# yell/boltzmann-machines

Measured on AMD Instinct MI355X. Metric: Gibbs-steps/sec (CD-k, 784x1024 RBM, batch 512), higher is better.
Workload: dtype f32

## Files before the change

boltzmann_machines_amd/_ffi.py:

```python
import ctypes as C
import os

import numpy as np

from . import build as _build

MAX_LAYERS = 4
UNIT_BERNOULLI, UNIT_GAUSSIAN, UNIT_MULTINOMIAL = 0, 1, 2


class Bm355Error(RuntimeError):
    pass


class RbmConfig(C.Structure):
    _fields_ = [('n_visible', C.c_int32), ('n_hidden', C.c_int32), ('v_unit', C.c_int32),
                ('sample_v_states', C.c_int32), ('sample_h_states', C.c_int32),
                ('dbm_first', C.c_int32), ('dbm_last', C.c_int32), ('max_batch', C.c_int32),
                ('l2', C.c_float), ('sparsity_target', C.c_float), ('sparsity_cost', C.c_float),
                ('sparsity_damping', C.c_float), ('dropout', C.c_float),
                ('h_unit', C.c_int32), ('n_samples', C.c_int32)]


class DbmConfig(C.Structure):
# ... 67 lines not shown
    'bm_rbm64_train_step': [_vp, _vp, C.c_int32, C.c_double, C.c_double, C.c_int32],
    'bm_rbm64_train_step_metrics': [_vp, _vp, C.c_int32, C.c_double, C.c_double, C.c_int32, C.POINTER(C.c_double)],
    'bm_rbm64_transform': [_vp, _vp, C.c_int32, C.c_int32, _vp],
    'bm_rbm64_metrics': [_vp, _vp, C.c_int32, C.c_int32, C.POINTER(C.c_double)],
    'bm_rbm64_free_energy': [_vp, _vp, C.c_int32, C.POINTER(C.c_double)],
    'bm_dbm64_create': [C.POINTER(DbmConfig), C.POINTER(C.c_double), C.POINTER(_vp)],
    'bm_dbm64_destroy': [_vp],
    'bm_dbm64_sync': [_vp],
    'bm_dbm64_seed': [_vp, C.c_uint64],
    'bm_dbm64_set_row_offset': [_vp, C.c_int64, C.c_int64],
    'bm_dbm64_set_param': [_vp, C.c_char_p, _vp, _sz],
    'bm_dbm64_get_param': [_vp, C.c_char_p, _vp, _sz],
    'bm_dbm64_train_step': [_vp, _vp, C.c_double, C.c_double, C.c_int32, C.POINTER(C.c_int32), C.POINTER(C.c_double)],
    'bm_dbm64_metrics': [_vp, _vp, C.c_int32, C.POINTER(C.c_int32), C.POINTER(C.c_double)],
    'bm_dbm64_mean_field': [_vp, _vp, _vp, C.POINTER(C.c_int32)],
    'bm_dbm64_reconstruct': [_vp, _vp, _vp],
    'bm_dbm64_sample_v': [_vp, C.c_int32, _vp],
    'bm_dbm64_ais': [_vp, C.c_int32, C.c_int32, C.c_int32, C.c_uint64, C.c_int64, _vp],
    'bm_dbm64_log_proba': [_vp, _vp, _vp],
    'bm_rbm_create': [C.POINTER(RbmConfig), C.POINTER(_vp)],
    'bm_rbm_destroy': [_vp],
    'bm_rbm_sync': [_vp],
    'bm_rbm_set_param': [_vp, C.c_char_p, _vp, _sz],
    'bm_rbm_get_param': [_vp, C.c_char_p, _vp, _sz],
    'bm_rbm_set_param_dev': [_vp, C.c_char_p, _vp, _sz],
    'bm_rbm_dev_ptr': [_vp, C.c_char_p, C.POINTER(_vp), C.POINTER(_sz)],
    'bm_rbm_seed': [_vp, _u64],
    'bm_rbm_set_row_offset': [_vp, _i64],
    'bm_rbm_train_step': [_vp, _vp, _i32, _f32, _f32, _i32],
    'bm_rbm_train_step_metrics': [_vp, _vp, _i32, _f32, _f32, _i32, _fp],
    'bm_rbm_train_step_metrics_async': [_vp, _vp, _i32, _f32, _f32, _i32],
    'bm_rbm_collect_metrics': [_vp, _fp, _i32, C.POINTER(C.c_int32)],
    'bm_rbm_train_epoch': [_vp, _vp, _i64, _i32, _f32, _f32, _i32],
    'bm_rbm_stage': [_vp, _i32],
    'bm_rbm_get_staged': [_vp, _i32, C.c_char_p, _vp, _sz],
    'bm_rbm_grad_step': [_vp, _vp, _i32, _i32],
    'bm_rbm_apply_step': [_vp, _i32, _f32, _f32],
    'bm_rbm_transform': [_vp, _vp, _i32, _i32, _vp],
    'bm_rbm_metrics': [_vp, _vp, _i32, _i32, _fp],
    'bm_rbm_free_energy': [_vp, _vp, _i32, _fp],
    'bm_rbm_free_energy_rows': [_vp, _vp, _i32, _vp],
    'bm_rbm_ais': [_vp, _i32, _i32, _i32, _vp, _u64, _i64, _vp],
    'bm_rbm_gibbs': [_vp, _vp, _vp, _i32, _i32],
    'bm_rbm_gibbs_clamped': [_vp, _vp, _vp, _vp, _i32, _i32, _vp, _vp],
    'bm_rbm_pt_init': [_vp, _i32, _i32, _vp, _vp, _i64],
    'bm_rbm_pt_sweep': [_vp, _i32],
    'bm_rbm_pt_read': [_vp, _vp, _vp, _vp, _vp],
    'bm_rbm_train_step_pt': [_vp, _vp, _i32, _f32, _f32, _i32],
    'bm_rbm_train_epoch_pt': [_vp, _vp, _i64, _i32, _f32, _f32, _i32],
    'bm_rbm_stream': [_vp, C.POINTER(_vp)],
    'bm_rbm_profile': [_vp, _i32],
    'bm_rbm_kernel_times': [_vp, _fp, _ip],
    'bm_rbm_chain_stats': [_vp, C.POINTER(C.c_int64)],
    'bm_rbm_timer_start': [_vp],
    'bm_rbm_timer_stop': [_vp, _fp],
    'bm_rbm_timer_mark': [_vp],
    'bm_rbm_timer_elapsed': [_vp, _fp],
    'bm_dbm_create': [C.POINTER(DbmConfig), C.POINTER(_vp)],
    'bm_dbm_destroy': [_vp],
    'bm_dbm_sync': [_vp],
    'bm_dbm_seed': [_vp, _u64],
    'bm_dbm_set_row_offset': [_vp, _i64, _i64],
    'bm_dbm_set_param': [_vp, C.c_char_p, _vp, _sz],
    'bm_dbm_get_param': [_vp, C.c_char_p, _vp, _sz],
    'bm_dbm_dev_ptr': [_vp, C.c_char_p, C.POINTER(_vp), C.POINTER(_sz)],
    'bm_dbm_train_step': [_vp, _vp, _f32, _f32, _i32, _ip, _fp],
    'bm_dbm_metrics': [_vp, _vp, _i32, _ip, _fp],
    'bm_dbm_grad_step': [_vp, _vp, _i32, _ip],
    'bm_dbm_apply_step': [_vp, _i32, _i32, _f32, _f32],
    'bm_dbm_set_mf_allreduce': [_vp, _vp, _vp],
    'bm_dbm_set_comm': [_vp, _vp],
    'bm_dbm_ais_sharded': [_vp, _vp, _i32, _i32, _i32, _u64, _vp],
    'bm_dbm_ais_sharded_direct': [_vp, _vp, _i32, _i32, _i32, _u64, _vp],
    'bm_dbm_stream': [_vp, C.POINTER(_vp)],
    'bm_dbm_mean_field': [_vp, _vp, _vp, _ip],
    'bm_dbm_reconstruct': [_vp, _vp, _vp],
    'bm_dbm_sample_v': [_vp, _i32, _vp],
    'bm_dbm_sample_v_clamped': [_vp, _i32, _vp, _vp, _vp],
    'bm_dbm_pt_init': [_vp, _i32, _i32, _vp, _vp, _i64],
    'bm_dbm_pt_sweep': [_vp, _i32],
    'bm_dbm_pt_read': [_vp, _vp, _vp, _vp, _vp, _vp],
    'bm_dbm_ais': [_vp, _i32, _i32, _i32, _u64, _i64, _vp],
    'bm_dbm_log_proba': [_vp, _vp, _vp],
    'bm_dbm_timer_start': [_vp],
    'bm_dbm_timer_stop': [_vp, _fp],
    'bm_dbm_timer_mark': [_vp],
    'bm_dbm_timer_elapsed': [_vp, _fp],
}
_RESTYPE = {'bm_last_error': C.c_char_p, 'bm_version': C.c_char_p}
MF_REDUCE_FN = C.CFUNCTYPE(C.c_float, C.c_float, C.c_void_p)

_lib = None


def load(rebuild=True):
    global _lib
    if _lib is not None:
        return _lib
    path = _build.LIB
    if rebuild and _build.needs_build():
        import shutil
        have_hipcc = bool(shutil.which('hipcc')) or os.path.exists('/opt/rocm/bin/hipcc')
        try:
            _build.build()
        except Exception as e:
            if have_hipcc or not os.path.exists(path):
# ... 86 lines not shown
```

boltzmann_machines_amd/csrc/bm_gemm.h:

```cpp
#pragma once
#include <hip/hip_runtime.h>
#include <stdint.h>
#include <stdlib.h>
#include <string.h>

namespace bm {

struct NoSide {
    static constexpr bool kFinalSync = true;
    static constexpr bool kSplitFill = false, kCohQ = false;
    static constexpr bool kCanAbort = false;
    __device__ __forceinline__ void wait_inputs() {}
    __device__ __forceinline__ void post_fill() {}
    __device__ __forceinline__ void fill() {}
    __device__ __forceinline__ void drain() {}
};

#define BM_ABL(bit) ((ABL >> (bit)) & 1)

typedef float f32x4 __attribute__((ext_vector_type(4)));
typedef float f32x2v __attribute__((ext_vector_type(2)));

constexpr int NT = 256;

enum : int { KM = 0, XM = 1 };

template <int WI_, int WJ_, int MI_, int NJ_, int BK_, int NB_ = 4>
struct Geo {
    static constexpr int WI = WI_, WJ = WJ_, MI = MI_, NJ = NJ_, BK = BK_;
    static constexpr int NBUF = NB_;
    static constexpr int PF = NB_ - 1;
    static constexpr int NW = WI * WJ;
    static constexpr int NT = 64 * NW;
    static constexpr int TI = 16 * MI * WI;
    static constexpr int TJ = 16 * NJ * WJ;
    static constexpr int E = 4 * MI;
    static constexpr int P_BUF = TI * BK;
    static constexpr int Q_BUF = TJ * BK;
    static constexpr int SMEM_FLOATS = NBUF * (P_BUF + Q_BUF);
    static constexpr int NPP = P_BUF * 4 / (1024 * NW);
    static constexpr int NPQ = Q_BUF * 4 / (1024 * NW);
    static constexpr int NVP = TI * BK / (4 * NT);
    static constexpr int NVQ = TJ * BK / (4 * NT);
    static constexpr int SP = (MI == 2) ? 8 : 4;
    static constexpr int SQ = (NJ == 2) ? 8 : 4;
    static_assert(MI == 1 || MI == 2, "MI");
    static_assert(NJ == 1 || NJ == 2, "NJ");
    static_assert(BK == 32 || BK == 64, "BK");
    static_assert(NB_ >= 4 && NB_ <= 8, "ring depth");
    static_assert(NPP >= 1 && NPP * 1024 * NW == P_BUF * 4, "P chunk must split into whole DMA pieces per wave");
    static_assert(NPQ >= 1 && NPQ * 1024 * NW == Q_BUF * 4, "Q chunk must split into whole DMA pieces per wave");
    static_assert(NVP >= 1 && NVP * 4 * NT == TI * BK && NVQ >= 1 && NVQ * 4 * NT == TJ * BK, "register path split");
    static_assert(SMEM_FLOATS * 4 <= 160 * 1024 - 1024, "LDS");
};
using GeoAct = Geo<2, 2, 2, 1, 64>;
using GeoAct8 = Geo<2, 4, 1, 1, 64>;
using GeoActS = Geo<2, 2, 1, 1, 64>;
using GeoActS32 = Geo<2, 2, 1, 1, 32>;
using GeoAct32 = Geo<2, 2, 2, 1, 32>;
using GeoGrad = Geo<2, 2, 2, 2, 64>;
using GeoGrad8 = Geo<2, 4, 2, 1, 64>;
using GeoGrad8h = Geo<2, 4, 2, 1, 32>;
using GeoBf3S = Geo<1, 4, 2, 1, 64>;

struct Operand {
    const float *ptr;
    int ld;
    int nx;
    int vec;
};

static inline Operand make_operand(const float *p, int ld, int nx) {
    Operand o;
    o.ptr = p; o.ld = ld; o.nx = nx;
    o.vec = (((uintptr_t)p & 15u) == 0 && (ld & 3) == 0) ? 1 : 0;
    return o;
}

static inline bool operand_fast(const Operand &o, int layout, int K) {
    if (!o.ptr) return true;
    if (!o.vec) return false;
    return layout == KM ? (o.nx % 4 == 0 && o.nx >= 4) : (K % 4 == 0);
}

template <int BK> __device__ __forceinline__ int fx(int row) { return (BK == 64) ? (row & 15) : ((row >> 1) & 7); }
template <int S> __device__ __forceinline__ int fk(int row) { return S * ((row >> 2) & 1); }

template <int L, int TX, int BK, int S>
__device__ __forceinline__ int img_off(int row, int c4) {
    return (L == XM) ? row * BK + ((c4 ^ fx<BK>(row)) << 2) : row * TX + ((c4 ^ fk<S>(row)) << 2);
}

__device__ __forceinline__ float4 load4_guard(const float *p, bool row_ok, int col, int ncols, bool vec) {
    float4 v = make_float4(0.f, 0.f, 0.f, 0.f);
    if (row_ok) {
        if (vec && col + 3 < ncols) {
            v = *reinterpret_cast<const float4 *>(p);
        } else {
            if (col     < ncols) v.x = p[0];
            if (col + 1 < ncols) v.y = p[1];
            if (col + 2 < ncols) v.z = p[2];
            if (col + 3 < ncols) v.w = p[3];
        }
    }
    return v;
}

__device__ __forceinline__ float4 load4_coh(const float *p) {
    const unsigned long long *q = reinterpret_cast<const unsigned long long *>(p);
    const unsigned long long a = __hip_atomic_load(q, __ATOMIC_RELAXED, __HIP_MEMORY_SCOPE_AGENT);
    const unsigned long long b = __hip_atomic_load(q + 1, __ATOMIC_RELAXED, __HIP_MEMORY_SCOPE_AGENT);
    return make_float4(__uint_as_float((unsigned)a), __uint_as_float((unsigned)(a >> 32)),
                       __uint_as_float((unsigned)b), __uint_as_float((unsigned)(b >> 32)));
}

template <int L, int TX, int BK, int NTH, bool FAST, bool COH = false>
__device__ __forceinline__ void g2r(float4 (&reg)[TX * BK / (4 * NTH)], const float *ptr, int ld, int nx, int vec,
                                    int x0, int k0, int K, int tid) {
    static_assert(!COH || FAST, "coherent register path: 16-byte-legal operands only");
    constexpr int NV = TX * BK / (4 * NTH);
    constexpr int RC = (L == KM) ? TX / 4 : BK / 4;
#pragma unroll
    for (int n = 0; n < NV; ++n) {
        const int f = tid + n * NTH;
        const int row = f / RC, c4 = f % RC;
        const int k = (L == KM) ? k0 + row : k0 + c4 * 4;
        const int x = (L == KM) ? x0 + c4 * 4 : x0 + row;
        if (FAST) {
            const int kc = (L == KM) ? min(k, K - 1) : min(k, K - 4);
            const int xc = (L == KM) ? min(x, nx - 4) : min(x, nx - 1);
            const float *pc = (L == KM) ? ptr + (size_t)kc * ld + xc : ptr + (size_t)xc * ld + kc;
            reg[n] = COH ? load4_coh(pc) : *reinterpret_cast<const float4 *>(pc);
        } else if (L == KM) {
            reg[n] = load4_guard(ptr + (size_t)k * ld + x, k < K, x, nx, vec);
        } else {
            reg[n] = load4_guard(ptr + (size_t)x * ld + k, x < nx, k, K, vec);
        }
    }
}

template <int L, int TX, int BK, int NTH, int S, bool ZF = true>
__device__ __forceinline__ void r2s(const float4 (&reg)[TX * BK / (4 * NTH)], float *s, int tid, int kz) {
    constexpr int NV = TX * BK / (4 * NTH);
    constexpr int RC = (L == KM) ? TX / 4 : BK / 4;
#pragma unroll
    for (int n = 0; n < NV; ++n) {
        const int f = tid + n * NTH;
        const int row = f / RC, c4 = f % RC;
        float4 v = reg[n];
        if (!ZF) {
        } else if (L == KM) {
            if (row >= kz) v = make_float4(0.f, 0.f, 0.f, 0.f);
        } else {
            const int k = c4 * 4;
            if (k     >= kz) v.x = 0.f;
            if (k + 1 >= kz) v.y = 0.f;
            if (k + 2 >= kz) v.z = 0.f;
            if (k + 3 >= kz) v.w = 0.f;
        }
        *reinterpret_cast<float4 *>(s + img_off<L, TX, BK, S>(row, c4)) = v;
    }
}

template <class G> struct Frags {
    float p[G::BK / 4][G::MI];
    float q[G::BK / 4][G::NJ];
};

template <int QL, class G, int ABL = 0, int PL = KM>
__device__ __forceinline__ void read_frags(Frags<G> &f, const float *sP, const float *sQ, int wi, int wj, int lane) {
    static_assert(PL == KM || G::MI == 1, "x-major P needs MI == 1 (no interleaved sub-tiles)");
    constexpr int BK = G::BK;
    const int g = lane >> 4, l15 = lane & 15;
    if (BM_ABL(3)) {
#pragma unroll
        for (int kk = 0; kk < BK / 4; ++kk) { f.p[kk][0] = 1.f; f.p[kk][G::MI - 1] = 2.f; f.q[kk][0] = 1.f; f.q[kk][G::NJ - 1] = 1.f; }
        return;
    }
    if (PL == XM) {
        const int row = wi * 16 + l15;
#pragma unroll
        for (int m = 0; m < BK / 16; ++m) {
            const f32x4 v = *reinterpret_cast<const f32x4 *>(sP + img_off<XM, 0, BK, 0>(row, 4 * m + g));
#pragma unroll
            for (int j = 0; j < 4; ++j) f.p[4 * m + j][0] = v[j];
// ... 90 lines not shown
    Operand P2, Q2; int K2;
};

__device__ __forceinline__ int sel_i(int a, int b, int m) { return a ^ ((a ^ b) & m); }
__device__ __forceinline__ const float *sel_p(const float *a, const float *b, int m) {
    const uintptr_t ua = (uintptr_t)a, ub = (uintptr_t)b;
    return (const float *)(ua ^ ((ua ^ ub) & (uintptr_t)(intptr_t)m));
}

template <class G, int DW = G::NW> struct DmaPlan {
    static constexpr int NPP = G::P_BUF / (256 * DW), NPQ = G::Q_BUF / (256 * DW);
    uint32_t p[NPP], q[NPQ];
};

template <int L, int TX, int BK, int NW, int NP, int S>
__device__ __forceinline__ void plan_offsets(uint32_t (&off)[NP], int ld, int nx, int x0, int wave, int lane) {
    constexpr int RC = (L == KM) ? TX / 4 : BK / 4;
    constexpr int R = 64 / RC;
#pragma unroll
    for (int n = 0; n < NP; ++n) {
        const int pc = wave + n * NW;
        const int row = pc * R + lane / RC, slot = lane % RC;
        if (L == KM) {
            const int c4 = slot ^ fk<S>(row);
            off[n] = (uint32_t)(row * ld + min(x0 + c4 * 4, nx - 4)) * 4u;
        } else {
            const int c4 = slot ^ fx<BK>(row);
            off[n] = (uint32_t)(min(x0 + row, nx - 1) * ld + c4 * 4) * 4u;
        }
    }
}

template <int QL, class G, int PL = KM, int DW = G::NW>
__device__ __forceinline__ void make_plan(DmaPlan<G, DW> &pl, const Operand &P, const Operand &Q, int i0, int j0, int wave, int lane) {
    plan_offsets<PL, G::TI, G::BK, DW, DmaPlan<G, DW>::NPP, G::SP>(pl.p, P.ld, P.nx, i0, wave, lane);
    plan_offsets<QL, G::TJ, G::BK, DW, DmaPlan<G, DW>::NPQ, G::SQ>(pl.q, Q.ld, Q.nx, j0, wave, lane);
}

__device__ __forceinline__ void dma16(const char *src, float *lds_dst) {
    unsigned keep;
    const unsigned lds_addr = (unsigned)(uintptr_t)(__attribute__((address_space(3))) void *)lds_dst;
    asm volatile("s_mov_b32 %0, m0\n\ts_mov_b32 m0, %2\n\ts_nop 0\n\tglobal_load_lds_dwordx4 %1, off\n\ts_mov_b32 m0, %0"
                 : "=&s"(keep) : "v"(src), "s"(__builtin_amdgcn_readfirstlane(lds_addr)) : "memory");
}

__device__ __forceinline__ void dma16s(const void *sbase, uint32_t voff, unsigned lds_byte) {
    asm volatile("s_mov_b32 m0, %2\n\ts_nop 0\n\tglobal_load_lds_dwordx4 %1, %0"
                 :: "s"(sbase), "v"(voff), "s"(lds_byte) : "memory");
}
__device__ __forceinline__ void dma16s_coh(const void *sbase, uint32_t voff, unsigned lds_byte) {
    asm volatile("s_mov_b32 m0, %2\n\ts_nop 0\n\tglobal_load_lds_dwordx4 %1, %0 sc1"
                 :: "s"(sbase), "v"(voff), "s"(lds_byte) : "memory");
}
template <class G, int DW, bool QSC = false, bool QHALF = false>
__device__ __forceinline__ void dma_chunk_s(const DmaPlan<G, DW> &pl, const char *pb, const char *qb, unsigned ldsP, unsigned ldsQ) {
#pragma unroll
    for (int n = 0; n < DmaPlan<G, DW>::NPP; ++n) dma16s(pb, pl.p[n], ldsP + (unsigned)(n * DW * 1024));
#pragma unroll
    for (int n = 0; n < DmaPlan<G, DW>::NPQ; ++n) {
        if (QHALF && (n & 1)) continue;
        if (QSC) dma16s_coh(qb, pl.q[n], ldsQ + (unsigned)(n * DW * 1024));
        else     dma16s(qb, pl.q[n], ldsQ + (unsigned)(n * DW * 1024));
    }
}

template <int QL, class G, bool SEG2, int PL = KM, int DW = G::NW, bool QHALF = false>
__device__ __forceinline__ void dma_chunk(const KRange &kr, const DmaPlan<G, DW> &pl1, const DmaPlan<G, DW> &pl2, int nch1, int c,
                                          float *sP, float *sQ, int wave) {
    constexpr int BK = G::BK;
    const int m = SEG2 ? -(int)(c >= nch1) : 0;
    const int kc = c - (nch1 & m);
    const int ldp = SEG2 ? sel_i(kr.P1.ld, kr.P2.ld, m) : kr.P1.ld;
    const int ldq = SEG2 ? sel_i(kr.Q1.ld, kr.Q2.ld, m) : kr.Q1.ld;
    const char *pb = (const char *)((SEG2 ? sel_p(kr.P1.ptr, kr.P2.ptr, m) : kr.P1.ptr) +
                                    ((PL == KM) ? (size_t)kc * BK * ldp : (size_t)kc * BK));
    const char *qb = (const char *)((SEG2 ? sel_p(kr.Q1.ptr, kr.Q2.ptr, m) : kr.Q1.ptr) +
                                    ((QL == KM) ? (size_t)kc * BK * ldq : (size_t)kc * BK));
#pragma unroll
    for (int n = 0; n < DmaPlan<G, DW>::NPP; ++n) {
        const uint32_t o1 = pl1.p[n], o2 = SEG2 ? pl2.p[n] : 0u;
        const uint32_t o = SEG2 ? (o1 ^ ((o1 ^ o2) & (uint32_t)m)) : o1;
        dma16(pb + o, sP + (wave + n * DW) * 256);
    }
#pragma unroll
    for (int n = 0; n < DmaPlan<G, DW>::NPQ; ++n) {
        if (QHALF && (n & 1)) continue;
        const uint32_t o1 = pl1.q[n], o2 = SEG2 ? pl2.q[n] : 0u;
        const uint32_t o = SEG2 ? (o1 ^ ((o1 ^ o2) & (uint32_t)m)) : o1;
        dma16(qb + o, sQ + (wave + n * DW) * 256);
    }
}

template <int QL, class G, bool FAST, bool SEG2, int PL = KM, bool COHQ = false>
__device__ __forceinline__ void load_chunk(ChunkRegs<G> &r, const KRange &kr, int nch1, int i0, int j0, int c, int tid) {
    constexpr int BK = G::BK;
    if (!SEG2) {
        g2r<PL, G::TI, BK, G::NT, FAST>(r.p, kr.P1.ptr, kr.P1.ld, kr.P1.nx, kr.P1.vec, i0, c * BK, kr.K1, tid);
        g2r<QL, G::TJ, BK, G::NT, FAST, COHQ>(r.q, kr.Q1.ptr, kr.Q1.ld, kr.Q1.nx, kr.Q1.vec, j0, c * BK, kr.K1, tid);
    } else {
        const int m = -(int)((c >= nch1) & (kr.K2 > 0));
        const int kc = c - (nch1 & m);
        const int K = sel_i(kr.K1, kr.K2, m);
        g2r<PL, G::TI, BK, G::NT, FAST>(r.p, sel_p(kr.P1.ptr, kr.P2.ptr, m), sel_i(kr.P1.ld, kr.P2.ld, m),
                                        sel_i(kr.P1.nx, kr.P2.nx, m), sel_i(kr.P1.vec, kr.P2.vec, m), i0, kc * BK, K, tid);
        g2r<QL, G::TJ, BK, G::NT, FAST, COHQ>(r.q, sel_p(kr.Q1.ptr, kr.Q2.ptr, m), sel_i(kr.Q1.ld, kr.Q2.ld, m),
                                              sel_i(kr.Q1.nx, kr.Q2.nx, m), sel_i(kr.Q1.vec, kr.Q2.vec, m), j0, kc * BK, K, tid);
    }
}

template <int QL, class G, bool SEG2, int PL = KM>
__device__ __forceinline__ void store_chunk(const ChunkRegs<G> &r, const KRange &kr, int nch1, int c,
                                            float *sP, float *sQ, int tid) {
    constexpr int BK = G::BK;
    const int m = SEG2 ? -(int)((c >= nch1) & (kr.K2 > 0)) : 0;
    const int kz = sel_i(kr.K1, kr.K2, m) - (c - (nch1 & m)) * BK;
    r2s<PL, G::TI, BK, G::NT, G::SP>(r.p, sP, tid, kz);
    r2s<QL, G::TJ, BK, G::NT, G::SQ>(r.q, sQ, tid, kz);
}

template <class G> struct RegPlan {
    uint32_t p[G::NVP], q[G::NVQ];
};
template <int L, int TX, int BK, int NTH>
__device__ __forceinline__ void reg_offsets(uint32_t (&off)[TX * BK / (4 * NTH)], int ld, int nx, int x0, int tid) {
    constexpr int NV = TX * BK / (4 * NTH);
    constexpr int RC = (L == KM) ? TX / 4 : BK / 4;
#pragma unroll
    for (int n = 0; n < NV; ++n) {
        const int f = tid + n * NTH;
        const int row = f / RC, c4 = f % RC;
        off[n] = (L == KM) ? (uint32_t)(row * ld + min(x0 + c4 * 4, nx - 4)) * 4u
                           : (uint32_t)(min(x0 + row, nx - 1) * ld + c4 * 4) * 4u;
    }
}
template <int QL, class G, int PL = KM>
__device__ __forceinline__ void make_reg_plan(RegPlan<G> &pl, const Operand &P, const Operand &Q, int i0, int j0, int tid) {
    reg_offsets<PL, G::TI, G::BK, G::NT>(pl.p, P.ld, P.nx, i0, tid);
    reg_offsets<QL, G::TJ, G::BK, G::NT>(pl.q, Q.ld, Q.nx, j0, tid);
}
template <int QL, class G, bool SEG2, int PL = KM>
__device__ __forceinline__ void load_chunk_slim(ChunkRegs<G> &r, const KRange &kr, const RegPlan<G> &pl1,
                                                const RegPlan<G> &pl2, int nch1, int c) {
    constexpr int BK = G::BK;
    const int m = SEG2 ? -(int)(c >= nch1) : 0;
    const int kc = c - (nch1 & m);
    const int ldp = SEG2 ? sel_i(kr.P1.ld, kr.P2.ld, m) : kr.P1.ld;
    const int ldq = SEG2 ? sel_i(kr.Q1.ld, kr.Q2.ld, m) : kr.Q1.ld;
    const char *pb = (const char *)((SEG2 ? sel_p(kr.P1.ptr, kr.P2.ptr, m) : kr.P1.ptr) +
                                    ((PL == KM) ? (size_t)kc * BK * ldp : (size_t)kc * BK));
    const char *qb = (const char *)((SEG2 ? sel_p(kr.Q1.ptr, kr.Q2.ptr, m) : kr.Q1.ptr) +
                                    ((QL == KM) ? (size_t)kc * BK * ldq : (size_t)kc * BK));
#pragma unroll
    for (int n = 0; n < G::NVP; ++n) {
        const uint32_t o1 = pl1.p[n], o2 = SEG2 ? pl2.p[n] : 0u;
        const uint32_t o = SEG2 ? (o1 ^ ((o1 ^ o2) & (uint32_t)m)) : o1;
        r.p[n] = *reinterpret_cast<const float4 *>(pb + o);
    }
#pragma unroll
// ... 8 lines not shown
    r2s<PL, G::TI, G::BK, G::NT, G::SP, false>(r.p, sP, tid, 0);
    r2s<QL, G::TJ, G::BK, G::NT, G::SQ, false>(r.q, sQ, tid, 0);
}

enum : int { STG_DMA = 0, STG_REG = 1, STG_DMAH = 2 };

#define BM_WAIT_VM(n) asm volatile("s_waitcnt vmcnt(%0)" ::"n"(n) : "memory")
template <int NPW, int MAXC>
__device__ __forceinline__ void wait_vm_chunks(int n) {
    static_assert(MAXC * NPW <= 63, "vmcnt range");
    if (MAXC >= 4 && n >= 4)      BM_WAIT_VM(4 * NPW <= 63 ? 4 * NPW : 0);
    else if (MAXC >= 3 && n == 3) BM_WAIT_VM(3 * NPW <= 63 ? 3 * NPW : 0);
    else if (MAXC >= 2 && n == 2) BM_WAIT_VM(2 * NPW <= 63 ? 2 * NPW : 0);
    else if (n == 1)              BM_WAIT_VM(NPW);
    else                          BM_WAIT_VM(0);
}
__device__ __forceinline__ void wg_barrier() {
    asm volatile("s_waitcnt lgkmcnt(0)" ::: "memory");
    __builtin_amdgcn_s_barrier();
    asm volatile("" ::: "memory");
}

template <int QL, class G, bool FAST, bool SEG2, int ABL = 0, int PL = KM, int STG = STG_DMA, class Side = NoSide>
__device__ __forceinline__ void mainloop(f32x4 (&acc)[G::MI][G::NJ], const KRange &kr, int i0, int j0, float *smem,
                                         Side &side, long long *stamps = nullptr) {
#ifdef BM_PROBE
#define BM_MSTAMP(n) do { if (stamps && threadIdx.x == 0) stamps[n] = (long long)__builtin_readcyclecounter(); } while (0)
#else
#define BM_MSTAMP(n) do {} while (0)
#endif
    constexpr int BK = G::BK, P_BUF = G::P_BUF, Q_BUF = G::Q_BUF, NBUF = G::NBUF, PF = G::PF;
    constexpr int DW = (STG == STG_DMAH && G::NW == 8) ? 4 : G::NW;
    constexpr int NPW = DmaPlan<G, DW>::NPP + (BM_ABL(9) ? (DmaPlan<G, DW>::NPQ + 1) / 2 : DmaPlan<G, DW>::NPQ);
    const int tid = threadIdx.x, lane = tid & 63;
    const int w = __builtin_amdgcn_readfirstlane(tid >> 6);
    const int wi = w % G::WI, wj = w / G::WI;
    float *sP = smem, *sQ = smem + NBUF * P_BUF;
    const int nch1 = (kr.K1 + BK - 1) / BK;
    const int nch = nch1 + (SEG2 ? (kr.K2 + BK - 1) / BK : 0);
    const int nfull1 = kr.K1 / BK, nfull2 = SEG2 ? kr.K2 / BK : 0;
    auto is_full = [&](int c) -> bool {
        return (c < nfull1) | (SEG2 && c >= nch1 && c - nch1 < nfull2);
    };
    auto is_dma = [&](int c) -> bool {
        if (!FAST || STG == STG_REG || BM_ABL(6)) return false;
        return is_full(c);
    };
    ChunkRegs<G> gr;
    Frags<G> fa, fb;
    DmaPlan<G, DW> pl1, pl2;
    RegPlan<G> rp1, rp2;
    const bool dmaw = (DW == G::NW) || w < DW;
    ChunkRegs<G> g0, g1;
    if (FAST && STG != STG_REG && dmaw) {
        make_plan<QL, G, PL, DW>(pl1, kr.P1, kr.Q1, i0, j0, w, lane);
        if (SEG2) make_plan<QL, G, PL, DW>(pl2, kr.P2, kr.Q2, i0, j0, w, lane);
    }
    int n_reg = 0;
    if (FAST && STG == STG_REG && !BM_ABL(6) && !BM_ABL(0)) {
        while (n_reg + 4 < nch && is_full(n_reg + 4) && is_full(n_reg + 2)) ++n_reg;
        n_reg &= ~1;
        if (n_reg > 0 && !(is_full(0) && is_full(1) && is_full(2) && is_full(3))) n_reg = 0;
        if (n_reg > 0) {
            make_reg_plan<QL, G, PL>(rp1, kr.P1, kr.Q1, i0, j0, tid);
            if (SEG2) make_reg_plan<QL, G, PL>(rp2, kr.P2, kr.Q2, i0, j0, tid);
        }
    }
    BM_MSTAMP(0);
    if (n_reg > 0) {
        ChunkRegs<G> ga, gb;
        load_chunk_slim<QL, G, SEG2, PL>(ga, kr, rp1, rp2, nch1, 0);
        load_chunk_slim<QL, G, SEG2, PL>(gb, kr, rp1, rp2, nch1, 1);
        load_chunk_slim<QL, G, SEG2, PL>(g0, kr, rp1, rp2, nch1, 2);
        load_chunk_slim<QL, G, SEG2, PL>(g1, kr, rp1, rp2, nch1, 3);
        __builtin_amdgcn_sched_barrier(0);
        side.fill();
        __builtin_amdgcn_sched_barrier(0);
        store_chunk_slim<QL, G, PL>(ga, sP, sQ, tid);
        store_chunk_slim<QL, G, PL>(gb, sP + P_BUF, sQ + Q_BUF, tid);
    } else if constexpr (Side::kSplitFill) {
        static_assert(FAST && STG == STG_DMA && DW == G::NW, "chained fill");
        const unsigned l0 = (unsigned)(uintptr_t)(__attribute__((address_space(3))) void *)smem;
        const unsigned lP = l0 + (unsigned)w * 1024u, lQ = l0 + (unsigned)(NBUF * P_BUF * 4) + (unsigned)w * 1024u;
#pragma unroll
        for (int c = 0; c < PF; ++c) {
            const char *pb = (const char *)kr.P1.ptr + (size_t)c * ((PL == KM) ? (size_t)BK * kr.P1.ld * 4 : (size_t)BK * 4);
#pragma unroll
            for (int n = 0; n < DmaPlan<G, DW>::NPP; ++n) dma16s(pb, pl1.p[n], lP + (unsigned)(c * P_BUF * 4 + n * DW * 1024));
        }
        __builtin_amdgcn_sched_barrier(0);
        side.fill();
        __builtin_amdgcn_sched_barrier(0);
        side.wait_inputs();
#pragma unroll
        for (int c = 0; c < PF; ++c) {
            const char *qb = (const char *)kr.Q1.ptr + (size_t)c * ((QL == KM) ? (size_t)BK * kr.Q1.ld * 4 : (size_t)BK * 4);
#pragma unroll
            for (int n = 0; n < DmaPlan<G, DW>::NPQ; ++n) dma16s_coh(qb, pl1.q[n], lQ + (unsigned)(c * Q_BUF * 4 + n * DW * 1024));
        }
        constexpr int NQ_LEFT = (PF - 2) * DmaPlan<G, DW>::NPQ;
        BM_WAIT_VM(NQ_LEFT);
    } else {
#pragma unroll
        for (int c = 0; c < PF; ++c)
            if (c < nch && is_dma(c) && dmaw && !BM_ABL(0))
                dma_chunk<QL, G, SEG2, PL, DW, (BM_ABL(9) != 0)>(kr, pl1, pl2, nch1, c, sP + (c % NBUF) * P_BUF, sQ + (c % NBUF) * Q_BUF, w);
        __builtin_amdgcn_sched_barrier(0);
        side.fill();
        __builtin_amdgcn_sched_barrier(0);
#pragma unroll
        for (int c = 0; c < 2; ++c)
            if (c < nch && !is_dma(c) && !BM_ABL(0)) {
                load_chunk<QL, G, FAST, SEG2, PL>(gr, kr, nch1, i0, j0, c, tid);
                store_chunk<QL, G, SEG2, PL>(gr, kr, nch1, c, sP + (c % NBUF) * P_BUF, sQ + (c % NBUF) * Q_BUF, tid);
            }
        {
            int n_after = 0;
#pragma unroll
            for (int c = 2; c < PF; ++c) n_after += (c < nch && is_dma(c) && !BM_ABL(0)) ? 1 : 0;
            wait_vm_chunks<NPW, PF - 2>(n_after);
        }
    }
    BM_MSTAMP(1);
    if (!BM_ABL(5)) wg_barrier();
    if constexpr (Side::kCanAbort) {
        side.post_fill();
        if (side.aborted) { BM_WAIT_VM(0); return; }
    }
    read_frags<QL, G, ABL, PL>(fa, sP, sQ, wi, wj, lane);
    BM_MSTAMP(2);
    const int klast = (SEG2 && kr.K2 > 0) ? kr.K2 - (nch - nch1 - 1) * BK : kr.K1 - (nch1 - 1) * BK;
    const int nq_last = (klast + 15) / 16;
    constexpr int NM = (BK / 4) * G::MI * G::NJ;
    constexpr int NRP = (PL == XM) ? BK / 16 : BK / 4;
    constexpr int NRQ = (QL == XM) ? (BK / 16) * G::NJ : BK / 4;
    constexpr int NR = NRP + NRQ;
#define BM_SG(mask, n) __builtin_amdgcn_sched_group_barrier(mask, n, 0);
#ifndef BM_SCHED_VARIANT
#define BM_SCHED_VARIANT 0
#endif
#if BM_SCHED_VARIANT == 0
#define BM_SCHED_STEP                                                                             \
    if (DW == G::NW) { _Pragma("unroll") for (int s_ = 0; s_ < NPW; ++s_) { BM_SG(0x008, 1) BM_SG(0x020, 1) } } \
    _Pragma("unroll") for (int s_ = 0; s_ < NR; ++s_) { BM_SG(0x008, 1) BM_SG(0x100, 1) }         \
    BM_SG(0x008, NM)
#elif BM_SCHED_VARIANT == 1
#define BM_SCHED_STEP                                                                             \
    _Pragma("unroll") for (int s_ = 0; s_ < NR; ++s_) { BM_SG(0x008, 1) BM_SG(0x100, 1) }         \
    _Pragma("unroll") for (int s_ = 0; s_ < NPW; ++s_) { BM_SG(0x008, 1) BM_SG(0x020, 1) }        \
    BM_SG(0x008, NM)
#else
#define BM_SCHED_STEP
#endif
    static_assert(NBUF == 4, "the steps below are written for a 4-slot ring");
    int cc = 0;
    const unsigned lds0 = (unsigned)(uintptr_t)(__attribute__((address_space(3))) void *)smem;
    const unsigned ldsPw = lds0 + (unsigned)w * 1024u, ldsQw = lds0 + (unsigned)(NBUF * P_BUF * 4) + (unsigned)w * 1024u;
    bool in2 = false;
    auto chunk_bases = [&](int c, const char *&pb, const char *&qb) {
        const bool s2 = SEG2 && c >= nch1;
        const Operand &P = s2 ? kr.P2 : kr.P1, &Q = s2 ? kr.Q2 : kr.Q1;
        const int kc = s2 ? c - nch1 : c;
        pb = (const char *)P.ptr + (size_t)kc * ((PL == KM) ? (size_t)BK * P.ld * 4 : (size_t)BK * 4);
        qb = (const char *)Q.ptr + (size_t)kc * ((QL == KM) ? (size_t)BK * Q.ld * 4 : (size_t)BK * 4);
    };
#define BM_DMA_AT(CD, SD)                                                                         \
    {                                                                                             \
        if (SEG2 && !in2 && (CD) >= nch1) { in2 = true; pl1 = pl2; }                              \
        const char *pb_, *qb_;                                                                    \
        chunk_bases((CD), pb_, qb_);                                                              \
        if (dmaw) dma_chunk_s<G, DW, Side::kCohQ, (BM_ABL(9) != 0)>(pl1, pb_, qb_, ldsPw + (unsigned)((SD) * P_BUF * 4), \
                                     ldsQw + (unsigned)((SD) * Q_BUF * 4));                       \
    }
#define BM_STEP_Q(FC, FN, S)                                                                      \
    {                                                                                             \
        BM_DMA_AT(cc + PF, ((S) + PF) % NBUF)                                                     \
        read_frags<QL, G, ABL, PL>(FN, sP + (((S) + 1) % NBUF) * P_BUF, sQ + (((S) + 1) % NBUF) * Q_BUF, wi, wj, lane); \
        mfma_frags<G, ABL>(acc, FC);                                                              \
        BM_SCHED_STEP                                                                             \
        if (!BM_ABL(8)) BM_WAIT_VM((PF - 2) * NPW);                                               \
        if (!BM_ABL(5)) wg_barrier();                                                             \
        ++cc;                                                                                     \
    }
#define BM_STEP_T(FC, FN, S1, S2, S3)       \
    {                                                                                             \
        const int cd = cc + PF, cr = cc + 2;                                                      \
        const bool do_dma = cd < nch && is_dma(cd) && !BM_ABL(0);                                 \
        const bool do_reg = cr < nch && !is_dma(cr) && !BM_ABL(0);                                \
        if (cc == last - 1) side.drain();       \
        if (do_reg) load_chunk<QL, G, FAST, SEG2, PL, Side::kCohQ>(gr, kr, nch1, i0, j0, cr, tid); \
        if (do_dma) BM_DMA_AT(cd, S3)                                                             \
        read_frags<QL, G, ABL, PL>(FN, sP + (S1) * P_BUF, sQ + (S1) * Q_BUF, wi, wj, lane);       \
        mfma_frags<G, ABL>(acc, FC);                                                              \
        _Pragma("unroll") for (int s_ = 0; s_ < NR; ++s_) { BM_SG(0x008, 1) BM_SG(0x100, 1) }     \
        BM_SG(0x008, NM)                                                                          \
        if (do_reg) {                                                                             \
            BM_WAIT_VM(0);                                                                        \
            store_chunk<QL, G, SEG2, PL>(gr, kr, nch1, cr, sP + (S2) * P_BUF, sQ + (S2) * Q_BUF, tid); \
        } else if (cr < nch) {                                                                    \
             \
            int n_after = 0;                                                                      \
            _Pragma("unroll") for (int c_ = 3; c_ <= PF; ++c_) n_after += (cc + c_ < nch && is_dma(cc + c_) && !BM_ABL(0)) ? 1 : 0; \
            wait_vm_chunks<NPW, PF - 2>(n_after);                                                 \
        }                                                                                         \
        if (!BM_ABL(5)) wg_barrier();                                                             \
        ++cc;                                                                                     \
    }
#define BM_STEP_TC(FC, FN, S) BM_STEP_T(FC, FN, ((S) + 1) % NBUF, ((S) + 2) % NBUF, ((S) + 3) % NBUF)
#define BM_STEP_TR(FC, FN)    BM_STEP_T(FC, FN, (cc + 1) % NBUF, (cc + 2) % NBUF, (cc + 3) % NBUF)
    constexpr int NWR = G::NVP + G::NVQ;
#ifndef BM_REG_SCHED_VARIANT
#define BM_REG_SCHED_VARIANT 0
#endif
#if BM_REG_SCHED_VARIANT == 0
#define BM_REG_SCHED(RELOAD)                                                                      \
        _Pragma("unroll") for (int s_ = 0; s_ < NWR; ++s_) { BM_SG(0x008, 1) BM_SG(0x200, 1) }    \
        if (RELOAD) { _Pragma("unroll") for (int s_ = 0; s_ < NWR; ++s_) { BM_SG(0x008, 1) BM_SG(0x020, 1) } } \
        _Pragma("unroll") for (int s_ = 0; s_ < NR; ++s_) { BM_SG(0x008, 1) BM_SG(0x100, 1) }     \
        BM_SG(0x008, NM)
#elif BM_REG_SCHED_VARIANT == 1
#define BM_REG_SCHED(RELOAD)                                                                      \
        _Pragma("unroll") for (int s_ = 0; s_ < NR; ++s_) { BM_SG(0x008, (NM >= 64 ? 2 : 1)) BM_SG(0x100, 2) } \
        _Pragma("unroll") for (int s_ = 0; s_ < NWR; ++s_) { BM_SG(0x008, (NM >= 32 ? 2 : 1)) BM_SG(0x200, 1) } \
        if (RELOAD) { _Pragma("unroll") for (int s_ = 0; s_ < NWR; ++s_) { BM_SG(0x008, 1) BM_SG(0x020, 1) } } \
        BM_SG(0x008, NM)
#else
#define BM_REG_SCHED(RELOAD)
#endif
#define BM_STEP_REG(FC, FN, G_, RELOAD, S)                                                        \
    {                                                                                             \
        store_chunk_slim<QL, G, PL>(G_, sP + (((S) + 2) % NBUF) * P_BUF, sQ + (((S) + 2) % NBUF) * Q_BUF, tid); \
        if (RELOAD) load_chunk_slim<QL, G, SEG2, PL>(G_, kr, rp1, rp2, nch1, cc + 4);             \
        read_frags<QL, G, ABL, PL>(FN, sP + (((S) + 1) % NBUF) * P_BUF, sQ + (((S) + 1) % NBUF) * Q_BUF, wi, wj, lane); \
        mfma_frags<G, ABL>(acc, FC);                                                              \
        BM_REG_SCHED(RELOAD)                                                                      \
        if (!BM_ABL(5)) wg_barrier();                                                             \
        ++cc;                                                                                     \
    }
    if (n_reg > 0) {
        int left = n_reg;
#pragma unroll 1
        while (left >= 4) {
            BM_STEP_REG(fa, fb, g0, true, 0)
// ... 200 lines not shown
```

boltzmann_machines_amd/csrc/bm_kernels.h:

```cpp
#pragma once
#include <stdio.h>
#include <stdlib.h>
#include <string.h>
#include "bm_gemm.h"
#include "bm_bf3.h"
#include "bm_numerics.h"
#include "bm_rng.h"

namespace bm {

struct MfCtl { unsigned maxdiff; int done; int steps; float resid; };

struct ActArgs {
    Operand P1, Q1; int K1;
    int p_xm;
    Operand P2, Q2; int K2;
    int I, J;
    const float *bias;
    const float *sigma;
    float mult;
    float bmult;
    int kind;
    int sample;
    int lit;
// ... 62 lines not shown
        if (a.kind == 0) {
#pragma unroll
            for (int r = 0; r < 4; ++r) s[r] = (u32_to_uniform(wds[r]) < m[r]) ? 1.f : 0.f;
        } else {
            float n[4];
            box_muller(wds[0], wds[1], n[0], n[1]);
            box_muller(wds[2], wds[3], n[2], n[3]);
#pragma unroll
            for (int r = 0; r < 4; ++r) s[r] = n[r] * a.sigma[ib + r] + m[r];
        }
    } else {
#pragma unroll
        for (int r = 0; r < 4; ++r) {
            if (r >= nvalid) break;
            const unsigned long long idx = flat + r;
            uint32_t wds[4];
            philox_block(key, idx >> 2, wds);
            if (a.kind == 0) {
                s[r] = (u32_to_uniform(wds[idx & 3]) < m[r]) ? 1.f : 0.f;
            } else {
                float n0, n1;
                const int pr = (int)(idx & 3) >> 1;
                box_muller(wds[2 * pr], wds[2 * pr + 1], n0, n1);
                s[r] = ((idx & 1) ? n1 : n0) * a.sigma[ib + r] + m[r];
            }
        }
    }
}

#ifndef BM_NT_STORES
#define BM_NT_STORES 1
#endif
typedef float f32x2 __attribute__((ext_vector_type(2)));
__device__ __forceinline__ void stream_store4(float *p, float x, float y, float z, float w) {
    if (BM_NT_STORES) __builtin_nontemporal_store((f32x4){x, y, z, w}, reinterpret_cast<f32x4 *>(p));
    else *reinterpret_cast<float4 *>(p) = make_float4(x, y, z, w);
}
__device__ __forceinline__ void stream_store2(float *p, float x, float y) {
    if (BM_NT_STORES) __builtin_nontemporal_store((f32x2){x, y}, reinterpret_cast<f32x2 *>(p));
    else *reinterpret_cast<float2 *>(p) = make_float2(x, y);
}

template <bool CACHED = false>
__device__ __forceinline__ void store4(float *dst, size_t o, const float *v, int nvalid, bool v4) {
    if (v4) {
        if (CACHED) *reinterpret_cast<float4 *>(dst + o) = make_float4(v[0], v[1], v[2], v[3]);
        else stream_store4(dst + o, v[0], v[1], v[2], v[3]);
    } else {
#pragma unroll
        for (int r = 0; r < 4; ++r) if (r < nvalid) dst[o + r] = v[r];
    }
}

template <int MI> struct PhiloxFor { typedef PhiloxPair type; };
template <> struct PhiloxFor<1> { typedef PhiloxOne type; };

__device__ __forceinline__ float wave_max_lane63(float v) {
#define BM_DPP_MAX(ctrl, rmask) v = fmaxf(v, __int_as_float(__builtin_amdgcn_update_dpp(__float_as_int(v), __float_as_int(v), ctrl, rmask, 0xf, false)))
    BM_DPP_MAX(0xb1, 0xf);
    BM_DPP_MAX(0x4e, 0xf);
    BM_DPP_MAX(0x124, 0xf);
    BM_DPP_MAX(0x128, 0xf);
    BM_DPP_MAX(0x142, 0xa);
    BM_DPP_MAX(0x143, 0xc);
#undef BM_DPP_MAX
    return v;
}

template <int E, class Rng, bool MF = false, int NTH = 256> struct ActSide {
    static constexpr bool kFinalSync = false;
    static constexpr bool kSplitFill = false, kCohQ = false, kCanAbort = MF;
    static constexpr bool kMF = MF;
    const float *bias, *sigma;
    const float *prev_row;
    int ib0, I, with_rng;
    float bs[E], sg[E], pv[E];
    Rng rng;
    MfCtl *chk_ctl; const float *chk_slots; int chk_n; float chk_tol; const int *skip; float *s_chk; int aborted, nthreads;

    __device__ __forceinline__ void load_inputs() {
        const float *sp = sigma ? sigma : bias;
        const bool has_sigma = sigma != nullptr;
        if (MF && prev_row) {
            if (E == 4 && ib0 + 3 < I && (((uintptr_t)prev_row & 15u) == 0)) {
                const float4 t = *reinterpret_cast<const float4 *>(prev_row);
                pv[0] = t.x; pv[1] = t.y; pv[2] = t.z; pv[E - 1] = t.w;
            } else {
#pragma unroll
                for (int e = 0; e < E; ++e) pv[e] = (ib0 + e < I) ? prev_row[e] : 0.f;
            }
        }
        if (MF && E == 4 && ib0 + 3 < I && (((uintptr_t)(bias + ib0) & 15u) == 0) && (((uintptr_t)(sp + ib0) & 15u) == 0)) {
            const float4 b = *reinterpret_cast<const float4 *>(bias + ib0), v = *reinterpret_cast<const float4 *>(sp + ib0);
            bs[0] = b.x; bs[1] = b.y; bs[2] = b.z; bs[E - 1] = b.w;
            sg[0] = has_sigma ? v.x : 1.0f; sg[1] = has_sigma ? v.y : 1.0f; sg[2] = has_sigma ? v.z : 1.0f; sg[E - 1] = has_sigma ? v.w : 1.0f;
            return;
        }
#pragma unroll
        for (int e = 0; e < E; ++e) {
            const int i = (ib0 + e < I) ? ib0 + e : I - 1;
            bs[e] = bias[i];
            const float sv = sp[i];
            sg[e] = has_sigma ? sv : 1.0f;
        }
    }
    static constexpr int CHK_MAX = 4096;
    float *s_slots;
    static __device__ __forceinline__ void dma4_lane0(const void *src, float *lds_dst) {
        if ((threadIdx.x & 63) == 0) {
            unsigned keep;
            const unsigned lds_addr = (unsigned)(uintptr_t)(__attribute__((address_space(3))) void *)lds_dst;
            asm volatile("s_mov_b32 %0, m0\n\ts_mov_b32 m0, %2\n\ts_nop 0\n\tglobal_load_lds_dword %1, off\n\ts_mov_b32 m0, %0"
                         : "=&s"(keep) : "v"(src), "s"(__builtin_amdgcn_readfirstlane(lds_addr)) : "memory");
        }
    }
    __device__ __forceinline__ void preload() {
        if constexpr (MF) {
            load_inputs();
            aborted = 0;
            const int w = threadIdx.x >> 6, lane = threadIdx.x & 63;
            if (chk_ctl) {
                for (int p = w; p * 256 < chk_n && p * 256 < CHK_MAX; p += nthreads / 64)
                    dma16(reinterpret_cast<const char *>(chk_slots + 256 * p) + 16 * lane, s_slots + 256 * p);
                if (w == 0) dma4_lane0(&chk_ctl->done, s_slots + CHK_MAX);
            } else if (skip) {
// ... 98 lines not shown
            const int ib = ib0 + 4 * hlf;
            if (ib >= a.I) break;
            const int nvalid = (a.I - ib < 4) ? a.I - ib : 4;
            float m[4], s[4];
#pragma unroll
            for (int r = 0; r < 4; ++r) {
                const float x = (RT ? rm : a.mult) * z[4 * hlf + r];
                const float b = (RT ? rm : a.bmult) * bs[4 * hlf + r];
                m[r] = (a.kind == 0) ? (LIT ? sigmoid_literal(x + b) : (HWMATH ? sigmoid_hw(x + b) : sigmoid(x + b)))
                                     : (a.kind == 1 ? (x * sg[4 * hlf + r] + b) : (a.kind == 3 ? x + b : x));
                s[r] = m[r];
            }
            if (a.sample) {
                if (rng_fast) {
                    const uint32_t *wds = rng.words(hlf);
                    if (a.kind == 0) {
#pragma unroll
                        for (int r = 0; r < 4; ++r) s[r] = (u32_to_uniform(wds[r]) < m[r]) ? 1.f : 0.f;
                    } else {
                        float n[4];
                        box_muller(wds[0], wds[1], n[0], n[1]);
                        box_muller(wds[2], wds[3], n[2], n[3]);
#pragma unroll
                        for (int r = 0; r < 4; ++r) s[r] = n[r] * sg[4 * hlf + r] + m[r];
                    }
                } else {
                    const unsigned long long flat = (unsigned long long)(a.row0 + j) * (unsigned long long)a.I + ib;
                    draw4(a, key, flat, ib, nvalid, m, s, false);
                }
            }
            if constexpr (CL) {
#pragma unroll
                for (int r = 0; r < 4; ++r)
                    if (cm[hlf][r] != 0.f) { m[r] = cv[hlf][r]; s[r] = cv[hlf][r]; }
            }
            if constexpr (RT) {
#pragma unroll
                for (int r = 0; r < 4; ++r) sv[4 * hlf + r] = s[r];
            }
            const size_t o = (size_t)j * a.ldo + ib;
            if constexpr (SideT::kMF) {
                if (a.prev) {
#pragma unroll
                    for (int r = 0; r < 4; ++r)
                        if (r < nvalid) dmax = fmaxf(dmax, fabsf(m[r] - side.pv[4 * hlf + r]));
                }
            }
            const bool v4 = al_out && nvalid == 4;
            if (a.means) store4<HWMATH>(a.means, o, m, nvalid, v4 && (((uintptr_t)a.means & 15u) == 0));
            if (a.negmeans) {
                float nm[4];
#pragma unroll
                for (int r = 0; r < 4; ++r) nm[r] = -m[r];
                store4<HWMATH>(a.negmeans, o, nm, nvalid, v4 && (((uintptr_t)a.negmeans & 15u) == 0));
            }
            if (a.states) store4<HWMATH>(a.states, o, s, nvalid, v4 && (((uintptr_t)a.states & 15u) == 0));
            if constexpr (RT) {
                if (a.sel_out && rm == 1.0f) {
                    const int c = j / a.sel_R;
                    if (c < a.sel_rows)
                        store4<HWMATH>(a.sel_out, (size_t)c * a.sel_ld + ib, s, nvalid,
                                       nvalid == 4 && ((a.sel_ld & 3) == 0) && (((uintptr_t)a.sel_out & 15u) == 0));
                }
            }
            if (HWMATH && a.states16) {
                uint16_t *d = a.states16 + (size_t)j * a.ld16 + ib;
                if (nvalid == 4 && (ib & 3) == 0) {
                    uint2 pk;
                    pk.x = (__float_as_uint(s[0]) >> 16) | (__float_as_uint(s[1]) & 0xffff0000u);
                    pk.y = (__float_as_uint(s[2]) >> 16) | (__float_as_uint(s[3]) & 0xffff0000u);
                    *reinterpret_cast<uint2 *>(d) = pk;
                } else {
#pragma unroll
                    for (int r = 0; r < 4; ++r) if (r < nvalid) d[r] = (uint16_t)(__float_as_uint(s[r]) >> 16);
                }
            }
        }
    }
    if constexpr (FE) { if (a.fe_zero && i0 == 0 && j0 == 0 && tid < 6) a.fe_zero[tid] = 0.0; }
    bool row_sums = a.rowacc || a.rowdot_out;
    if constexpr (RT) row_sums = row_sums || a.rowen_out;
    if (row_sums) {
        float racc = 0.f, rdot = 0.f, racc2 = 0.f, ren = 0.f;
        (void)ren;
        if (j < a.J) {
            int fc = 0; float delta = 0.f;
            if constexpr (FE) {
                fc = (a.fe_flip == FE_FLIP_FROM_KEY) ? pll_flip_col(a.fe_key, (unsigned long long)(a.row0 + j), a.K1) : a.fe_flip[j];
                delta = 1.0f - 2.0f * a.fe_x[(size_t)j * a.fe_ldx + fc];
            }
#pragma unroll
            for (int hlf = 0; hlf < NH; ++hlf) {
                float qa = 0.f, qd = 0.f, qa2 = 0.f, qe = 0.f;
                (void)qe;
#pragma unroll
                for (int r = 0; r < 4; ++r) {
                    const int e = 4 * hlf + r, i = ib0 + e;
                    if (i >= a.I) break;
                    if (a.rowacc) {
                        if (a.dot_mat) {
                            qa += z[e] * a.dot_mat[(size_t)j * a.ld_dot + i];
                        } else {
                            const float t = z[e] + bs[e];
                            if constexpr (FE) qa2 += softplus(t + delta * a.fe_w[(size_t)fc * a.fe_ldw + i]);
                            if (a.rowacc_single) qa += HWMATH ? softplus_hw(a.beta_b * t) : softplus(a.beta_b * t);
                            else qa += softplus_hw(a.beta_b * t) - softplus_hw(a.beta_a * t);
                        }
// ... 116 lines not shown

template <class G, bool SEG2, int MINW>
__global__ __launch_bounds__(G::NT, MINW) void act_bf3_kernel(ActArgs a, Bf3Strip sp) {
    __shared__ __attribute__((aligned(16))) float smem[Bf3Geo<G>::SMEM_FLOATS];
    constexpr int E = G::E;
    const int ti = (int)blockIdx.x / sp.strips, st = (int)blockIdx.x % sp.strips;
    const int per = sp.tiles_j / sp.strips, rem = sp.tiles_j % sp.strips;
    const int tj0 = st * per + (st < rem ? st : rem), tj1 = tj0 + per + (st < rem ? 1 : 0);
    const int i0 = ti * G::TI;
    const int tid = threadIdx.x, lane = tid & 63, w = tid >> 6;
    const int wi = w % G::WI, wj = w / G::WI;
    const int g = lane >> 4, l15 = lane & 15;
    const int ib0 = i0 + wi * (16 * G::MI) + g * E;
    ActSide<E, typename PhiloxFor<G::MI>::type> side;
    side.bias = a.bias; side.sigma = a.sigma; side.ib0 = ib0; side.I = a.I; side.with_rng = 0;
    side.prev_row = nullptr;
    side.fill();
    side.with_rng = a.sample;
    Bf3Pipe<G, SEG2> pipe;
    pipe.setup(a.b3, i0, smem);
    if (tj0 < tj1) { pipe.set_tile(a.b3, tj0 * G::TJ); pipe.prefetch(); }
    for (int tj = tj0; tj < tj1; ++tj) {
        const int j0 = tj * G::TJ, j = j0 + wj * 16 + l15;
        f32x4 acc[G::MI][1];
#pragma unroll
        for (int t = 0; t < G::MI; ++t) acc[t][0] = (f32x4){0.f, 0.f, 0.f, 0.f};
        side.rng.init(a.key, ((unsigned long long)(a.row0 + j) * (unsigned long long)a.I + ib0) >> 2);
        if (a.sample) side.rng.fill();
        if (!(sp.abl & 2)) pipe.run(acc);
        if (tj + 1 < tj1) { pipe.set_tile(a.b3, (tj + 1) * G::TJ); pipe.prefetch(); }
        if (!(sp.abl & 1)) (void)act_epilogue<G, 0, decltype(side), true>(a, a.key, acc, side, i0, j0);
    }
}

struct ColSumJob {
    const float *A, *Bm;
    int lda, ldb, ncols, nrows;
    float *out;
};
constexpr int MAX_COLJOBS = 12;
struct ColSumArgs {
    ColSumJob job[MAX_COLJOBS];
    int first_wave[MAX_COLJOBS + 1];
    int njobs;
};

constexpr int CS_ROWS = 128;
constexpr int CS_LD = 80;
constexpr int CS_SMEM_FLOATS = 2 * CS_ROWS * CS_LD;

constexpr int CS_NV = CS_ROWS * 16 / NT;
struct ColRegs { float4 a[CS_NV], b[CS_NV]; };

__device__ __forceinline__ void cs_fetch(ColRegs &r, const float *A, int lda, const float *Bm, int ldb,
                                         int c0, int ncols, int nrows, int r0, int tid) {
    const int c4 = tid & 15;
    const int cc = min(c0 + 4 * c4, ncols - 4);
#pragma unroll
    for (int n = 0; n < CS_NV; ++n) {
        const int rc = min(r0 + (tid >> 4) + 16 * n, nrows - 1);
        r.a[n] = *reinterpret_cast<const float4 *>(A + (size_t)rc * lda + cc);
        r.b[n] = Bm ? *reinterpret_cast<const float4 *>(Bm + (size_t)rc * ldb + cc) : make_float4(0.f, 0.f, 0.f, 0.f);
    }
}

__device__ __forceinline__ void cs_stash(const ColRegs &r, float *sA, float *sB, int c0, int ncols, int nrows,
                                         int r0, int tid) {
    const int c4 = tid & 15;
#pragma unroll
    for (int n = 0; n < CS_NV; ++n) {
        const int row = (tid >> 4) + 16 * n;
        const bool ok = (r0 + row < nrows) && (c0 + 4 * c4 < ncols);
        float4 va = r.a[n], vb = r.b[n];
        if (!ok) { va = make_float4(0.f, 0.f, 0.f, 0.f); vb = va; }
        *reinterpret_cast<float4 *>(sA + row * CS_LD + 4 * c4) = va;
        *reinterpret_cast<float4 *>(sB + row * CS_LD + 4 * c4) = vb;
    }
}

__device__ __forceinline__ void block_colsum(const float *A, int lda, const float *Bm, int ldb,
                                             int c0, int ncols, int nrows, bool want2,
                                             float *smem, f32x4 &sum1, f32x4 &sum2, bool negB = false) {
    const int tid = threadIdx.x, lane = tid & 63, w = tid >> 6;
    const int g = lane >> 4, l15 = lane & 15;
    float *sA = smem, *sB = smem + CS_ROWS * CS_LD;
    sum1 = (f32x4){0.f, 0.f, 0.f, 0.f};
    sum2 = (f32x4){0.f, 0.f, 0.f, 0.f};
    const bool vec = (((uintptr_t)A & 15u) == 0) && ((lda & 3) == 0) && ((ncols & 3) == 0) &&
                     (!Bm || ((((uintptr_t)Bm & 15u) == 0) && ((ldb & 3) == 0)));
    ColRegs regs;
    if (vec) cs_fetch(regs, A, lda, Bm, ldb, c0, ncols, nrows, 0, tid);
    for (int r0 = 0; r0 < nrows; r0 += CS_ROWS) {
        const int nr = (nrows - r0 < CS_ROWS) ? nrows - r0 : CS_ROWS;
        if (vec) {
            cs_stash(regs, sA, sB, c0, ncols, nrows, r0, tid);
        } else {
            for (int e = tid; e < CS_ROWS * 64; e += NT) {
                const int row = e >> 6, cc = e & 63, c = c0 + cc;
                const bool ok = row < nr && c < ncols;
                sA[row * CS_LD + cc] = ok ? A[(size_t)(r0 + row) * lda + c] : 0.f;
                sB[row * CS_LD + cc] = (ok && Bm) ? Bm[(size_t)(r0 + row) * ldb + c] : 0.f;
            }
        }
        wg_barrier();
        if (vec) cs_fetch(regs, A, lda, Bm, ldb, c0, ncols, nrows, r0 + CS_ROWS, tid);
        const int nsteps = (((nr + 3) / 4) + 7) & ~7;
        const int co = w * 16 + l15;
        for (int s = 0; s < nsteps; s += 8) {
            float d[8], e[8];
#pragma unroll
            for (int u = 0; u < 8; ++u) {
                const int o = (4 * (s + u) + g) * CS_LD + co;
                e[u] = sB[o];
                d[u] = negB ? sA[o] + e[u] : sA[o] - e[u];
            }
#pragma unroll
            for (int u = 0; u < 8; ++u) {
                sum1 = __builtin_amdgcn_mfma_f32_16x16x4f32(d[u], 1.0f, sum1, 0, 0, 0);
                if (want2) sum2 = __builtin_amdgcn_mfma_f32_16x16x4f32(e[u], 1.0f, sum2, 0, 0, 0);
            }
        }
        wg_barrier();
    }
    if (negB) sum2 = -sum2;
}

__global__ __launch_bounds__(NT) void colsum_kernel(ColSumArgs a) {
    __shared__ __attribute__((aligned(16))) float smem[CS_SMEM_FLOATS];
    const int wv = blockIdx.x, lane = threadIdx.x & 63, w = threadIdx.x >> 6;
    int jb = 0;
    while (jb + 1 < a.njobs && wv >= a.first_wave[jb + 1]) ++jb;
    const ColSumJob J = a.job[jb];
    const int c0 = (wv - a.first_wave[jb]) * 64;
    f32x4 s1, s2;
    block_colsum(J.A, J.lda, J.Bm, J.ldb, c0, J.ncols, J.nrows, false, smem, s1, s2);
    if ((lane & 15) == 0) {
        const int g = lane >> 4;
#pragma unroll
        for (int r = 0; r < 4; ++r) {
            const int cc = c0 + w * 16 + g * 4 + r;
            if (cc < J.ncols) J.out[cc] = s1[r];
        }
    }
}

struct RbmBiasArgs {
    const float *sv, *sh, *sq;
    float *vb, *dvb, *hb, *dhb, *q, *pen;
    int V, H;
    float N, lr, mom, damping, cost, target;
};
__global__ void rbm_bias_kernel(RbmBiasArgs a) {
    const int c = blockIdx.x * blockDim.x + threadIdx.x;
    if (c < a.V) {
        const float g = a.sv[c] / a.N;
        const float d = a.lr * (a.mom * a.dvb[c] + g);
        a.dvb[c] = d;
        a.vb[c] = a.vb[c] + d;
    } else if (c < a.V + a.H) {
        const int h = c - a.V;
        const float qn = a.damping * a.q[h] + (1.0f - a.damping) * a.sq[h];
        a.q[h] = qn;
        const float pen = a.cost * (qn - a.target);
        a.pen[h] = pen;
        float g = a.sh[h] / a.N;
        g = g - pen;
        const float d = a.lr * (a.mom * a.dhb[h] + g);
        a.dhb[h] = d;
        a.hb[h] = a.hb[h] + d;
    }
}

struct RbmBiasFusedArgs {
    const float *X, *vs, *h0m, *hm;
    int ldx, ldv, ldh0, ldh, B;
    int hm_negated;
    float *raw_tail;
    int raw_only;
    RbmBiasArgs u;
};
__device__ __forceinline__ void rbm_bias_fused_block(const RbmBiasFusedArgs &a, int wv, float *smem) {
    const int lane = threadIdx.x & 63, w = threadIdx.x >> 6, g = lane >> 4;
    const int nv = (a.u.V + 63) / 64;
    f32x4 s1, s2;
    if (wv < nv) {
        const int c0 = wv * 64;
        block_colsum(a.X, a.ldx, a.vs, a.ldv, c0, a.u.V, a.B, false, smem, s1, s2);
        if ((lane & 15) == 0) {
#pragma unroll
            for (int r = 0; r < 4; ++r) {
                const int c = c0 + w * 16 + g * 4 + r;
                if (c < a.u.V) {
                    a.raw_tail[c] = s1[r];
                    if (a.raw_only) continue;
                    const float gr = s1[r] / a.u.N;
                    const float d = a.u.lr * (a.u.mom * a.u.dvb[c] + gr);
                    a.u.dvb[c] = d;
                    a.u.vb[c] = a.u.vb[c] + d;
                }
            }
        }
    } else {
        const int c0 = (wv - nv) * 64;
        block_colsum(a.h0m, a.ldh0, a.hm, a.ldh, c0, a.u.H, a.B, true, smem, s1, s2, a.hm_negated != 0);
        if ((lane & 15) == 0) {
#pragma unroll
            for (int r = 0; r < 4; ++r) {
                const int h = c0 + w * 16 + g * 4 + r;
                if (h < a.u.H) {
                    const float sq = s2[r];
                    a.raw_tail[a.u.V + h] = s1[r];
                    a.raw_tail[a.u.V + a.u.H + h] = sq;
                    if (a.raw_only) continue;
                    const float qn = a.u.damping * a.u.q[h] + (1.0f - a.u.damping) * sq;
                    a.u.q[h] = qn;
                    const float pen = a.u.cost * (qn - a.u.target);
                    a.u.pen[h] = pen;
                    float gr = s1[r] / a.u.N;
                    gr = gr - pen;
                    const float d = a.u.lr * (a.u.mom * a.u.dhb[h] + gr);
                    a.u.dhb[h] = d;
                    a.u.hb[h] = a.u.hb[h] + d;
                }
            }
        }
    }
}

__global__ __launch_bounds__(NT) void rbm_bias_fused_kernel(RbmBiasFusedArgs a) {
    __shared__ __attribute__((aligned(16))) float smem[CS_SMEM_FLOATS];
    rbm_bias_fused_block(a, blockIdx.x, smem);
}

struct GradArgs {
    Operand Ppos, Qpos; int Kpos;
    Operand Pneg, Qneg; int Kneg;
    int I, J;
    int form;
    int fused;
    float *raw;
    float *raw2;
    float *W, *dW;
    float *Wt;
    int ldw, ldwt;
    const float *pen;
    float N, M, l2, lr, mom;
    int nbias;
    RbmBiasFusedArgs bias;
    int fetch_at_fill;
    int map_xi;
#ifdef BM_PROBE
    long long *dbg;
#endif
};

__device__ __forceinline__ void apply_w_update(float g, float pen, float l2, float lr, float mom,
                                               float &w, float &dw) {
    g = __fsub_rn(g, __fmul_rn(l2, w));
    g = __fsub_rn(g, pen);
    const float d = __fmul_rn(lr, __fadd_rn(__fmul_rn(mom, dw), g));
    dw = d;
    w = __fadd_rn(w, d);
}
__device__ __forceinline__ bool grad_pow2(float N) { return ((__float_as_uint(N) & 0x007fffffu) == 0u) && N >= 1.0f; }
__device__ __forceinline__ float grad_norm1(float r, float N, float invN, bool pow2) {
    return pow2 ? __fmul_rn(r, invN) : __fdiv_rn(r, N);
}
__device__ __forceinline__ float grad_norm2(float r, float r2, float N, float M, float invN, float invM, bool pow2) {
    return pow2 ? __fsub_rn(__fmul_rn(r, invN), __fmul_rn(r2, invM)) : __fsub_rn(__fdiv_rn(r, N), __fdiv_rn(r2, M));
}

struct DivBy {
    float n, inv; bool pow2;
    __device__ __forceinline__ explicit DivBy(float N) : n(N), inv(1.0f / N),
        pow2(grad_pow2(N)) {}
};

template <int NJ> struct GradSide {
    static constexpr bool kFinalSync = true;
    static constexpr bool kSplitFill = false, kCohQ = false, kCanAbort = false;
    const float *W, *dW; int ldw, I, J, ib0, jb[NJ]; bool on, vec8;
    float4 w[NJ][2], d[NJ][2];
    bool at_fill;
    __device__ __forceinline__ void fill() { if (at_fill) fetch(); }
    __device__ __forceinline__ void drain() { if (!at_fill) fetch(); }
    __device__ __forceinline__ void fetch() {
        if (!on || ib0 >= I) return;
#pragma unroll
        for (int n = 0; n < NJ; ++n) {
            if (jb[n] >= J) continue;
            const size_t o = (size_t)jb[n] * ldw + ib0;
            if (vec8) {
                w[n][0] = *reinterpret_cast<const float4 *>(W + o);  w[n][1] = *reinterpret_cast<const float4 *>(W + o + 4);
                d[n][0] = *reinterpret_cast<const float4 *>(dW + o); d[n][1] = *reinterpret_cast<const float4 *>(dW + o + 4);
            } else {
                float tw[8], td[8];
#pragma unroll
                for (int e = 0; e < 8; ++e) {
                    const bool ok = ib0 + e < I;
                    tw[e] = ok ? W[o + e] : 0.f;
                    td[e] = ok ? dW[o + e] : 0.f;
                }
                w[n][0] = make_float4(tw[0], tw[1], tw[2], tw[3]); w[n][1] = make_float4(tw[4], tw[5], tw[6], tw[7]);
                d[n][0] = make_float4(td[0], td[1], td[2], td[3]); d[n][1] = make_float4(td[4], td[5], td[6], td[7]);
            }
        }
    }
};

template <class G, bool FAST, int ABL = 0, int STG = STG_DMA, int MINB = 1>
__global__ __launch_bounds__(G::NT, MINB) void grad_kernel(GradArgs a, TileMap tmap) {
    constexpr int TI = G::TI, NJ = G::NJ;
    static_assert(G::MI == 2 && G::TI == 64 && G::TJ == 64, "grad_kernel: 64 x 64 tiles, 8 consecutive outputs per lane");
    __shared__ __attribute__((aligned(16))) float smem[G::SMEM_FLOATS];
    constexpr bool kBias = G::SMEM_FLOATS >= CS_SMEM_FLOATS;
    static_assert(G::NT >= NT, "bias path");
    const int ntile_blocks = (int)gridDim.x - a.nbias;
    if ((int)blockIdx.x >= ntile_blocks) {
        if constexpr (kBias) {
            if (G::NT > NT && threadIdx.x >= NT) return;
            rbm_bias_fused_block(a.bias, (int)blockIdx.x - ntile_blocks, smem);
        }
        return;
    }
    asm volatile("" :: "s"(a.Ppos.ptr), "s"(a.Qpos.ptr), "s"(a.Ppos.ld), "s"(a.Qpos.ld), "s"(a.Ppos.nx), "s"(a.Qpos.nx),
                       "s"(a.Pneg.ptr), "s"(a.Qneg.ptr), "s"(a.Pneg.ld), "s"(a.Qneg.ld), "s"(a.Kpos), "s"(a.Kneg),
                       "s"(a.I), "s"(a.J), "s"(a.W), "s"(a.dW), "s"(a.ldw), "s"(a.form), "s"(a.fused));
    constexpr int TJ2 = G::TJ;
    int ti, tj;
    if (tmap.slab) {
        block_to_tile((a.J + TJ2 - 1) / TJ2, ti, tj, 0, a.nbias);
    } else {
        TILE_WORDS(tmap, (int)blockIdx.x);
        TILE_OF_BLOCK(tmap, (int)blockIdx.x, ntile_blocks, ti, tj);
    }
    const int i0 = ti * TI, j0 = tj * TJ2;
    const int tid = threadIdx.x, lane = tid & 63, w = tid >> 6;
    const int wi = w % G::WI, wj = w / G::WI;
    const int g = lane >> 4, l15 = lane & 15;
    const int ib0 = i0 + wi * 32 + g * 8;

#ifdef BM_PROBE
#define BM_GSTAMP(n) do { if (a.dbg && threadIdx.x == 0) a.dbg[blockIdx.x * 4 + (n)] = (long long)__builtin_readcyclecounter(); } while (0)
#else
#define BM_GSTAMP(n) do {} while (0)
#endif
    BM_GSTAMP(0);
    f32x4 pos[2][NJ], neg[2][NJ];
#pragma unroll
    for (int t = 0; t < 2; ++t)
#pragma unroll
        for (int n = 0; n < NJ; ++n) pos[t][n] = neg[t][n] = (f32x4){0.f, 0.f, 0.f, 0.f};
    GradSide<NJ> side;
    side.W = a.W; side.dW = a.dW; side.ldw = a.ldw; side.I = a.I; side.J = a.J; side.ib0 = ib0;
#pragma unroll
    for (int n = 0; n < NJ; ++n) side.jb[n] = j0 + wj * (16 * NJ) + lane_j<KM, G>(l15, n);
    side.vec8 = (ib0 + 7 < a.I) && ((a.ldw & 3) == 0);
    side.at_fill = true;
    side.on = a.fused != 0 && a.fetch_at_fill != 0;
    KRange kr;
    kr.P1 = a.Ppos; kr.Q1 = a.Qpos; kr.K1 = a.Kpos;
    if (a.form == 0) {
        kr.P2 = a.Pneg; kr.Q2 = a.Qneg; kr.K2 = a.Kneg;
        mainloop<KM, G, FAST, true, ABL, KM, STG>(pos, kr, i0, j0, smem, side);
    } else {
        kr.P2 = a.Ppos; kr.Q2 = a.Qpos; kr.K2 = 0;
        mainloop<KM, G, FAST, false, 0, KM, STG>(pos, kr, i0, j0, smem, side);
        kr.P1 = a.Pneg; kr.Q1 = a.Qneg; kr.K1 = a.Kneg;
        mainloop<KM, G, FAST, false, 0, KM, STG>(neg, kr, i0, j0, smem, side);
    }

    BM_GSTAMP(1);
    if (ib0 >= a.I) return;
    if (!a.fetch_at_fill) { side.on = a.fused != 0; side.fetch(); }
    const DivBy divN(a.N), divM(a.M);
    float wt[NJ][8];
    bool jok[NJ];
#pragma unroll
    for (int n = 0; n < NJ; ++n) {
        const int j = side.jb[n];
        jok[n] = j < a.J;
        if (!jok[n]) continue;
        float pv[8], nv[8];
        lane_outputs<G>(pos, n, pv);
        lane_outputs<G>(neg, n, nv);
        const size_t o = (size_t)j * a.ldw + ib0;
        if (!a.fused) {
#pragma unroll
            for (int e = 0; e < 8; ++e) {
                if (ib0 + e >= a.I) break;
                a.raw[o + e] = pv[e];
                if (a.form != 0) a.raw2[o + e] = nv[e];
            }
            continue;
        }
        float wv[8] = {side.w[n][0].x, side.w[n][0].y, side.w[n][0].z, side.w[n][0].w, side.w[n][1].x, side.w[n][1].y, side.w[n][1].z, side.w[n][1].w};
        float dv[8] = {side.d[n][0].x, side.d[n][0].y, side.d[n][0].z, side.d[n][0].w, side.d[n][1].x, side.d[n][1].y, side.d[n][1].z, side.d[n][1].w};
        float pe[8];
#pragma unroll
        for (int e = 0; e < 8; ++e) pe[e] = (a.pen && ib0 + e < a.I) ? a.pen[ib0 + e] : 0.f;
        float gr[8];
        if (divN.pow2 && divM.pow2) {
#pragma unroll
            for (int e = 0; e < 8; ++e) gr[e] = (a.form == 0) ? grad_norm1(pv[e], a.N, divN.inv, true)
                                                              : grad_norm2(pv[e], nv[e], a.N, a.M, divN.inv, divM.inv, true);
        } else {
#pragma unroll
            for (int e = 0; e < 8; ++e) gr[e] = (a.form == 0) ? grad_norm1(pv[e], a.N, 0.f, false)
                                                              : grad_norm2(pv[e], nv[e], a.N, a.M, 0.f, 0.f, false);
        }
#pragma unroll
        for (int e = 0; e < 8; ++e) {
            apply_w_update(gr[e], pe[e], a.l2, a.lr, a.mom, wv[e], dv[e]);
            wt[n][e] = wv[e];
        }
        if (side.vec8) {
            stream_store4(a.W + o, wv[0], wv[1], wv[2], wv[3]);
            stream_store4(a.W + o + 4, wv[4], wv[5], wv[6], wv[7]);
            stream_store4(a.dW + o, dv[0], dv[1], dv[2], dv[3]);
            stream_store4(a.dW + o + 4, dv[4], dv[5], dv[6], dv[7]);
        } else {
#pragma unroll
            for (int e = 0; e < 8; ++e)
                if (ib0 + e < a.I) { a.W[o + e] = wv[e]; a.dW[o + e] = dv[e]; }
        }
    }
    if (a.fused && a.Wt) {
        const int ja = side.jb[0];
        const bool pair = NJ == 2 && jok[0] && jok[NJ - 1] && ((a.ldwt & 1) == 0);
#pragma unroll
        for (int e = 0; e < 8; ++e) {
            if (ib0 + e >= a.I) break;
            float *dst = a.Wt + (size_t)(ib0 + e) * a.ldwt + ja;
            if (pair) {
                stream_store2(dst, wt[0][e], wt[NJ - 1][e]);
            } else {
                if (jok[0]) dst[0] = wt[0][e];
                if (NJ == 2 && jok[NJ - 1]) dst[1] = wt[NJ - 1][e];
            }
        }
    }
    BM_GSTAMP(2);
}

struct ApplyWArgs {
    const float *raw, *raw2;
    float *W, *dW, *Wt;
    const float *pen;
    int I, J, ldw, ldwt;
    int form;
    float N, M, l2, lr, mom;
};
__global__ void apply_w_kernel(ApplyWArgs a) {
    const size_t n = (size_t)a.I * a.J;
    for (size_t e = (size_t)blockIdx.x * blockDim.x + threadIdx.x; e < n; e += (size_t)gridDim.x * blockDim.x) {
        const int i = (int)(e % (size_t)a.I), j = (int)(e / (size_t)a.I);
        const size_t o = (size_t)j * a.ldw + i;
        const float gr = (a.form == 0) ? grad_norm1(a.raw[o], a.N, 0.f, false) : grad_norm2(a.raw[o], a.raw2[o], a.N, a.M, 0.f, 0.f, false);
        float wv = a.W[o], dv = a.dW[o];
        apply_w_update(gr, a.pen ? a.pen[i] : 0.f, a.l2, a.lr, a.mom, wv, dv);
        a.W[o] = wv;
        a.dW[o] = dv;
        if (a.Wt) a.Wt[(size_t)i * a.ldwt + j] = wv;
    }
}

__device__ __forceinline__ void rbm_bias_update(const RbmBiasArgs &a, int c) {
    if (c < a.V) {
        const float g = a.sv[c] / a.N;
        const float d = a.lr * (a.mom * a.dvb[c] + g);
        a.dvb[c] = d;
        a.vb[c] = a.vb[c] + d;
    } else if (c < a.V + a.H) {
        const int h = c - a.V;
        const float qn = a.damping * a.q[h] + (1.0f - a.damping) * a.sq[h];
        a.q[h] = qn;
        const float pen = a.cost * (qn - a.target);
        a.pen[h] = pen;
        float g = a.sh[h] / a.N;
        g = g - pen;
        const float d = a.lr * (a.mom * a.dhb[h] + g);
        a.dhb[h] = d;
        a.hb[h] = a.hb[h] + d;
    }
}
__global__ __launch_bounds__(256) void apply_w_tiled_kernel(ApplyWArgs a, RbmBiasArgs b, int nbias) {
    __shared__ float tile[64][65];
    const int ntile = (int)gridDim.x - nbias;
    if ((int)blockIdx.x >= ntile) {
        rbm_bias_update(b, ((int)blockIdx.x - ntile) * 256 + (int)threadIdx.x);
        return;
    }
    const int tiles_i = (a.I + 63) / 64;
    const int i0 = ((int)blockIdx.x % tiles_i) * 64, j0 = ((int)blockIdx.x / tiles_i) * 64;
    const int tid = threadIdx.x, c4 = tid & 15, r0 = tid >> 4;
// ... 718 lines not shown
```

boltzmann_machines_amd/csrc/bm_launch.h:

```cpp
#pragma once
#include <array>
#include <map>
#include <mutex>
#include "bm_common.h"

namespace bm {

template <class G> static inline int tile_grid(int I, int J) { return ((I + G::TI - 1) / G::TI) * ((J + G::TJ - 1) / G::TJ); }

static inline int device_cu_count() {
    static const int n = [] {
        hipDeviceProp_t pr;
        int d = 0;
        (void)hipGetDevice(&d);
        return (hipGetDeviceProperties(&pr, d) == hipSuccess && pr.multiProcessorCount > 0) ? pr.multiProcessorCount : 256;
    }();
    return n;
}
static inline int dbg_int(const char *name) { const char *e = dbg(name); return e ? atoi(e) : 0; }

constexpr int XI_MODEL = 0, XI_SLAB = -1;
struct Tuned { int geo = 0; int xi = XI_MODEL; };
constexpr int TUNE_REP = 4, TUNE_ROUNDS = 3;
constexpr float NOT_TIMED = 1e30f;
// ... 297 lines not shown
                      operand_fast(g.Pneg, KM, g.Kneg) && operand_fast(g.Qneg, KM, g.Kneg);
    const dim3 grid(tile_grid<G>(g.I, g.J) + g.nbias), blk(G::NT);
    if (fast) hipLaunchKernelGGL((grad_kernel<G, true, 0, STG, MINB>), grid, blk, 0, st, g, tmap);
    else      hipLaunchKernelGGL((grad_kernel<G, false, 0, STG_DMA, MINB>), grid, blk, 0, st, g, tmap);
}
static inline void launch_grad_as(int geo, const GradArgs &g, hipStream_t st) {
    if (geo == 9 && g.nbias == 0) launch_grad_geo<GeoGrad8h, STG_DMA, 4>(g, st);
    else if (geo == 9)   launch_grad_geo<GeoGrad8, STG_DMA>(g, st);
    else if (geo == 208) launch_grad_geo<GeoGrad8, STG_DMAH>(g, st);
    else if (geo == 108) launch_grad_geo<GeoGrad8, STG_REG>(g, st);
    else if (geo == 104) launch_grad_geo<GeoGrad, STG_REG>(g, st);
    else if (geo == 8)   launch_grad_geo<GeoGrad8, STG_DMA>(g, st);
    else                 launch_grad_geo<GeoGrad, STG_DMA>(g, st);
}
static inline Tuned tune_grad_shape(const GradArgs &g, hipStream_t st) {
    constexpr int NC = 5;
    static const int cand[NC] = {4, 8, 104, 108, 9};
    Tuned T;
    T.geo = 4;
    const size_t mat = (((size_t)g.J * (size_t)g.ldw) + 3) & ~(size_t)3;
    float *s = tune_scratch(4 * mat);
    if (!s) return T;
    GradArgs t = g;
    t.nbias = 0; t.pen = nullptr; t.Wt = nullptr;
    t.W = s; t.dW = s + mat; t.raw = s + 2 * mat; t.raw2 = s + 3 * mat;
    (void)hipMemsetAsync(s, 0, 4 * mat * sizeof(float), st);
#ifdef BM_PROBE
    t.dbg = nullptr;
#endif
    TuneTimer tm;
    if (!tm.init(st)) return T;
    float us[NC], xi_us[5];
    best_of(tm, TUNE_ROUNDS, TUNE_REP, NC, us, [&](int c) { launch_grad_as(cand[c], t, st); });
    const int b = fastest(us, NC);
    if (b >= 0) T.geo = cand[b];
    T.xi = tune_tile_map(tm, t, xi_us, [&] { launch_grad_as(T.geo, t, st); });
    if (tune_log())
        fprintf(stderr, "bm355 tune: grad I=%d J=%d K=%d+%d form=%d fused=%d -> geometry %d (us, dma: 4w %.1f, 8w %.1f; reg: 4w %.1f, 8w %.1f; 8w bk32 x2: %.1f), "
                        "tile map %d (9 slab, else XCD grid xi; us: slab %.1f, 8x1 %.1f, 4x2 %.1f, 2x4 %.1f, 1x8 %.1f)\n",
                g.I, g.J, g.Kpos, g.Kneg, g.form, g.fused, T.geo, us[0], us[1], us[2], us[3], us[4], T.xi == XI_SLAB ? 9 : T.xi, xi_us[4], xi_us[0], xi_us[1], xi_us[2], xi_us[3]);
    return T;
}
static inline void launch_grad(const GradArgs &g_in, hipStream_t st) {
    static const int fetch_env = std::max(0, dbg_int("grad_fetch")), geo_env = dbg_int("grad_geo");
    GradArgs g = g_in;
    g.fetch_at_fill = fetch_env;
    if (geo_env) { launch_grad_as(geo_env, g, st); return; }
    static TuneMemo<6> memo;
    const Tuned T = memo.get({g.I, g.J, g.Kpos, g.Kneg, g.form | (g.fused << 1), g.ldw}, [&] { return tune_grad_shape(g, st); });
    if (T.xi != XI_MODEL && !g.map_xi) g.map_xi = T.xi;
    launch_grad_as(T.geo, g, st);
}

static inline void launch_fe_hidden(const FeArgs &f, hipStream_t st) {
    const bool fast = operand_fast(f.P, KM, f.K) && operand_fast(f.Q, XM, f.K);
    const dim3 grid(tile_grid<GeoAct>(f.I, f.J)), blk(NT);
    if (fast) hipLaunchKernelGGL((fe_hidden_kernel<true>), grid, blk, 0, st, f);
    else      hipLaunchKernelGGL((fe_hidden_kernel<false>), grid, blk, 0, st, f);
}

static inline void launch_apply_w(const ApplyWArgs &a, const RbmBiasArgs *bias, hipStream_t st) {
    const bool tiled = (a.I % 4 == 0) && (a.ldw % 4 == 0) && (!a.Wt || a.ldwt % 4 == 0);
    if (tiled) {
        RbmBiasArgs b;
        memset(&b, 0, sizeof(b));
        int nb = 0;
        if (bias) { b = *bias; nb = (b.V + b.H + 255) / 256; }
        const int ntile = ((a.I + 63) / 64) * ((a.J + 63) / 64);
        hipLaunchKernelGGL(apply_w_tiled_kernel, dim3(ntile + nb), dim3(256), 0, st, a, b, nb);
    } else {
        if (bias) hipLaunchKernelGGL(rbm_bias_kernel, dim3((bias->V + bias->H + 255) / 256), dim3(256), 0, st, *bias);
        hipLaunchKernelGGL(apply_w_kernel, dim3(1024), dim3(256), 0, st, a);
    }
}

}
```

boltzmann_machines_amd/csrc/bm_rbm.hip:

```cpp
#include "../../include/bm355.h"
#include "bm_common.h"
#include "bm_kernels.h"
#include "bm_chain.h"
#include "bm_pt.h"

#include <math.h>
#include <atomic>
#include <memory>

namespace bm {

static thread_local char g_err[1024] = "";
void set_error(const char *fmt, ...) {
    va_list ap;
    va_start(ap, fmt);
    vsnprintf(g_err, sizeof(g_err), fmt, ap);
    va_end(ap);
}

enum : uint32_t { SITE_DROPOUT = 1, SITE_H0 = 2, SITE_V = 3, SITE_H = 4, SITE_PLL = 5, SITE_FE = 6 };
enum : uint32_t { SITE_AIS_V0 = 7, SITE_AIS_V = 8, SITE_AIS_H = 9 };
enum : uint32_t { SITE_PT_SWAP = 10, SITE_PT_V0 = 11 };

}

using namespace bm;

struct bm_xchg;
static int xchg_check_status(bm_xchg *x);
static void xchg_bind_user(bm_xchg *x, bm_xchg **slot);
static void xchg_dw_replaced(bm_xchg *x);

struct bm_rbm {
    bm_rbm_config cfg;
    bm_xchg *xchg_used = nullptr;
    bool dw_sharded = false;
    int V, H, maxB;
    Stream stream;
    Stream comm_stream;
    Stream stage_stream;
    Event ev0, ev1;
    Mat W, dW;
    Mat Wt;
    bool use_wt = false, wt_valid = false;
    DevBuf vb, hb, dvb, dhb, q, sigma;
    Mat h0m, h0s, hm, hs, hneg;
    Mat vm, vs, Xs, Xd;
    DevBuf grad;
    DevBuf grad_alt;
    int grad_slot = 0;
    Event ev_ready[2], ev_reduced[2];
    DevBuf pen;
    DevBuf rowacc;
    DevBuf hhat;
    DevArray<int> flip;
    DevArray<double> scal;
    bool multinomial() const { return cfg.h_unit == BM_UNIT_MULTINOMIAL; }
    uint64_t seed = 0;
    uint32_t call = 0;
    int64_t row0 = 0;
    const float *Xin = nullptr;
    int Xin_ld = 0;
    bool hm_is_neg = false;
    bool fe_in_chain = false;
    DevBuf fe_part;
    int ais_rows = 0;
    Mat av, ah;
    DevBuf apart_h, apart_v;
    DevArray<double> alogw;
    DevBuf abase, adot, abeta, atable;
    int pt_rows = 0, pt_M = 0, pt_R = 0;
    int64_t pt_chain0 = 0;
    long long pt_step = 0;
    Mat ptv, pth;
    DevBuf ptpart_v, ptpart_h;
    DevBuf pt_mult, pt_beta;
    DevArray<int> pt_idx;
    DevArray<unsigned long long> pt_cnt;
    int fer_rows = 0;
    DevBuf fer_part, fer_out;
    int fast = 0;
    bool fast_now = false;
    Mat16 W3, W3t, hs16, vs16;
    DevArray<int> nonbinary;
    struct Stage { Mat W, dW; DevBuf vb, hb, dvb, dhb, q, sigma; Event ev; bool ready = false;
                   std::atomic<int> readers{0}; } stage[2];
    int last_stage = -1;
    Pinned<float> stage_host;
    int device = 0;
    static constexpr int MRING = 4096;
    Pinned<double> mring;
    double *mring_dev = nullptr;
    std::vector<int> mring_B;
    int mring_n = 0;
    Event ev_mlast;
    bool prof = false;
    struct Rec { int cls; Event a, b; };
    std::vector<Rec> recs;
    size_t grad_tail() const { return (size_t)V * W.ld; }
    ChainState chain;
};

enum { KC_UP = 0, KC_DOWN = 1, KC_GRAD = 2, KC_COLSUM = 3, KC_BIAS = 4, KC_OTHER = 5 };

static int check_dw(const bm_rbm *h, const char *what) {
    BM_CHECK(!h->dw_sharded, "%s: after bm_rbm_exchange_apply_direct this rank holds only its slice of the momentum buffer dW; "
             "every rank must call bm_rbm_exchange_gather_dw first (DirectExchange.gather_dw())", what);
    return 0;
}

struct ProfScope {
    bm_rbm *h; hipEvent_t b = nullptr;
    ProfScope(bm_rbm *h_, int cls) : h(h_) {
        if (!h->prof) return;
        bm_rbm::Rec r{cls};
        (void)create(r.a); (void)create(r.b);
        (void)hipEventRecord(r.a, h->stream);
        b = r.b;
        h->recs.push_back(std::move(r));
    }
    ~ProfScope() { if (b) (void)hipEventRecord(b, h->stream); }
};

static PhiloxKey make_key(const bm_rbm *h, uint32_t site, int t) {
    PhiloxKey k;
    k.k0 = (uint32_t)h->seed;
    k.k1 = (uint32_t)(h->seed >> 32);
    k.site = site + 16u * (uint32_t)t;
    k.call = h->call;
    return k;
}

static void act_pass(bm_rbm *h, const ActArgs &a, const Operand *alt_p = nullptr) {
    if (h->chain.on) {
        h->chain.rec.push_back(a);
        h->chain.alt_p.resize(h->chain.rec.size(), Operand{nullptr, 0, 0, 0});
        if (alt_p) h->chain.alt_p.back() = *alt_p;
    } else if (alt_p) {
        ActArgs b = a;
        b.P1 = *alt_p; b.p_xm = 1;
        launch_act(b, h->stream);
    } else launch_act(a, h->stream);
}
static void chain_begin(bm_rbm *h) {
    h->chain.on = !h->prof && !h->multinomial() && !h->fast_now && chain_mode(h->chain) > 0;
}
static int chain_end(bm_rbm *h) {
    BM_CHECK(chain_flush(h->chain, h->stream, h->maxB) == 0, "chained launch: %s", hipGetErrorString(hipGetLastError()));
    return 0;
}

static void ensure_wt(bm_rbm *h) {
    if (!h->use_wt || h->wt_valid) return;
    const int nt = ((h->V + 31) / 32) * ((h->H + 31) / 32);
    hipLaunchKernelGGL(transpose_kernel, dim3(nt), dim3(256), 0, h->stream, (const float *)h->W.p, h->W.ld, h->Wt.p, h->Wt.ld, h->V, h->H);
    h->wt_valid = true;
}

static void launch_up(bm_rbm *h, const float *v, int ldv, int B, float *means, float *states, int ldo,
                      int sample, uint32_t site, int t, float *negmeans = nullptr, bool fe = false) {
    ProfScope _ps(h, KC_UP);
    ActArgs a;
    memset(&a, 0, sizeof(a));
    a.P1 = make_operand(h->W.p, h->W.ld, h->H);
    a.Q1 = make_operand(v, ldv, B);
    a.K1 = h->V;
    a.I = h->H; a.J = B;
    a.bias = h->hb.p; a.sigma = nullptr;
    a.mult = 1.0f + (h->cfg.dbm_first ? 1.0f : 0.0f);
    a.bmult = a.mult;
    a.kind = BM_UNIT_BERNOULLI;
    a.sample = states ? sample : 0;
    a.means = means; a.states = states; a.negmeans = negmeans; a.ldo = ldo;
    a.key = make_key(h, site, t);
    a.row0 = h->row0;
    if (fe) {
        const int nslot = (h->H + 15) / 16, rm = (nslot + 3) & ~3;
        a.rowacc = h->fe_part.p; a.rowacc_single = 1; a.beta_b = 1.f; a.ld_part = h->maxB; a.fe_rm = rm;
        a.fe_rowacc2 = h->fe_part.p + (size_t)rm * h->maxB;
        a.fe_flip = FE_FLIP_FROM_KEY; a.fe_key = make_key(h, SITE_PLL, 0); a.fe_zero = h->scal.p;
        a.fe_x = v; a.fe_ldx = ldv; a.fe_w = h->W.p; a.fe_ldw = h->W.ld;
    }
    if (h->fast_now && v == h->vs.p) {
        a.b3.P1 = Bf3Operand{h->W3t.p, h->W3t.plane_stride(), h->W3t.ld, h->H};
        a.b3.Q1 = Bf3Operand{h->vs16.p, 0, h->vs16.ld, B};
        a.b3.K1 = h->vs16.ld;
        if (states == h->hs.p) { a.states16 = h->hs16.p; a.ld16 = h->hs16.ld; }
    }
    if (h->multinomial()) {
        if (!means) { means = h->hm.p; ldo = h->hm.ld; }
        a.kind = 3; a.sample = 0; a.means = means; a.ldo = ldo; a.states = nullptr; a.negmeans = nullptr;
        launch_act(a, h->stream);
        SmArgs m;
        memset(&m, 0, sizeof(m));
        m.L = means; m.ld = ldo; m.I = h->H; m.J = B; m.M = h->cfg.n_samples; m.sample = sample;
        m.states = states; m.negmeans = negmeans; m.key = a.key; m.row0 = h->row0;
        hipLaunchKernelGGL(softmax_multinomial_kernel, dim3(B), dim3(64), 2 * (size_t)h->H * sizeof(float), h->stream, m);
        return;
    }
    if (h->use_wt && h->wt_valid && !(h->fast_now && v == h->vs.p)) {
        const Operand wt = make_operand(h->Wt.p, h->Wt.ld, h->H);
        act_pass(h, a, &wt);
    } else act_pass(h, a);
}

static void launch_down(bm_rbm *h, const float *hs, int ldh, int B, float *means, float *states, int ldo,
                        int sample, uint32_t site, int t, const float *clamp_val = nullptr, const float *clamp_mask = nullptr) {
    ProfScope _ps(h, KC_DOWN);
    ActArgs a;
    memset(&a, 0, sizeof(a));
    a.P1 = make_operand(h->W.p, h->W.ld, h->V);
    a.p_xm = 1;
    a.Q1 = make_operand(hs, ldh, B);
    a.K1 = h->H;
    a.I = h->V; a.J = B;
    a.bias = h->vb.p; a.sigma = h->sigma.p;
    a.mult = 1.0f + (h->cfg.dbm_last ? 1.0f : 0.0f);
    a.bmult = a.mult;
    a.kind = h->cfg.v_unit;
    a.sample = sample;
    a.means = means; a.states = states; a.ldo = ldo;
    a.key = make_key(h, site, t);
    a.row0 = h->row0;
    a.clamp_val = clamp_val; a.clamp_mask = clamp_mask; a.ld_clamp = h->V;
    if (h->fast_now && hs == h->hs.p) {
        a.b3.P1 = Bf3Operand{h->W3.p, h->W3.plane_stride(), h->W3.ld, h->V};
        a.b3.Q1 = Bf3Operand{h->hs16.p, 0, h->hs16.ld, B};
        a.b3.K1 = h->hs16.ld;
        if (states == h->vs.p) { a.states16 = h->vs16.p; a.ld16 = h->vs16.ld; }
    }
    act_pass(h, a);
}

static bool metrics_fused_ok(const bm_rbm *h);
static void metrics_prep(bm_rbm *h, int B);
static int run_chain(bm_rbm *h, const float *X_dev, int B, int k, float *hm_out, bool need_vm = true, bool for_update = false,
                     bool split_step = false, bool fetch = false) {
    BM_CHECK(B >= 1 && B <= h->maxB, "batch %d outside [1, max_batch=%d]", B, h->maxB);
    BM_CHECK(k >= 1, "n_gibbs_steps must be >= 1 (got %d)", k);
    if (!split_step) ensure_wt(h);
    const float *Xin = X_dev;
    int ldx = h->V;
    if (h->cfg.v_unit == BM_UNIT_GAUSSIAN) {
        hipLaunchKernelGGL(div_cols_kernel, dim3(256), dim3(256), 0, h->stream, Xin, ldx, h->sigma.p, h->Xs.p,
                           h->Xs.ld, B, h->V);
        Xin = h->Xs.p; ldx = h->Xs.ld;
    }
    if (h->cfg.dropout >= 0.f) {
        hipLaunchKernelGGL(dropout_kernel, dim3(256), dim3(256), 0, h->stream, Xin, ldx, h->Xd.p, h->Xd.ld, B, h->V,
                           h->cfg.dropout, make_key(h, SITE_DROPOUT, 0),
                           (unsigned long long)h->row0 * (unsigned long long)h->V);
        Xin = h->Xd.p; ldx = h->Xd.ld;
    }
    h->Xin = Xin; h->Xin_ld = ldx;
    const bool fe = fetch && metrics_fused_ok(h);
    if (fe && !h->fe_part.p) BM_TRY(h->fe_part.alloc((size_t)2 * ((((h->H + 15) / 16) + 3) & ~3) * h->maxB));
    h->fe_in_chain = fe;
    if (fetch && !fe) metrics_prep(h, B);
    chain_begin(h);
    launch_up(h, Xin, ldx, B, h->h0m.p, h->h0s.p, h->h0m.ld, 1, SITE_H0, 0, nullptr, fe);
    const float *hstate = h->cfg.sample_h_states ? h->h0s.p : h->h0m.p;
    for (int t = 0; t < k; ++t) {
        const bool last = t == k - 1;
        launch_down(h, hstate, h->hs.ld, B, (need_vm && last) ? h->vm.p : nullptr, h->vs.p, h->vm.ld,
                    h->cfg.sample_v_states, SITE_V, t);
        const bool last_out = hm_out && last;
        const bool neg_only = last && !hm_out && !need_vm && !h->multinomial();
        h->hm_is_neg = neg_only;
        launch_up(h, h->vs.p, h->vs.ld, B, last_out ? hm_out : (neg_only ? nullptr : h->hm.p), last ? nullptr : h->hs.p,
                  last_out ? h->H : h->hm.ld, h->cfg.sample_h_states, SITE_H, t, (!hm_out && last) ? h->hneg.p : nullptr);
        hstate = h->hs.p;
    }
    BM_TRY(chain_end(h));
    return 0;
}

static void fill_bias(bm_rbm *h, float N, float lr, float mom, RbmBiasArgs &b) {
    float *tail = h->grad.p + h->grad_tail();
    b.sv = tail; b.sh = tail + h->V; b.sq = tail + h->V + h->H;
    b.vb = h->vb.p; b.dvb = h->dvb.p; b.hb = h->hb.p; b.dhb = h->dhb.p; b.q = h->q.p; b.pen = h->pen.p;
    b.V = h->V; b.H = h->H;
    b.N = N; b.lr = lr; b.mom = mom;
    b.damping = h->cfg.sparsity_damping; b.cost = h->cfg.sparsity_cost; b.target = h->cfg.sparsity_target;
}

static int fill_bias_fused(bm_rbm *h, int B, float lr, float mom, RbmBiasFusedArgs &a) {
    memset(&a, 0, sizeof(a));
    a.X = h->Xin; a.ldx = h->Xin_ld; a.vs = h->vs.p; a.ldv = h->vs.ld;
    a.h0m = h->h0m.p; a.ldh0 = h->h0m.ld; a.B = B;
    if (h->hm_is_neg) { a.hm = h->hneg.p; a.ldh = h->hneg.ld; a.hm_negated = 1; }
    else              { a.hm = h->hm.p; a.ldh = h->hm.ld; }
    a.raw_tail = h->grad.p + h->grad_tail();
    RbmBiasArgs &b = a.u;
    b.vb = h->vb.p; b.dvb = h->dvb.p; b.hb = h->hb.p; b.dhb = h->dhb.p; b.q = h->q.p; b.pen = h->pen.p;
    b.V = h->V; b.H = h->H;
    b.N = (float)B; b.lr = lr; b.mom = mom;
    b.damping = h->cfg.sparsity_damping; b.cost = h->cfg.sparsity_cost; b.target = h->cfg.sparsity_target;
    return (h->V + 63) / 64 + (h->H + 63) / 64;
}

static void launch_bias_fused(bm_rbm *h, int B, float lr, float mom) {
    ProfScope _ps(h, KC_COLSUM);
    RbmBiasFusedArgs a;
    const int nw = fill_bias_fused(h, B, lr, mom, a);
    hipLaunchKernelGGL(rbm_bias_fused_kernel, dim3(nw), dim3(NT), 0, h->stream, a);
}

static void rbm_grad(bm_rbm *h, int B, int fused, float N, float lr, float mom, bool with_bias);

static void launch_update_fused(bm_rbm *h, int B, float lr, float mom) {
    if (h->cfg.sparsity_cost != 0.f) {
        launch_bias_fused(h, B, lr, mom);
        rbm_grad(h, B, 1, (float)B, lr, mom, false);
    } else {
        rbm_grad(h, B, 1, (float)B, lr, mom, true);
    }
}

static void fill_grad(bm_rbm *h, int B, int fused, float N, float lr, float mom, GradArgs &g) {
    memset(&g, 0, sizeof(g));
    g.Ppos = make_operand(h->h0m.p, h->h0m.ld, h->H);
    g.Qpos = make_operand(h->Xin, h->Xin_ld, h->V);
    g.Kpos = B;
    g.Pneg = make_operand(h->hneg.p, h->hneg.ld, h->H);
    g.Qneg = make_operand(h->vs.p, h->vs.ld, h->V);
    g.Kneg = B;
    g.I = h->H; g.J = h->V;
    g.form = 0; g.fused = fused;
    g.raw = h->grad.p; g.raw2 = nullptr;
    g.W = h->W.p; g.dW = h->dW.p; g.Wt = nullptr;
    g.ldw = h->W.ld; g.ldwt = 0;
    if (h->use_wt && fused) { g.Wt = h->Wt.p; g.ldwt = h->Wt.ld; }
    g.N = N; g.M = N; g.l2 = h->cfg.l2; g.lr = lr; g.mom = mom;
}
static void rbm_grad(bm_rbm *h, int B, int fused, float N, float lr, float mom, bool with_bias) {
    ProfScope _ps(h, KC_GRAD);
    GradArgs g;
    fill_grad(h, B, fused, N, lr, mom, g);
    g.pen = with_bias ? nullptr : h->pen.p;
    if (with_bias) {
        g.nbias = fill_bias_fused(h, B, lr, mom, g.bias);
        g.bias.raw_only = fused ? 0 : 1;
    }
    bm::launch_grad(g, h->stream);
    if (fused && h->use_wt) h->wt_valid = true;
}

static void launch_fe(bm_rbm *h, const float *Xin, int ldx, int B, bool with_flip) {
    FeArgs f;
    memset(&f, 0, sizeof(f));
    f.P = make_operand(h->W.p, h->W.ld, h->H);
    f.Q = make_operand(Xin, ldx, B);
    f.K = h->V; f.I = h->H; f.J = B;
    f.hb = h->hb.p;
    f.rowacc = h->rowacc.p;
    if (with_flip) { f.rowacc2 = h->rowacc.p + h->maxB; f.flip_col = h->flip.p; }
    if (h->multinomial()) {
        (void)hipMemsetAsync(h->hhat.p, 0, 3 * (size_t)h->H * sizeof(float), h->stream);
        const int M = h->cfg.n_samples;
        hipLaunchKernelGGL(mn_hhat_kernel, dim3((M + 255) / 256), dim3(256), 0, h->stream, h->hhat.p, h->H, M,
                           make_key(h, SITE_FE, 0), make_key(h, SITE_FE, 1), make_key(h, SITE_FE, 2));
        f.hvec = h->hhat.p;
        f.rowacc3 = h->rowacc.p + 2 * (size_t)h->maxB;
    }
    launch_fe_hidden(f, h->stream);
    FeRowArgs r;
    memset(&r, 0, sizeof(r));
    r.X = Xin; r.ld = ldx; r.V = h->V; r.B = B;
    r.vb = h->vb.p; r.sigma = (h->cfg.v_unit == BM_UNIT_GAUSSIAN) ? h->sigma.p : nullptr;
    r.rowacc = f.rowacc; r.rowacc2 = f.rowacc2; r.rowacc3 = f.rowacc3; r.flip_col = f.flip_col; r.out = h->scal.p + 2;
    hipLaunchKernelGGL(fe_row_kernel, dim3((B + FE_ROWS_PER_WG - 1) / FE_ROWS_PER_WG), dim3(256), 0, h->stream, r);
}

static double mn_fe_const(const bm_rbm *h) {
    if (!h->multinomial()) return 0.0;
    const double M = h->cfg.n_samples, K = h->H;
    return -lgamma(M + K) + lgamma(M + 1.0) + lgamma(K);
}

static void metrics_to_out4(const bm_rbm *h, const double *host, int B, float *out4);
static bool metrics_fused_ok(const bm_rbm *h) {
    static const bool off = bm::dbg("metrics_fused") && atoi(bm::dbg("metrics_fused")) == 0;
    return !off && !h->multinomial() && !h->cfg.dbm_first && !h->fast_now && (h->W.ld & 3) == 0;
}
static void metrics_prep(bm_rbm *h, int B) {
    MetricsPrepArgs mp;
    mp.scal = h->scal.p; mp.rowacc = h->rowacc.p; mp.n_rowacc = 3 * h->maxB; mp.flip = h->flip.p; mp.B = B; mp.V = h->V;
    mp.key = make_key(h, SITE_PLL, 0); mp.row0 = (unsigned long long)h->row0;
    hipLaunchKernelGGL(metrics_prep_kernel, dim3(8), dim3(256), 0, h->stream, mp);
}
static int metrics_from_chain(bm_rbm *h, int B, float *out4) {
    const SqJob msre{h->Xin, h->Xin_ld, h->vm.p, h->vm.ld, B, h->V, h->scal.p + 0};
    const SqJob l2{h->W.p, h->W.ld, nullptr, 0, h->V, h->H, h->scal.p + 1};
    if (h->fe_in_chain) {
        FeRowArgs r;
// ... 258 lines not shown
    auto h = std::make_unique<bm_rbm>();
    h->cfg = *cfg;
    h->V = cfg->n_visible; h->H = cfg->n_hidden; h->maxB = cfg->max_batch;
    const int V = h->V, H = h->H, B = h->maxB;
    BM_HIP(hipGetDevice(&h->device));
    BM_TRY(create(h->stream)); BM_TRY(create(h->ev0)); BM_TRY(create(h->ev1));
    BM_TRY(h->W.alloc(V, H)); BM_TRY(h->dW.alloc(V, H));
    {
        const char *e = bm::dbg("up_xm");
        h->use_wt = !(e && atoi(e) == 0) && (V % 4 == 0) && !h->multinomial();
        if (h->use_wt) BM_TRY(h->Wt.alloc(H, V));
    }
    BM_TRY(h->vb.alloc(V)); BM_TRY(h->hb.alloc(H)); BM_TRY(h->dvb.alloc(V)); BM_TRY(h->dhb.alloc(H));
    BM_TRY(h->q.alloc(H)); BM_TRY(h->sigma.alloc(V));
    BM_TRY(h->h0m.alloc(B, H)); BM_TRY(h->h0s.alloc(B, H)); BM_TRY(h->hm.alloc(B, H)); BM_TRY(h->hs.alloc(B, H)); BM_TRY(h->hneg.alloc(B, H));
    BM_TRY(h->vm.alloc(B, V)); BM_TRY(h->vs.alloc(B, V)); BM_TRY(h->Xs.alloc(B, V)); BM_TRY(h->Xd.alloc(B, V));
    BM_TRY(h->grad.alloc(h->grad_tail() + V + 2 * (size_t)H));
    BM_TRY(h->pen.alloc(H));
    BM_TRY(h->rowacc.alloc(3 * (size_t)B)); BM_TRY(h->hhat.alloc(3 * (size_t)H));
    BM_TRY(h->flip.alloc(B)); BM_TRY(h->scal.alloc(6));
    {
        std::vector<float> ones(V, 1.0f);
        BM_HIP(hipMemcpy(h->sigma.p, ones.data(), V * sizeof(float), hipMemcpyHostToDevice));
    }
    *out = h.release();
    return 0;
}

int bm_rbm_destroy(bm_rbm *h) {
    if (!h) return 0;
    for (hipStream_t st : {h->stream.h, h->comm_stream.h, h->stage_stream.h}) if (st) (void)hipStreamSynchronize(st);
    if (h->xchg_used) xchg_bind_user(h->xchg_used, nullptr);
    delete h;
    return 0;
}

static int check_device_status(bm_rbm *h) {
    if (h->xchg_used) BM_TRY(xchg_check_status(h->xchg_used));
    if (h->chain.status) {
        int st[2] = {0, 0};
        BM_HIP(hipMemcpy(st, h->chain.status, sizeof(st), hipMemcpyDeviceToHost));
        const long long expect = h->chain.tiles_expected & 0xffffffffLL;
        if (st[0] != 0 || (long long)(unsigned)st[1] != expect) {
            h->chain.mode = 0;
            h->chain.tiles_expected = 0;
            BM_HIP(hipMemset(h->chain.status, 0, sizeof(st)));
            BM_CHECK(st[0] == 0, "chained propagation launch failed (status %d: %s); the results since the last check are "
                     "invalid, chained launches are now off for this handle", st[0],
                     st[0] == CHAIN_ERR_TIMEOUT ? "a wait for a producing tile expired" : "not an 8-XCD device");
            BM_CHECK(false, "chained propagation launches computed %u tiles, expected %lld; the results since the last check "
                     "are invalid, chained launches are now off for this handle", (unsigned)st[1], expect);
        }
    }
    return 0;
}

int bm_rbm_sync(bm_rbm *h) {
    BM_HIP(hipStreamSynchronize(h->stream));
    BM_TRY(check_device_status(h));
    if (h->nonbinary.p) {
        int bad = 0;
        BM_HIP(hipMemcpy(&bad, h->nonbinary.p, sizeof(int), hipMemcpyDeviceToHost));
        if (bad) {
            BM_HIP(hipMemset(h->nonbinary.p, 0, sizeof(int)));
            BM_CHECK(false, "fast-binary mode: bm_rbm_gibbs was given hidden states that are not a {0,1} bitmap");
        }
    }
    return 0;
}

int bm_rbm_set_fast_binary(bm_rbm *h, int32_t on) {
    BM_CHECK(h, "null argument");
    h->fast = (on >= 2 || (on == 1 && (long long)h->V * h->H >= (8ll << 20))) ? 1 : 0;
    return 0;
}

static DevBuf *find_vec(bm_rbm *h, const std::string &n) {
    if (n == "vb") return &h->vb;
    if (n == "hb") return &h->hb;
    if (n == "dvb") return &h->dvb;
    if (n == "dhb") return &h->dhb;
    if (n == "q_means") return &h->q;
    if (n == "sigma") return &h->sigma;
    return nullptr;
}

int bm_rbm_set_param(bm_rbm *h, const char *name, const float *host, size_t n) {
    const std::string nm(name ? name : "");
    BM_HIP(hipStreamSynchronize(h->stream));
    if (nm == "W" || nm == "dW") {
        BM_CHECK(n == (size_t)h->V * h->H, "variable '%s' has %zu elements, got %zu", name, (size_t)h->V * h->H, n);
        BM_TRY((nm == "W" ? h->W : h->dW).upload(host));
        if (nm == "W") h->wt_valid = false;
        else { h->dw_sharded = false; if (h->xchg_used) xchg_dw_replaced(h->xchg_used); }
        return 0;
    }
    DevBuf *b = find_vec(h, nm);
    BM_CHECK(b, "unknown RBM variable '%s'", name ? name : "(null)");
    BM_CHECK(n == b->n, "variable '%s' has %zu elements, got %zu", name, b->n, n);
    BM_HIP(hipMemcpy(b->p, host, n * sizeof(float), hipMemcpyHostToDevice));
    return 0;
}

int bm_rbm_set_param_dev(bm_rbm *h, const char *name, const float *src_dev, size_t n) {
    const std::string nm(name ? name : "");
    BM_CHECK(h && src_dev, "null argument");
// ... 97 lines not shown
    if (out_n) *out_n = b->n;
    return 0;
}

int bm_rbm_seed(bm_rbm *h, uint64_t seed) { h->seed = seed; h->call = 0; return 0; }
int bm_rbm_set_row_offset(bm_rbm *h, int64_t row0) { h->row0 = row0; return 0; }

int bm_rbm_train_step(bm_rbm *h, const float *X_dev, int32_t B, float lr, float mom, int32_t k) {
    BM_TRY(check_dw(h, "bm_rbm_train_step"));
    BM_TRY(run_chain(h, X_dev, B, k, nullptr, false, true));
    launch_update_fused(h, B, lr, mom);
    h->call++;
    BM_HIP(hipGetLastError());
    return 0;
}

int bm_rbm_train_step_metrics(bm_rbm *h, const float *X_dev, int32_t B, float lr, float mom, int32_t k,
                              float *out4) {
    BM_TRY(check_dw(h, "bm_rbm_train_step_metrics"));
    BM_TRY(run_chain(h, X_dev, B, k, nullptr, true, false, false, true));
    BM_TRY(metrics_from_chain(h, B, out4));
    launch_update_fused(h, B, lr, mom);
    h->call++;
    BM_HIP(hipGetLastError());
    return 0;
}

int bm_rbm_train_step_metrics_async(bm_rbm *h, const float *X_dev, int32_t B, float lr, float mom, int32_t k) {
    if (!h->mring) {
        Pinned<double> ring;
        BM_TRY(create(ring, (size_t)bm_rbm::MRING * 6));
        BM_TRY(create(h->ev_mlast, hipEventDisableTiming));
        BM_HIP(hipHostGetDevicePointer((void **)&h->mring_dev, ring, 0));
        h->mring_B.resize(bm_rbm::MRING);
        h->mring = std::move(ring);
    }
    BM_CHECK(h->mring_n < bm_rbm::MRING, "%d metric fetches are pending: call bm_rbm_collect_metrics", h->mring_n);
    BM_TRY(check_dw(h, "bm_rbm_train_step_metrics_async"));
    BM_TRY(run_chain(h, X_dev, B, k, nullptr, true, false, false, true));
    BM_TRY(metrics_from_chain(h, B, nullptr));
    hipLaunchKernelGGL(scal_to_host_kernel, dim3(1), dim3(64), 0, h->stream, (const double *)h->scal.p,
                       h->mring_dev + (size_t)h->mring_n * 6);
    BM_HIP(hipEventRecord(h->ev_mlast, h->stream));
    h->mring_B[h->mring_n++] = B;
    launch_update_fused(h, B, lr, mom);
    h->call++;
    BM_HIP(hipGetLastError());
    return 0;
}
int bm_rbm_collect_metrics(bm_rbm *h, float *out4n, int32_t max_n, int32_t *out_n) {
    BM_CHECK(h && out_n && (out4n || max_n == 0), "null argument");
    BM_CHECK(h->mring_n <= max_n, "%d fetches pending, room for %d", h->mring_n, (int)max_n);
    if (h->mring_n > 0 && h->ev_mlast) BM_HIP(hipEventSynchronize(h->ev_mlast));
    if (h->chain.status || h->xchg_used) {
        BM_HIP(hipStreamSynchronize(h->stream));
        const int rc = check_device_status(h);
        if (rc) { h->mring_n = 0; *out_n = 0; return rc; }
    }
    for (int i = 0; i < h->mring_n; ++i) metrics_to_out4(h, h->mring + (size_t)i * 6, h->mring_B[i], out4n + 4 * (size_t)i);
    *out_n = h->mring_n;
    h->mring_n = 0;
    return 0;
}

int bm_rbm_train_epoch(bm_rbm *h, const float *X_dev, int64_t N, int32_t batch, float lr, float mom, int32_t k) {
    BM_CHECK(batch >= 1 && N >= 1, "bad N=%lld batch=%d", (long long)N, batch);
    for (int64_t s = 0; s < N; s += batch) {
        const int B = (int)((N - s < batch) ? (N - s) : batch);
        BM_TRY(bm_rbm_train_step(h, X_dev + (size_t)s * h->V, B, lr, mom, k));
    }
    return 0;
}

int bm_rbm_grad_step(bm_rbm *h, const float *X_dev, int32_t B, int32_t k) {
    BM_TRY(run_chain(h, X_dev, B, k, nullptr, false, false, true));
    rbm_grad(h, B, 0, (float)B, 0.f, 0.f, true);
    h->call++;
    BM_HIP(hipGetLastError());
    return 0;
}

static int ensure_delayed(bm_rbm *h) {
    if (h->comm_stream) return 0;
    BM_TRY(h->grad_alt.alloc(h->grad.n));
    for (int i = 0; i < 2; ++i) {
        BM_TRY(create(h->ev_ready[i], hipEventDisableTiming));
        BM_TRY(create(h->ev_reduced[i], hipEventDisableTiming));
    }
    return create(h->comm_stream);
}
int bm_rbm_set_grad_slot(bm_rbm *h, int32_t slot) {
    BM_CHECK(h && (slot == 0 || slot == 1), "slot must be 0 or 1");
    if (slot == h->grad_slot) return 0;
    BM_TRY(ensure_delayed(h));
    std::swap(h->grad, h->grad_alt);
    h->grad_slot = slot;
    return 0;
}
int bm_rbm_allreduce_grads_async(bm_rbm *h, bm_comm *c) {
    BM_CHECK(h && c, "null argument");
    BM_TRY(ensure_delayed(h));
    const int s = h->grad_slot;
    BM_HIP(hipEventRecord(h->ev_ready[s], h->stream));
    BM_HIP(hipStreamWaitEvent(h->comm_stream, h->ev_ready[s], 0));
    BM_TRY(bm_comm_allreduce_sum(c, h->grad.p, h->grad.n, (void *)h->comm_stream));
    BM_HIP(hipEventRecord(h->ev_reduced[s], h->comm_stream));
    return 0;
// ... 307 lines not shown
    h->pt_step += k;
    h->call++;
    BM_HIP(hipGetLastError());
    return 0;
}

int bm_rbm_train_epoch_pt(bm_rbm *h, const float *X_dev, int64_t N, int32_t batch, float lr, float mom, int32_t k) {
    BM_CHECK(h && X_dev, "null argument");
    BM_CHECK(batch >= 1 && N >= 1, "bad N=%lld batch=%d", (long long)N, batch);
    for (int64_t s = 0; s < N; s += batch) {
        const int B = (int)((N - s < batch) ? (N - s) : batch);
        BM_TRY(bm_rbm_train_step_pt(h, X_dev + (size_t)s * h->V, B, lr, mom, k));
    }
    return 0;
}

int bm_debug_tile_map(int32_t tiles_i, int32_t tiles_j, double bytes_i, double bytes_j, int32_t *out_ti, int32_t *out_tj,
                      int32_t *out_map5) {
    BM_CHECK(tiles_i >= 1 && tiles_j >= 1 && out_ti && out_tj, "bad arguments");
    const TileMap m = make_tile_map(tiles_i, tiles_j, bytes_i, bytes_j);
    const int nb = tiles_i * tiles_j;
    for (int b = 0; b < nb; ++b) { int ti = -1, tj = -1; tile_of_block(m, b, nb, ti, tj); out_ti[b] = ti; out_tj[b] = tj; }
    if (out_map5) { out_map5[0] = m.xi; out_map5[1] = m.xj; out_map5[2] = m.gj; out_map5[3] = m.tiles_i; out_map5[4] = m.tiles_j; }
    return 0;
}

int bm_rbm_stream(bm_rbm *h, void **out_stream) { *out_stream = (void *)h->stream; return 0; }

int bm_rbm_profile(bm_rbm *h, int32_t enable) {
    BM_HIP(hipStreamSynchronize(h->stream));
    h->recs.clear();
    h->prof = enable != 0;
    return 0;
}

int bm_rbm_kernel_times(bm_rbm *h, float *ms6, int32_t *n6) {
    BM_HIP(hipStreamSynchronize(h->stream));
    for (int c = 0; c < BM_NUM_KERNEL_CLASSES; ++c) { ms6[c] = 0.f; n6[c] = 0; }
    for (auto &r : h->recs) {
        float ms = 0.f;
        BM_HIP(hipEventElapsedTime(&ms, r.a, r.b));
        ms6[r.cls] += ms;
        n6[r.cls] += 1;
    }
    return 0;
}

int bm_rbm_chain_stats(bm_rbm *h, int64_t *out3) {
    BM_CHECK(h && out3, "null argument");
    out3[0] = (int64_t)h->chain.launches; out3[1] = (int64_t)h->chain.tiles_expected; out3[2] = (int64_t)chain_mode(h->chain);
    return 0;
}

int bm_rbm_timer_start(bm_rbm *h) { BM_HIP(hipEventRecord(h->ev0, h->stream)); return 0; }
int bm_rbm_timer_mark(bm_rbm *h) { BM_HIP(hipEventRecord(h->ev1, h->stream)); return 0; }
int bm_rbm_timer_elapsed(bm_rbm *h, float *out_ms) {
    BM_HIP(hipEventSynchronize(h->ev1));
    BM_HIP(hipEventElapsedTime(out_ms, h->ev0, h->ev1));
    return 0;
}
int bm_rbm_timer_stop(bm_rbm *h, float *out_ms) {
    BM_HIP(hipEventRecord(h->ev1, h->stream));
    BM_HIP(hipEventSynchronize(h->ev1));
    BM_HIP(hipEventElapsedTime(out_ms, h->ev0, h->ev1));
    return 0;
}

}
```

boltzmann_machines_amd/engine.py:

```python
import ctypes as C

import numpy as np

from . import _ffi
from ._ffi import DeviceArray, check

RBM_VARS = ('W', 'vb', 'hb', 'dW', 'dvb', 'dhb', 'q_means', 'sigma')


def as_device(X):
    if isinstance(X, DeviceArray):
        return X
    return DeviceArray.from_numpy(np.asarray(X), np.float32)


class RbmEngine(object):
    dtype = np.float32

    def __init__(self, n_visible, n_hidden, v_unit=_ffi.UNIT_BERNOULLI, sample_v_states=False,
                 sample_h_states=True, dbm_first=False, dbm_last=False, max_batch=10, l2=1e-4,
                 sparsity_target=0.1, sparsity_cost=0., sparsity_damping=0.9, dropout=None,
                 h_unit=_ffi.UNIT_BERNOULLI, n_samples=0):
        self.lib = _ffi.load()
        self.V, self.H, self.max_batch = int(n_visible), int(n_hidden), int(max_batch)
# ... 120 lines not shown
    def ais(self, n_betas, n_runs, k, seed, chain0=0, base_bias=None):
        out = np.empty(n_runs, dtype=np.float32)
        a = None
        if base_bias is not None:
            a = np.ascontiguousarray(base_bias, dtype=np.float32)
            if a.shape != (self.V,):
                raise ValueError('base_bias has shape %r, expected (%d,)' % (a.shape, self.V))
        check(self.lib.bm_rbm_ais(self._h, n_betas, n_runs, k, a.ctypes.data_as(C.c_void_p) if a is not None else None,
                                  int(seed), int(chain0), out.ctypes.data_as(C.c_void_p)))
        return out

    def gibbs(self, Hd, Vd, B, n_steps):
        check(self.lib.bm_rbm_gibbs(self._h, Hd.ptr, Vd.ptr, B, n_steps))

    def gibbs_clamped(self, Vd, Hd, B, n_steps, clamp_val_d, clamp_mask_d, Vmean_d=None, row=0):
        ov, oh = row * self.V, row * self.H
        check(self.lib.bm_rbm_gibbs_clamped(self._h, Vd.offset_ptr(ov), Hd.offset_ptr(oh),
                                            Vmean_d.offset_ptr(ov) if Vmean_d is not None else None, B, n_steps,
                                            clamp_val_d.offset_ptr(ov), clamp_mask_d.offset_ptr(ov)))

    def pt_init(self, n_chains, betas, V0_d=None, chain0=0):
        b = np.ascontiguousarray(betas, dtype=np.float32).ravel()
        check(self.lib.bm_rbm_pt_init(self._h, int(n_chains), len(b), b.ctypes.data_as(C.c_void_p),
                                      V0_d.ptr if V0_d is not None else None, int(chain0)))
        self._pt_shape = (int(n_chains), len(b))
        self._pt_train_key = None

    def pt_sweep(self, n_steps):
        check(self.lib.bm_rbm_pt_sweep(self._h, int(n_steps)))

    def pt_read(self, Vd=None, Hd=None):
        M, R = getattr(self, '_pt_shape', (0, 1))
        swaps = np.zeros((2, max(R - 1, 0)), dtype=np.int64)
        idx = np.zeros((M, R), dtype=np.int32)
        check(self.lib.bm_rbm_pt_read(self._h, Vd.ptr if Vd is not None else None, Hd.ptr if Hd is not None else None,
                                      swaps.ctypes.data_as(C.c_void_p) if swaps.size else None,
                                      idx.ctypes.data_as(C.c_void_p) if idx.size else None))
        return swaps, idx

    def train_step_pt(self, Xd, B, lr, momentum, k, row=0):
        check(self.lib.bm_rbm_train_step_pt(self._h, Xd.offset_ptr(row * self.V), B, lr, momentum, k))

    def train_epoch_pt(self, Xd, N, batch, lr, momentum, k, row=0):
        check(self.lib.bm_rbm_train_epoch_pt(self._h, Xd.offset_ptr(row * self.V), N, batch, lr, momentum, k))

    def stream(self):
        p = C.c_void_p()
        check(self.lib.bm_rbm_stream(self._h, C.byref(p)))
        return p.value

    def chain_stats(self):
        out = (C.c_int64 * 3)()
        check(self.lib.bm_rbm_chain_stats(self._h, out))
        return int(out[0]), int(out[1]), int(out[2])

    def profile(self, enable):
        check(self.lib.bm_rbm_profile(self._h, int(bool(enable))))

    def kernel_times(self):
        ms, n = (C.c_float * 6)(), (C.c_int32 * 6)()
        check(self.lib.bm_rbm_kernel_times(self._h, ms, n))
        names = ('act_up', 'act_down', 'grad', 'colsum', 'bias', 'other')
        return {k: (float(ms[i]), int(n[i])) for i, k in enumerate(names)}

    def timer_start(self):
        check(self.lib.bm_rbm_timer_start(self._h))

    def timer_stop(self):
        ms = C.c_float()
        check(self.lib.bm_rbm_timer_stop(self._h, C.byref(ms)))
        return float(ms.value)

    def timer_mark(self):
        check(self.lib.bm_rbm_timer_mark(self._h))

    def timer_elapsed(self):
        ms = C.c_float()
        check(self.lib.bm_rbm_timer_elapsed(self._h, C.byref(ms)))
        return float(ms.value)


class RbmEngine64(object):

    dtype = np.float64

    def __init__(self, n_visible, n_hidden, v_unit=_ffi.UNIT_BERNOULLI, sample_v_states=False,
                 sample_h_states=True, dbm_first=False, dbm_last=False, max_batch=10, l2=1e-4,
                 sparsity_target=0.1, sparsity_cost=0., sparsity_damping=0.9, dropout=None,
                 h_unit=_ffi.UNIT_BERNOULLI, n_samples=0):
        self.lib = _ffi.load()
        self.V, self.H, self.max_batch = int(n_visible), int(n_hidden), int(max_batch)
        drop = -1.0 if dropout is None else float(dropout)
        cfg = _ffi.RbmConfig(self.V, self.H, int(v_unit), int(bool(sample_v_states)),
                             int(bool(sample_h_states)), int(bool(dbm_first)), int(bool(dbm_last)),
                             self.max_batch, float(l2), float(sparsity_target), float(sparsity_cost),
                             float(sparsity_damping), drop, int(h_unit), int(n_samples))
        hyper = (C.c_double * 5)(float(l2), float(sparsity_target), float(sparsity_cost), float(sparsity_damping), drop)
        self._h = C.c_void_p()
        check(self.lib.bm_rbm64_create(C.byref(cfg), hyper, C.byref(self._h)))

    def close(self):
        if getattr(self, '_h', None) is not None and self._h:
            self.lib.bm_rbm64_destroy(self._h)
            self._h = None

    def __del__(self):
# ... 347 lines not shown
```

include/bm355.h:

```cpp
#ifndef BM355_H
#define BM355_H

#include <stddef.h>
#include <stdint.h>

#ifdef __cplusplus
extern "C" {
#endif

const char *bm_last_error(void);
const char *bm_version(void);
int bm_device_count(void);
int bm_set_device(int device);

int bm_dev_alloc(size_t bytes, void **out_dev);
int bm_dev_free(void *dev);
int bm_h2d(void *dst_dev, const void *src_host, size_t bytes);
int bm_d2h(void *dst_host, const void *src_dev, size_t bytes);
int bm_dev_memset(void *dst_dev, int value, size_t bytes);

int bm_debug_tile_map(int32_t tiles_i, int32_t tiles_j, double bytes_i, double bytes_j, int32_t *out_ti,
                      int32_t *out_tj, int32_t *out_map5);

typedef struct bm_rbm bm_rbm;
// ... 26 lines not shown
int bm_rbm_set_param_dev(bm_rbm *h, const char *name, const float *src_dev, size_t n);
int bm_rbm_get_param(bm_rbm *h, const char *name, float *host, size_t n);
int bm_rbm_dev_ptr(bm_rbm *h, const char *name, void **out_dev, size_t *out_n);

int bm_rbm_seed(bm_rbm *h, uint64_t seed);
int bm_rbm_set_row_offset(bm_rbm *h, int64_t row0);

int bm_rbm_train_step(bm_rbm *h, const float *X_dev, int32_t B,
                      float learning_rate, float momentum, int32_t n_gibbs_steps);
int bm_rbm_train_step_metrics(bm_rbm *h, const float *X_dev, int32_t B,
                              float learning_rate, float momentum, int32_t n_gibbs_steps,
                              float *out4);
int bm_rbm_train_step_metrics_async(bm_rbm *h, const float *X_dev, int32_t B,
                                    float learning_rate, float momentum, int32_t n_gibbs_steps);
int bm_rbm_collect_metrics(bm_rbm *h, float *out4n, int32_t max_n, int32_t *out_n);
int bm_rbm_train_epoch(bm_rbm *h, const float *X_dev, int64_t N, int32_t batch,
                       float learning_rate, float momentum, int32_t n_gibbs_steps);

int bm_rbm_stage(bm_rbm *h, int32_t slot);
int bm_rbm_get_staged(bm_rbm *h, int32_t slot, const char *name, float *host, size_t n);

int bm_rbm_grad_step(bm_rbm *h, const float *X_dev, int32_t B_local, int32_t n_gibbs_steps);
int bm_rbm_apply_step(bm_rbm *h, int32_t B_global, float learning_rate, float momentum);

int bm_rbm_transform(bm_rbm *h, const float *X_dev, int32_t B, int32_t n_gibbs_steps,
                     float *H_dev);

int bm_rbm_metrics(bm_rbm *h, const float *X_dev, int32_t B, int32_t n_gibbs_steps,
                   float *out4);
int bm_rbm_free_energy(bm_rbm *h, const float *X_dev, int32_t B, float *out1);
int bm_rbm_free_energy_rows(bm_rbm *h, const float *X_dev, int32_t B, float *out_host);
int bm_rbm_ais(bm_rbm *h, int32_t n_betas, int32_t n_runs, int32_t n_gibbs_steps, const float *base_bias_host,
               uint64_t seed, int64_t chain0, float *values_host);

int bm_rbm_gibbs(bm_rbm *h, float *H_dev, float *V_dev, int32_t B, int32_t n_steps);

int bm_rbm_gibbs_clamped(bm_rbm *h, float *V_dev, float *H_dev, float *Vmean_dev, int32_t B, int32_t n_steps,
                         const float *clamp_val_dev, const float *clamp_mask_dev);

int bm_rbm_pt_init(bm_rbm *h, int32_t n_chains, int32_t n_temps, const float *betas_host, const float *V0_dev, int64_t chain0);
int bm_rbm_pt_sweep(bm_rbm *h, int32_t n_steps);
int bm_rbm_pt_read(bm_rbm *h, float *V_dev, float *H_dev, int64_t *swaps_host, int32_t *ladder_idx_host);

int bm_rbm_train_step_pt(bm_rbm *h, const float *X_dev, int32_t B, float lr, float mom, int32_t n_gibbs_steps);
int bm_rbm_train_epoch_pt(bm_rbm *h, const float *X_dev, int64_t N, int32_t batch, float lr, float mom, int32_t n_gibbs_steps);

int bm_rbm_stream(bm_rbm *h, void **out_stream);

#define BM_NUM_KERNEL_CLASSES 6
int bm_rbm_profile(bm_rbm *h, int32_t enable);
int bm_rbm_kernel_times(bm_rbm *h, float *ms6, int32_t *n6);

int bm_rbm_chain_stats(bm_rbm *h, int64_t *out3);

int bm_rbm_timer_start(bm_rbm *h);
int bm_rbm_timer_stop(bm_rbm *h, float *out_ms);
int bm_rbm_timer_mark(bm_rbm *h);
int bm_rbm_timer_elapsed(bm_rbm *h, float *out_ms);

typedef struct bm_rbm64 bm_rbm64;
int bm_rbm64_create(const bm_rbm_config *cfg, const double *hyper5, bm_rbm64 **out);
int bm_rbm64_destroy(bm_rbm64 *h);
int bm_rbm64_sync(bm_rbm64 *h);
int bm_rbm64_seed(bm_rbm64 *h, uint64_t seed);
int bm_rbm64_set_row_offset(bm_rbm64 *h, int64_t row0);
int bm_rbm64_set_param(bm_rbm64 *h, const char *name, const double *host, size_t n);
int bm_rbm64_get_param(bm_rbm64 *h, const char *name, double *host, size_t n);
int bm_rbm64_train_step(bm_rbm64 *h, const double *X_dev, int32_t B,
                        double learning_rate, double momentum, int32_t n_gibbs_steps);
int bm_rbm64_train_step_metrics(bm_rbm64 *h, const double *X_dev, int32_t B,
                                double learning_rate, double momentum, int32_t n_gibbs_steps, double *out4);
int bm_rbm64_transform(bm_rbm64 *h, const double *X_dev, int32_t B, int32_t n_gibbs_steps,
                       double *H_dev);
int bm_rbm64_metrics(bm_rbm64 *h, const double *X_dev, int32_t B, int32_t n_gibbs_steps,
                     double *out4);
int bm_rbm64_free_energy(bm_rbm64 *h, const double *X_dev, int32_t B, double *out1);


typedef struct bm_dbm bm_dbm;

#define BM_DBM_MAX_LAYERS 4

typedef struct bm_dbm_config {
    int32_t n_layers;
    int32_t n_visible;
    int32_t n_hiddens[BM_DBM_MAX_LAYERS];
    int32_t v_unit;
    int32_t sample_v_states;
    int32_t sample_h_states[BM_DBM_MAX_LAYERS];
    int32_t n_particles;
    int32_t batch_size;
    int32_t max_mf_updates;
    float   mf_tol;
    float   l2;
    float   max_norm;
    float   sparsity_target[BM_DBM_MAX_LAYERS];
    float   sparsity_cost[BM_DBM_MAX_LAYERS];
    float   sparsity_damping;
    int32_t h_unit[BM_DBM_MAX_LAYERS];
    int32_t n_samples[BM_DBM_MAX_LAYERS];
} bm_dbm_config;

int bm_dbm_create(const bm_dbm_config *cfg, bm_dbm **out);
int bm_dbm_destroy(bm_dbm *h);
int bm_dbm_sync(bm_dbm *h);
int bm_dbm_seed(bm_dbm *h, uint64_t seed);
// ... 102 lines not shown
```

Baseline: 15870.

## Fuse final hidden-up, gradient and bias into one persistent tail kernel

Adds a persistent tail kernel that claims work items through an atomic counter and runs the last up-pass tiles, the gradient GEMM tiles and the bias column sums in one launch. Gradient and bias items wait on per-tile generation flags instead of kernel boundaries, and read the freshly written negative means through system-coherent loads and write-through stores. The goal is to remove launch gaps and tail idle time between dependent stages at the end of each CD step. In exchange it adds spin-waiting, coherence-bypassing memory traffic and extra flag and claim bookkeeping, and it is enabled only on gfx950 when the legality and size rules hold.

```diff
diff --git a/boltzmann_machines_amd/_ffi.py b/boltzmann_machines_amd/_ffi.py
--- a/boltzmann_machines_amd/_ffi.py
+++ b/boltzmann_machines_amd/_ffi.py
@@ -143,6 +143,7 @@
     'bm_rbm_profile': [_vp, _i32],
     'bm_rbm_kernel_times': [_vp, _fp, _ip],
     'bm_rbm_chain_stats': [_vp, C.POINTER(C.c_int64)],
+    'bm_rbm_tail_stats': [_vp, C.POINTER(C.c_int64)],
     'bm_rbm_timer_start': [_vp],
     'bm_rbm_timer_stop': [_vp, _fp],
     'bm_rbm_timer_mark': [_vp],
diff --git a/boltzmann_machines_amd/csrc/bm_gemm.h b/boltzmann_machines_amd/csrc/bm_gemm.h
--- a/boltzmann_machines_amd/csrc/bm_gemm.h
+++ b/boltzmann_machines_amd/csrc/bm_gemm.h
@@ -10,6 +10,7 @@
     static constexpr bool kFinalSync = true;
     static constexpr bool kSplitFill = false, kCohQ = false;
     static constexpr bool kCanAbort = false;
+    static constexpr bool kWaitSeg2 = false, kCohP2 = false;
     __device__ __forceinline__ void wait_inputs() {}
     __device__ __forceinline__ void post_fill() {}
     __device__ __forceinline__ void fill() {}
@@ -106,15 +107,18 @@
     return v;
 }
 
+template <int COH = 1>
 __device__ __forceinline__ float4 load4_coh(const float *p) {
     const unsigned long long *q = reinterpret_cast<const unsigned long long *>(p);
-    const unsigned long long a = __hip_atomic_load(q, __ATOMIC_RELAXED, __HIP_MEMORY_SCOPE_AGENT);
-    const unsigned long long b = __hip_atomic_load(q + 1, __ATOMIC_RELAXED, __HIP_MEMORY_SCOPE_AGENT);
+    const unsigned long long a = (COH == 2) ? __hip_atomic_load(q, __ATOMIC_RELAXED, __HIP_MEMORY_SCOPE_SYSTEM)
+                                            : __hip_atomic_load(q, __ATOMIC_RELAXED, __HIP_MEMORY_SCOPE_AGENT);
+    const unsigned long long b = (COH == 2) ? __hip_atomic_load(q + 1, __ATOMIC_RELAXED, __HIP_MEMORY_SCOPE_SYSTEM)
+                                            : __hip_atomic_load(q + 1, __ATOMIC_RELAXED, __HIP_MEMORY_SCOPE_AGENT);
     return make_float4(__uint_as_float((unsigned)a), __uint_as_float((unsigned)(a >> 32)),
                        __uint_as_float((unsigned)b), __uint_as_float((unsigned)(b >> 32)));
 }
 
-template <int L, int TX, int BK, int NTH, bool FAST, bool COH = false>
+template <int L, int TX, int BK, int NTH, bool FAST, int COH = 0>
 __device__ __forceinline__ void g2r(float4 (&reg)[TX * BK / (4 * NTH)], const float *ptr, int ld, int nx, int vec,
                                     int x0, int k0, int K, int tid) {
     static_assert(!COH || FAST, "coherent register path: 16-byte-legal operands only");
@@ -130,7 +134,7 @@
             const int kc = (L == KM) ? min(k, K - 1) : min(k, K - 4);
             const int xc = (L == KM) ? min(x, nx - 4) : min(x, nx - 1);
             const float *pc = (L == KM) ? ptr + (size_t)kc * ld + xc : ptr + (size_t)xc * ld + kc;
-            reg[n] = COH ? load4_coh(pc) : *reinterpret_cast<const float4 *>(pc);
+            if constexpr (COH != 0) reg[n] = load4_coh<COH>(pc); else reg[n] = *reinterpret_cast<const float4 *>(pc);
         } else if (L == KM) {
             reg[n] = load4_guard(ptr + (size_t)k * ld + x, k < K, x, nx, vec);
         } else {
@@ -327,10 +331,26 @@
     asm volatile("s_mov_b32 m0, %2\n\ts_nop 0\n\tglobal_load_lds_dwordx4 %1, %0 sc1"
                  :: "s"(sbase), "v"(voff), "s"(lds_byte) : "memory");
 }
-template <class G, int DW, bool QSC = false, bool QHALF = false>
-__device__ __forceinline__ void dma_chunk_s(const DmaPlan<G, DW> &pl, const char *pb, const char *qb, unsigned ldsP, unsigned ldsQ) {
-#pragma unroll
-    for (int n = 0; n < DmaPlan<G, DW>::NPP; ++n) dma16s(pb, pl.p[n], ldsP + (unsigned)(n * DW * 1024));
+__device__ __forceinline__ void dma16s_sys(const void *sbase, uint32_t voff, unsigned lds_byte) {
+    asm volatile("s_mov_b32 m0, %2\n\ts_nop 0\n\tglobal_load_lds_dwordx4 %1, %0 sc0 sc1"
+                 :: "s"(sbase), "v"(voff), "s"(lds_byte) : "memory");
+}
+__device__ __forceinline__ void dma16_sys(const char *src, float *lds_dst) {
+    unsigned keep;
+    const unsigned lds_addr = (unsigned)(uintptr_t)(__attribute__((address_space(3))) void *)lds_dst;
+    asm volatile("s_mov_b32 %0, m0\n\ts_mov_b32 m0, %2\n\ts_nop 0\n\tglobal_load_lds_dwordx4 %1, off sc0 sc1\n\ts_mov_b32 m0, %0"
+                 : "=&s"(keep) : "v"(src), "s"(__builtin_amdgcn_readfirstlane(lds_addr)) : "memory");
+}
+template <class G, int DW, bool QSC = false, bool QHALF = false, bool PSC2 = false>
+__device__ __forceinline__ void dma_chunk_s(const DmaPlan<G, DW> &pl, const char *pb, const char *qb, unsigned ldsP, unsigned ldsQ,
+                                            bool psys = false) {
+    if (PSC2 && psys) {
+#pragma unroll
+        for (int n = 0; n < DmaPlan<G, DW>::NPP; ++n) dma16s_sys(pb, pl.p[n], ldsP + (unsigned)(n * DW * 1024));
+    } else {
+#pragma unroll
+        for (int n = 0; n < DmaPlan<G, DW>::NPP; ++n) dma16s(pb, pl.p[n], ldsP + (unsigned)(n * DW * 1024));
+    }
 #pragma unroll
     for (int n = 0; n < DmaPlan<G, DW>::NPQ; ++n) {
         if (QHALF && (n & 1)) continue;
@@ -339,7 +359,7 @@
     }
 }
 
-template <int QL, class G, bool SEG2, int PL = KM, int DW = G::NW, bool QHALF = false>
+template <int QL, class G, bool SEG2, int PL = KM, int DW = G::NW, bool QHALF = false, bool PSC2 = false>
 __device__ __forceinline__ void dma_chunk(const KRange &kr, const DmaPlan<G, DW> &pl1, const DmaPlan<G, DW> &pl2, int nch1, int c,
                                           float *sP, float *sQ, int wave) {
     constexpr int BK = G::BK;
@@ -355,7 +375,8 @@
     for (int n = 0; n < DmaPlan<G, DW>::NPP; ++n) {
         const uint32_t o1 = pl1.p[n], o2 = SEG2 ? pl2.p[n] : 0u;
         const uint32_t o = SEG2 ? (o1 ^ ((o1 ^ o2) & (uint32_t)m)) : o1;
-        dma16(pb + o, sP + (wave + n * DW) * 256);
+        if (PSC2 && m) dma16_sys(pb + o, sP + (wave + n * DW) * 256);
+        else           dma16(pb + o, sP + (wave + n * DW) * 256);
     }
 #pragma unroll
     for (int n = 0; n < DmaPlan<G, DW>::NPQ; ++n) {
@@ -366,19 +387,22 @@
     }
 }
 
-template <int QL, class G, bool FAST, bool SEG2, int PL = KM, bool COHQ = false>
+template <int QL, class G, bool FAST, bool SEG2, int PL = KM, bool COHQ = false, bool COHP2 = false>
 __device__ __forceinline__ void load_chunk(ChunkRegs<G> &r, const KRange &kr, int nch1, int i0, int j0, int c, int tid) {
     constexpr int BK = G::BK;
     if (!SEG2) {
         g2r<PL, G::TI, BK, G::NT, FAST>(r.p, kr.P1.ptr, kr.P1.ld, kr.P1.nx, kr.P1.vec, i0, c * BK, kr.K1, tid);
-        g2r<QL, G::TJ, BK, G::NT, FAST, COHQ>(r.q, kr.Q1.ptr, kr.Q1.ld, kr.Q1.nx, kr.Q1.vec, j0, c * BK, kr.K1, tid);
+        g2r<QL, G::TJ, BK, G::NT, FAST, COHQ ? 1 : 0>(r.q, kr.Q1.ptr, kr.Q1.ld, kr.Q1.nx, kr.Q1.vec, j0, c * BK, kr.K1, tid);
     } else {
         const int m = -(int)((c >= nch1) & (kr.K2 > 0));
         const int kc = c - (nch1 & m);
         const int K = sel_i(kr.K1, kr.K2, m);
-        g2r<PL, G::TI, BK, G::NT, FAST>(r.p, sel_p(kr.P1.ptr, kr.P2.ptr, m), sel_i(kr.P1.ld, kr.P2.ld, m),
-                                        sel_i(kr.P1.nx, kr.P2.nx, m), sel_i(kr.P1.vec, kr.P2.vec, m), i0, kc * BK, K, tid);
-        g2r<QL, G::TJ, BK, G::NT, FAST, COHQ>(r.q, sel_p(kr.Q1.ptr, kr.Q2.ptr, m), sel_i(kr.Q1.ld, kr.Q2.ld, m),
+        if (COHP2 && m)
+            g2r<PL, G::TI, BK, G::NT, FAST, COHP2 ? 2 : 0>(r.p, kr.P2.ptr, kr.P2.ld, kr.P2.nx, kr.P2.vec, i0, kc * BK, K, tid);
+        else
+            g2r<PL, G::TI, BK, G::NT, FAST>(r.p, sel_p(kr.P1.ptr, kr.P2.ptr, m), sel_i(kr.P1.ld, kr.P2.ld, m),
+                                            sel_i(kr.P1.nx, kr.P2.nx, m), sel_i(kr.P1.vec, kr.P2.vec, m), i0, kc * BK, K, tid);
+        g2r<QL, G::TJ, BK, G::NT, FAST, COHQ ? 1 : 0>(r.q, sel_p(kr.Q1.ptr, kr.Q2.ptr, m), sel_i(kr.Q1.ld, kr.Q2.ld, m),
                                               sel_i(kr.Q1.nx, kr.Q2.nx, m), sel_i(kr.Q1.vec, kr.Q2.vec, m), j0, kc * BK, K, tid);
     }
 }
@@ -493,6 +517,13 @@
     RegPlan<G> rp1, rp2;
     const bool dmaw = (DW == G::NW) || w < DW;
     ChunkRegs<G> g0, g1;
+    static_assert(!(Side::kWaitSeg2 && SEG2) || (FAST && STG == STG_DMA), "segment-2 wait: 16-byte operands, DMA staging");
+    bool waited2 = false;
+    auto seg2_gate = [&](int c) {
+        if constexpr (Side::kWaitSeg2 && SEG2) {
+            if (!waited2 && c >= nch1) { side.wait_inputs(); waited2 = true; }
+        }
+    };
     if (FAST && STG != STG_REG && dmaw) {
         make_plan<QL, G, PL, DW>(pl1, kr.P1, kr.Q1, i0, j0, w, lane);
         if (SEG2) make_plan<QL, G, PL, DW>(pl2, kr.P2, kr.Q2, i0, j0, w, lane);
@@ -544,15 +575,18 @@
     } else {
 #pragma unroll
         for (int c = 0; c < PF; ++c)
-            if (c < nch && is_dma(c) && dmaw && !BM_ABL(0))
-                dma_chunk<QL, G, SEG2, PL, DW, (BM_ABL(9) != 0)>(kr, pl1, pl2, nch1, c, sP + (c % NBUF) * P_BUF, sQ + (c % NBUF) * Q_BUF, w);
+            if (c < nch && is_dma(c) && !BM_ABL(0)) {
+                seg2_gate(c);
+                if (dmaw) dma_chunk<QL, G, SEG2, PL, DW, (BM_ABL(9) != 0), Side::kCohP2>(kr, pl1, pl2, nch1, c, sP + (c % NBUF) * P_BUF, sQ + (c % NBUF) * Q_BUF, w);
+            }
         __builtin_amdgcn_sched_barrier(0);
         side.fill();
         __builtin_amdgcn_sched_barrier(0);
 #pragma unroll
         for (int c = 0; c < 2; ++c)
             if (c < nch && !is_dma(c) && !BM_ABL(0)) {
-                load_chunk<QL, G, FAST, SEG2, PL>(gr, kr, nch1, i0, j0, c, tid);
+                seg2_gate(c);
+                load_chunk<QL, G, FAST, SEG2, PL, false, Side::kCohP2>(gr, kr, nch1, i0, j0, c, tid);
                 store_chunk<QL, G, SEG2, PL>(gr, kr, nch1, c, sP + (c % NBUF) * P_BUF, sQ + (c % NBUF) * Q_BUF, tid);
             }
         {
@@ -607,11 +641,11 @@
     };
 #define BM_DMA_AT(CD, SD)                                                                         \
     {                                                                                             \
-        if (SEG2 && !in2 && (CD) >= nch1) { in2 = true; pl1 = pl2; }                              \
+        if (SEG2 && !in2 && (CD) >= nch1) { seg2_gate(CD); in2 = true; pl1 = pl2; }               \
         const char *pb_, *qb_;                                                                    \
         chunk_bases((CD), pb_, qb_);                                                              \
-        if (dmaw) dma_chunk_s<G, DW, Side::kCohQ, (BM_ABL(9) != 0)>(pl1, pb_, qb_, ldsPw + (unsigned)((SD) * P_BUF * 4), \
-                                     ldsQw + (unsigned)((SD) * Q_BUF * 4));                       \
+        if (dmaw) dma_chunk_s<G, DW, Side::kCohQ, (BM_ABL(9) != 0), Side::kCohP2>(pl1, pb_, qb_, ldsPw + (unsigned)((SD) * P_BUF * 4), \
+                                     ldsQw + (unsigned)((SD) * Q_BUF * 4), in2);                  \
     }
 #define BM_STEP_Q(FC, FN, S)                                                                      \
     {                                                                                             \
@@ -629,7 +663,7 @@
         const bool do_dma = cd < nch && is_dma(cd) && !BM_ABL(0);                                 \
         const bool do_reg = cr < nch && !is_dma(cr) && !BM_ABL(0);                                \
         if (cc == last - 1) side.drain();       \
-        if (do_reg) load_chunk<QL, G, FAST, SEG2, PL, Side::kCohQ>(gr, kr, nch1, i0, j0, cr, tid); \
+        if (do_reg) { seg2_gate(cr); load_chunk<QL, G, FAST, SEG2, PL, Side::kCohQ, Side::kCohP2>(gr, kr, nch1, i0, j0, cr, tid); } \
         if (do_dma) BM_DMA_AT(cd, S3)                                                             \
         read_frags<QL, G, ABL, PL>(FN, sP + (S1) * P_BUF, sQ + (S1) * Q_BUF, wi, wj, lane);       \
         mfma_frags<G, ABL>(acc, FC);                                                              \
diff --git a/boltzmann_machines_amd/csrc/bm_kernels.h b/boltzmann_machines_amd/csrc/bm_kernels.h
--- a/boltzmann_machines_amd/csrc/bm_kernels.h
+++ b/boltzmann_machines_amd/csrc/bm_kernels.h
@@ -138,6 +138,17 @@
     }
 }
 
+__device__ __forceinline__ void store4_wt(float *dst, size_t o, const float *v, int nvalid, bool v4) {
+    if (v4) {
+        const f32x4 t = {v[0], v[1], v[2], v[3]};
+        asm volatile("global_store_dwordx4 %0, %1, off sc0 sc1\n\ts_nop 1" :: "v"(dst + o), "v"(t) : "memory");
+    } else {
+#pragma unroll
+        for (int r = 0; r < 4; ++r)
+            if (r < nvalid) __hip_atomic_store(reinterpret_cast<unsigned *>(dst + o + r), __float_as_uint(v[r]), __ATOMIC_RELAXED, __HIP_MEMORY_SCOPE_SYSTEM);
+    }
+}
+
 template <int MI> struct PhiloxFor { typedef PhiloxPair type; };
 template <> struct PhiloxFor<1> { typedef PhiloxOne type; };
 
@@ -156,7 +167,9 @@
 template <int E, class Rng, bool MF = false, int NTH = 256> struct ActSide {
     static constexpr bool kFinalSync = false;
     static constexpr bool kSplitFill = false, kCohQ = false, kCanAbort = MF;
+    static constexpr bool kWaitSeg2 = false, kCohP2 = false;
     static constexpr bool kMF = MF;
+    static constexpr bool kWtNeg = false;
     const float *bias, *sigma;
     const float *prev_row;
     int ib0, I, with_rng;
@@ -361,7 +374,8 @@
                 float nm[4];
 #pragma unroll
                 for (int r = 0; r < 4; ++r) nm[r] = -m[r];
-                store4<HWMATH>(a.negmeans, o, nm, nvalid, v4 && (((uintptr_t)a.negmeans & 15u) == 0));
+                if constexpr (SideT::kWtNeg) store4_wt(a.negmeans, o, nm, nvalid, v4 && (((uintptr_t)a.negmeans & 15u) == 0));
+                else store4<HWMATH>(a.negmeans, o, nm, nvalid, v4 && (((uintptr_t)a.negmeans & 15u) == 0));
             }
             if (a.states) store4<HWMATH>(a.states, o, s, nvalid, v4 && (((uintptr_t)a.states & 15u) == 0));
             if constexpr (RT) {
@@ -584,6 +598,7 @@
 constexpr int CS_NV = CS_ROWS * 16 / NT;
 struct ColRegs { float4 a[CS_NV], b[CS_NV]; };
 
+template <bool COHB = false>
 __device__ __forceinline__ void cs_fetch(ColRegs &r, const float *A, int lda, const float *Bm, int ldb,
                                          int c0, int ncols, int nrows, int r0, int tid) {
     const int c4 = tid & 15;
@@ -592,7 +607,8 @@
     for (int n = 0; n < CS_NV; ++n) {
         const int rc = min(r0 + (tid >> 4) + 16 * n, nrows - 1);
         r.a[n] = *reinterpret_cast<const float4 *>(A + (size_t)rc * lda + cc);
-        r.b[n] = Bm ? *reinterpret_cast<const float4 *>(Bm + (size_t)rc * ldb + cc) : make_float4(0.f, 0.f, 0.f, 0.f);
+        if constexpr (COHB) r.b[n] = load4_coh<2>(Bm + (size_t)rc * ldb + cc);
+        else r.b[n] = Bm ? *reinterpret_cast<const float4 *>(Bm + (size_t)rc * ldb + cc) : make_float4(0.f, 0.f, 0.f, 0.f);
     }
 }
 
@@ -610,6 +626,7 @@
     }
 }
 
+template <bool COHB = false>
 __device__ __forceinline__ void block_colsum(const float *A, int lda, const float *Bm, int ldb,
                                              int c0, int ncols, int nrows, bool want2,
                                              float *smem, f32x4 &sum1, f32x4 &sum2, bool negB = false) {
@@ -621,7 +638,7 @@
     const bool vec = (((uintptr_t)A & 15u) == 0) && ((lda & 3) == 0) && ((ncols & 3) == 0) &&
                      (!Bm || ((((uintptr_t)Bm & 15u) == 0) && ((ldb & 3) == 0)));
     ColRegs regs;
-    if (vec) cs_fetch(regs, A, lda, Bm, ldb, c0, ncols, nrows, 0, tid);
+    if (vec) cs_fetch<COHB>(regs, A, lda, Bm, ldb, c0, ncols, nrows, 0, tid);
     for (int r0 = 0; r0 < nrows; r0 += CS_ROWS) {
         const int nr = (nrows - r0 < CS_ROWS) ? nrows - r0 : CS_ROWS;
         if (vec) {
@@ -631,11 +648,15 @@
                 const int row = e >> 6, cc = e & 63, c = c0 + cc;
                 const bool ok = row < nr && c < ncols;
                 sA[row * CS_LD + cc] = ok ? A[(size_t)(r0 + row) * lda + c] : 0.f;
-                sB[row * CS_LD + cc] = (ok && Bm) ? Bm[(size_t)(r0 + row) * ldb + c] : 0.f;
+                if constexpr (COHB)
+                    sB[row * CS_LD + cc] = ok ? __uint_as_float(__hip_atomic_load(reinterpret_cast<const unsigned *>(Bm + (size_t)(r0 + row) * ldb + c),
+                                                                                  __ATOMIC_RELAXED, __HIP_MEMORY_SCOPE_SYSTEM)) : 0.f;
+                else
+                    sB[row * CS_LD + cc] = (ok && Bm) ? Bm[(size_t)(r0 + row) * ldb + c] : 0.f;
             }
         }
         wg_barrier();
-        if (vec) cs_fetch(regs, A, lda, Bm, ldb, c0, ncols, nrows, r0 + CS_ROWS, tid);
+        if (vec) cs_fetch<COHB>(regs, A, lda, Bm, ldb, c0, ncols, nrows, r0 + CS_ROWS, tid);
         const int nsteps = (((nr + 3) / 4) + 7) & ~7;
         const int co = w * 16 + l15;
         for (int s = 0; s < nsteps; s += 8) {
@@ -711,6 +732,7 @@
     int raw_only;
     RbmBiasArgs u;
 };
+template <bool COHH = false>
 __device__ __forceinline__ void rbm_bias_fused_block(const RbmBiasFusedArgs &a, int wv, float *smem) {
     const int lane = threadIdx.x & 63, w = threadIdx.x >> 6, g = lane >> 4;
     const int nv = (a.u.V + 63) / 64;
@@ -734,7 +756,7 @@
         }
     } else {
         const int c0 = (wv - nv) * 64;
-        block_colsum(a.h0m, a.ldh0, a.hm, a.ldh, c0, a.u.H, a.B, true, smem, s1, s2, a.hm_negated != 0);
+        block_colsum<COHH>(a.h0m, a.ldh0, a.hm, a.ldh, c0, a.u.H, a.B, true, smem, s1, s2, a.hm_negated != 0);
         if ((lane & 15) == 0) {
 #pragma unroll
             for (int r = 0; r < 4; ++r) {
@@ -811,6 +833,7 @@
 template <int NJ> struct GradSide {
     static constexpr bool kFinalSync = true;
     static constexpr bool kSplitFill = false, kCohQ = false, kCanAbort = false;
+    static constexpr bool kWaitSeg2 = false, kCohP2 = false;
     const float *W, *dW; int ldw, I, J, ib0, jb[NJ]; bool on, vec8;
     float4 w[NJ][2], d[NJ][2];
     bool at_fill;
@@ -840,10 +863,121 @@
     }
 };
 
+template <class G, bool FAST, int ABL, int STG, class SideT>
+__device__ __forceinline__ void grad_tile(const GradArgs &a, int ti, int tj, float *smem, SideT &side) {
+    constexpr int TI = G::TI, NJ = G::NJ, TJ2 = G::TJ;
+    static_assert(G::MI == 2 && G::TI == 64 && G::TJ == 64, "grad_kernel: 64 x 64 tiles, 8 consecutive outputs per lane");
+    const int i0 = ti * TI, j0 = tj * TJ2;
+    const int tid = threadIdx.x, lane = tid & 63, w = tid >> 6;
+    const int wi = w % G::WI, wj = w / G::WI;
+    const int g = lane >> 4, l15 = lane & 15;
+    const int ib0 = i0 + wi * 32 + g * 8;
+
+#ifdef BM_PROBE
+#define BM_GSTAMP(n) do { if (a.dbg && threadIdx.x == 0) a.dbg[blockIdx.x * 4 + (n)] = (long long)__builtin_readcyclecounter(); } while (0)
+#else
+#define BM_GSTAMP(n) do {} while (0)
+#endif
+    BM_GSTAMP(0);
+    f32x4 pos[2][NJ], neg[2][NJ];
+#pragma unroll
+    for (int t = 0; t < 2; ++t)
+#pragma unroll
+        for (int n = 0; n < NJ; ++n) pos[t][n] = neg[t][n] = (f32x4){0.f, 0.f, 0.f, 0.f};
+    side.W = a.W; side.dW = a.dW; side.ldw = a.ldw; side.I = a.I; side.J = a.J; side.ib0 = ib0;
+#pragma unroll
+    for (int n = 0; n < NJ; ++n) side.jb[n] = j0 + wj * (16 * NJ) + lane_j<KM, G>(l15, n);
+    side.vec8 = (ib0 + 7 < a.I) && ((a.ldw & 3) == 0);
+    side.at_fill = true;
+    side.on = a.fused != 0 && a.fetch_at_fill != 0;
+    KRange kr;
+    kr.P1 = a.Ppos; kr.Q1 = a.Qpos; kr.K1 = a.Kpos;
+    if (SideT::kWaitSeg2 || a.form == 0) {
+        kr.P2 = a.Pneg; kr.Q2 = a.Qneg; kr.K2 = a.Kneg;
+        mainloop<KM, G, FAST, true, ABL, KM, STG>(pos, kr, i0, j0, smem, side);
+    } else {
+        kr.P2 = a.Ppos; kr.Q2 = a.Qpos; kr.K2 = 0;
+        mainloop<KM, G, FAST, false, 0, KM, STG>(pos, kr, i0, j0, smem, side);
+        kr.P1 = a.Pneg; kr.Q1 = a.Qneg; kr.K1 = a.Kneg;
+        mainloop<KM, G, FAST, false, 0, KM, STG>(neg, kr, i0, j0, smem, side);
+    }
+
+    BM_GSTAMP(1);
+    if (ib0 >= a.I) return;
+    if (!a.fetch_at_fill) { side.on = a.fused != 0; side.fetch(); }
+    const DivBy divN(a.N), divM(a.M);
+    float wt[NJ][8];
+    bool jok[NJ];
+#pragma unroll
+    for (int n = 0; n < NJ; ++n) {
+        const int j = side.jb[n];
+        jok[n] = j < a.J;
+        if (!jok[n]) continue;
+        float pv[8], nv[8];
+        lane_outputs<G>(pos, n, pv);
+        lane_outputs<G>(neg, n, nv);
+        const size_t o = (size_t)j * a.ldw + ib0;
+        if (!a.fused) {
+#pragma unroll
+            for (int e = 0; e < 8; ++e) {
+                if (ib0 + e >= a.I) break;
+                a.raw[o + e] = pv[e];
+                if (a.form != 0) a.raw2[o + e] = nv[e];
+            }
+            continue;
+        }
+        float wv[8] = {side.w[n][0].x, side.w[n][0].y, side.w[n][0].z, side.w[n][0].w, side.w[n][1].x, side.w[n][1].y, side.w[n][1].z, side.w[n][1].w};
+        float dv[8] = {side.d[n][0].x, side.d[n][0].y, side.d[n][0].z, side.d[n][0].w, side.d[n][1].x, side.d[n][1].y, side.d[n][1].z, side.d[n][1].w};
+        float pe[8];
+#pragma unroll
+        for (int e = 0; e < 8; ++e) pe[e] = (a.pen && ib0 + e < a.I) ? a.pen[ib0 + e] : 0.f;
+        float gr[8];
+        if (divN.pow2 && divM.pow2) {
+#pragma unroll
+            for (int e = 0; e < 8; ++e) gr[e] = (a.form == 0) ? grad_norm1(pv[e], a.N, divN.inv, true)
+                                                              : grad_norm2(pv[e], nv[e], a.N, a.M, divN.inv, divM.inv, true);
+        } else {
+#pragma unroll
+            for (int e = 0; e < 8; ++e) gr[e] = (a.form == 0) ? grad_norm1(pv[e], a.N, 0.f, false)
+                                                              : grad_norm2(pv[e], nv[e], a.N, a.M, 0.f, 0.f, false);
+        }
+#pragma unroll
+        for (int e = 0; e < 8; ++e) {
+            apply_w_update(gr[e], pe[e], a.l2, a.lr, a.mom, wv[e], dv[e]);
+            wt[n][e] = wv[e];
+        }
+        if (side.vec8) {
+            stream_store4(a.W + o, wv[0], wv[1], wv[2], wv[3]);
+            stream_store4(a.W + o + 4, wv[4], wv[5], wv[6], wv[7]);
+            stream_store4(a.dW + o, dv[0], dv[1], dv[2], dv[3]);
+            stream_store4(a.dW + o + 4, dv[4], dv[5], dv[6], dv[7]);
+        } else {
+#pragma unroll
+            for (int e = 0; e < 8; ++e)
+                if (ib0 + e < a.I) { a.W[o + e] = wv[e]; a.dW[o + e] = dv[e]; }
+        }
+    }
+    if (a.fused && a.Wt) {
+        const int ja = side.jb[0];
+        const bool pair = NJ == 2 && jok[0] && jok[NJ - 1] && ((a.ldwt & 1) == 0);
+#pragma unroll
+        for (int e = 0; e < 8; ++e) {
+            if (ib0 + e >= a.I) break;
+            float *dst = a.Wt + (size_t)(ib0 + e) * a.ldwt + ja;
+            if (pair) {
+                stream_store2(dst, wt[0][e], wt[NJ - 1][e]);
+            } else {
+                if (jok[0]) dst[0] = wt[0][e];
+                if (NJ == 2 && jok[NJ - 1]) dst[1] = wt[NJ - 1][e];
+            }
+        }
+    }
+    BM_GSTAMP(2);
+}
+
 template <class G, bool FAST, int ABL = 0, int STG = STG_DMA, int MINB = 1>
 __global__ __launch_bounds__(G::NT, MINB) void grad_kernel(GradArgs a, TileMap tmap) {
-    constexpr int TI = G::TI, NJ = G::NJ;
-    static_assert(G::MI == 2 && G::TI == 64 && G::TJ == 64, "grad_kernel: 64 x 64 tiles, 8 consecutive outputs per lane");
+    constexpr int NJ = G::NJ;
     __shared__ __attribute__((aligned(16))) float smem[G::SMEM_FLOATS];
     constexpr bool kBias = G::SMEM_FLOATS >= CS_SMEM_FLOATS;
     static_assert(G::NT >= NT, "bias path");
@@ -866,113 +1000,8 @@
         TILE_WORDS(tmap, (int)blockIdx.x);
         TILE_OF_BLOCK(tmap, (int)blockIdx.x, ntile_blocks, ti, tj);
     }
-    const int i0 = ti * TI, j0 = tj * TJ2;
-    const int tid = threadIdx.x, lane = tid & 63, w = tid >> 6;
-    const int wi = w % G::WI, wj = w / G::WI;
-    const int g = lane >> 4, l15 = lane & 15;
-    const int ib0 = i0 + wi * 32 + g * 8;
-
-#ifdef BM_PROBE
-#define BM_GSTAMP(n) do { if (a.dbg && threadIdx.x == 0) a.dbg[blockIdx.x * 4 + (n)] = (long long)__builtin_readcyclecounter(); } while (0)
-#else
-#define BM_GSTAMP(n) do {} while (0)
-#endif
-    BM_GSTAMP(0);
-    f32x4 pos[2][NJ], neg[2][NJ];
-#pragma unroll
-    for (int t = 0; t < 2; ++t)
-#pragma unroll
-        for (int n = 0; n < NJ; ++n) pos[t][n] = neg[t][n] = (f32x4){0.f, 0.f, 0.f, 0.f};
     GradSide<NJ> side;
-    side.W = a.W; side.dW = a.dW; side.ldw = a.ldw; side.I = a.I; side.J = a.J; side.ib0 = ib0;
-#pragma unroll
-    for (int n = 0; n < NJ; ++n) side.jb[n] = j0 + wj * (16 * NJ) + lane_j<KM, G>(l15, n);
-    side.vec8 = (ib0 + 7 < a.I) && ((a.ldw & 3) == 0);
-    side.at_fill = true;
-    side.on = a.fused != 0 && a.fetch_at_fill != 0;
-    KRange kr;
-    kr.P1 = a.Ppos; kr.Q1 = a.Qpos; kr.K1 = a.Kpos;
-    if (a.form == 0) {
-        kr.P2 = a.Pneg; kr.Q2 = a.Qneg; kr.K2 = a.Kneg;
-        mainloop<KM, G, FAST, true, ABL, KM, STG>(pos, kr, i0, j0, smem, side);
-    } else {
-        kr.P2 = a.Ppos; kr.Q2 = a.Qpos; kr.K2 = 0;
-        mainloop<KM, G, FAST, false, 0, KM, STG>(pos, kr, i0, j0, smem, side);
-        kr.P1 = a.Pneg; kr.Q1 = a.Qneg; kr.K1 = a.Kneg;
-        mainloop<KM, G, FAST, false, 0, KM, STG>(neg, kr, i0, j0, smem, side);
-    }
-
-    BM_GSTAMP(1);
-    if (ib0 >= a.I) return;
-    if (!a.fetch_at_fill) { side.on = a.fused != 0; side.fetch(); }
-    const DivBy divN(a.N), divM(a.M);
-    float wt[NJ][8];
-    bool jok[NJ];
-#pragma unroll
-    for (int n = 0; n < NJ; ++n) {
-        const int j = side.jb[n];
-        jok[n] = j < a.J;
-        if (!jok[n]) continue;
-        float pv[8], nv[8];
-        lane_outputs<G>(pos, n, pv);
-        lane_outputs<G>(neg, n, nv);
-        const size_t o = (size_t)j * a.ldw + ib0;
-        if (!a.fused) {
-#pragma unroll
-            for (int e = 0; e < 8; ++e) {
-                if (ib0 + e >= a.I) break;
-                a.raw[o + e] = pv[e];
-                if (a.form != 0) a.raw2[o + e] = nv[e];
-            }
-            continue;
-        }
-        float wv[8] = {side.w[n][0].x, side.w[n][0].y, side.w[n][0].z, side.w[n][0].w, side.w[n][1].x, side.w[n][1].y, side.w[n][1].z, side.w[n][1].w};
-        float dv[8] = {side.d[n][0].x, side.d[n][0].y, side.d[n][0].z, side.d[n][0].w, side.d[n][1].x, side.d[n][1].y, side.d[n][1].z, side.d[n][1].w};
-        float pe[8];
-#pragma unroll
-        for (int e = 0; e < 8; ++e) pe[e] = (a.pen && ib0 + e < a.I) ? a.pen[ib0 + e] : 0.f;
-        float gr[8];
-        if (divN.pow2 && divM.pow2) {
-#pragma unroll
-            for (int e = 0; e < 8; ++e) gr[e] = (a.form == 0) ? grad_norm1(pv[e], a.N, divN.inv, true)
-                                                              : grad_norm2(pv[e], nv[e], a.N, a.M, divN.inv, divM.inv, true);
-        } else {
-#pragma unroll
-            for (int e = 0; e < 8; ++e) gr[e] = (a.form == 0) ? grad_norm1(pv[e], a.N, 0.f, false)
-                                                              : grad_norm2(pv[e], nv[e], a.N, a.M, 0.f, 0.f, false);
-        }
-#pragma unroll
-        for (int e = 0; e < 8; ++e) {
-            apply_w_update(gr[e], pe[e], a.l2, a.lr, a.mom, wv[e], dv[e]);
-            wt[n][e] = wv[e];
-        }
-        if (side.vec8) {
-            stream_store4(a.W + o, wv[0], wv[1], wv[2], wv[3]);
-            stream_store4(a.W + o + 4, wv[4], wv[5], wv[6], wv[7]);
-            stream_store4(a.dW + o, dv[0], dv[1], dv[2], dv[3]);
-            stream_store4(a.dW + o + 4, dv[4], dv[5], dv[6], dv[7]);
-        } else {
-#pragma unroll
-            for (int e = 0; e < 8; ++e)
-                if (ib0 + e < a.I) { a.W[o + e] = wv[e]; a.dW[o + e] = dv[e]; }
-        }
-    }
-    if (a.fused && a.Wt) {
-        const int ja = side.jb[0];
-        const bool pair = NJ == 2 && jok[0] && jok[NJ - 1] && ((a.ldwt & 1) == 0);
-#pragma unroll
-        for (int e = 0; e < 8; ++e) {
-            if (ib0 + e >= a.I) break;
-            float *dst = a.Wt + (size_t)(ib0 + e) * a.ldwt + ja;
-            if (pair) {
-                stream_store2(dst, wt[0][e], wt[NJ - 1][e]);
-            } else {
-                if (jok[0]) dst[0] = wt[0][e];
-                if (NJ == 2 && jok[NJ - 1]) dst[1] = wt[NJ - 1][e];
-            }
-        }
-    }
-    BM_GSTAMP(2);
+    grad_tile<G, FAST, ABL, STG>(a, ti, tj, smem, side);
 }
 
 struct ApplyWArgs {
diff --git a/boltzmann_machines_amd/csrc/bm_launch.h b/boltzmann_machines_amd/csrc/bm_launch.h
--- a/boltzmann_machines_amd/csrc/bm_launch.h
+++ b/boltzmann_machines_amd/csrc/bm_launch.h
@@ -373,6 +373,11 @@
     launch_grad_as(T.geo, g, st);
 }
 
+static inline bool tail_rule(int n_up, int n_grad, int ncu) {
+    (void)n_up; (void)n_grad; (void)ncu;
+    return false;
+}
+
 static inline void launch_fe_hidden(const FeArgs &f, hipStream_t st) {
     const bool fast = operand_fast(f.P, KM, f.K) && operand_fast(f.Q, XM, f.K);
     const dim3 grid(tile_grid<GeoAct>(f.I, f.J)), blk(NT);
diff --git a/boltzmann_machines_amd/csrc/bm_rbm.hip b/boltzmann_machines_amd/csrc/bm_rbm.hip
--- a/boltzmann_machines_amd/csrc/bm_rbm.hip
+++ b/boltzmann_machines_amd/csrc/bm_rbm.hip
@@ -2,6 +2,7 @@
 #include "bm_common.h"
 #include "bm_kernels.h"
 #include "bm_chain.h"
+#include "bm_tail.h"
 #include "bm_pt.h"
 
 #include <math.h>
@@ -99,6 +100,9 @@
     std::vector<Rec> recs;
     size_t grad_tail() const { return (size_t)V * W.ld; }
     ChainState chain;
+    TailState tail;
+    bool tail_defer = false, tail_pending = false;
+    ActArgs tail_up;
 };
 
 enum { KC_UP = 0, KC_DOWN = 1, KC_GRAD = 2, KC_COLSUM = 3, KC_BIAS = 4, KC_OTHER = 5 };
@@ -198,10 +202,16 @@
         hipLaunchKernelGGL(softmax_multinomial_kernel, dim3(B), dim3(64), 2 * (size_t)h->H * sizeof(float), h->stream, m);
         return;
     }
-    if (h->use_wt && h->wt_valid && !(h->fast_now && v == h->vs.p)) {
-        const Operand wt = make_operand(h->Wt.p, h->Wt.ld, h->H);
-        act_pass(h, a, &wt);
-    } else act_pass(h, a);
+    const bool xm = h->use_wt && h->wt_valid && !(h->fast_now && v == h->vs.p);
+    const Operand wt = make_operand(h->Wt.p, h->Wt.ld, h->H);
+    if (h->tail_defer) {
+        if (xm) { a.P1 = wt; a.p_xm = 1; }
+        h->tail_up = a;
+        h->tail_pending = true;
+        return;
+    }
+    if (xm) act_pass(h, a, &wt);
+    else act_pass(h, a);
 }
 
 static void launch_down(bm_rbm *h, const float *hs, int ldh, int B, float *means, float *states, int ldo,
@@ -267,8 +277,11 @@
         const bool last_out = hm_out && last;
         const bool neg_only = last && !hm_out && !need_vm && !h->multinomial();
         h->hm_is_neg = neg_only;
+        h->tail_defer = neg_only && for_update && !h->prof && !h->fast_now && h->cfg.sparsity_cost == 0.f &&
+                        operand_fast(make_operand(Xin, ldx, h->V), KM, B) && (h->H & 3) == 0 && tail_wanted(h->tail, h->H, h->V, B);
         launch_up(h, h->vs.p, h->vs.ld, B, last_out ? hm_out : (neg_only ? nullptr : h->hm.p), last ? nullptr : h->hs.p,
                   last_out ? h->H : h->hm.ld, h->cfg.sample_h_states, SITE_H, t, (!hm_out && last) ? h->hneg.p : nullptr);
+        h->tail_defer = false;
         hstate = h->hs.p;
     }
     BM_TRY(chain_end(h));
@@ -341,6 +354,16 @@
     if (with_bias) {
         g.nbias = fill_bias_fused(h, B, lr, mom, g.bias);
         g.bias.raw_only = fused ? 0 : 1;
+    }
+    if (h->tail_pending) {
+        h->tail_pending = false;
+        const int rc = tail_launch(h->tail, h->tail_up, g, h->stream);
+        if (rc < 0) { (void)hipGetLastError(); h->tail.mode = 0; }
+        if (rc != 0) launch_act(h->tail_up, h->stream);
+        else {
+            if (fused && h->use_wt) h->wt_valid = true;
+            return;
+        }
     }
     bm::launch_grad(g, h->stream);
     if (fused && h->use_wt) h->wt_valid = true;
@@ -705,6 +728,20 @@
                      "are invalid, chained launches are now off for this handle", (unsigned)st[1], expect);
         }
     }
+    if (h->tail.status) {
+        int st[2] = {0, 0};
+        BM_HIP(hipMemcpy(st, h->tail.status, sizeof(st), hipMemcpyDeviceToHost));
+        const long long expect = h->tail.items_expected & 0xffffffffLL;
+        if (st[0] != 0 || (long long)(unsigned)st[1] != expect) {
+            h->tail.mode = 0;
+            h->tail.items_expected = 0;
+            BM_HIP(hipMemset(h->tail.status, 0, sizeof(st)));
+            BM_CHECK(st[0] == 0, "fused tail launch failed (status %d: a wait for a prop-up tile expired); the results since the last "
+                     "check are invalid, the fused tail launch is now off for this handle", st[0]);
+            BM_CHECK(false, "fused tail launches computed %u items, expected %lld; the results since the last check are invalid, "
+                     "the fused tail launch is now off for this handle", (unsigned)st[1], expect);
+        }
+    }
     return 0;
 }
 
@@ -908,7 +945,7 @@
     BM_CHECK(h && out_n && (out4n || max_n == 0), "null argument");
     BM_CHECK(h->mring_n <= max_n, "%d fetches pending, room for %d", h->mring_n, (int)max_n);
     if (h->mring_n > 0 && h->ev_mlast) BM_HIP(hipEventSynchronize(h->ev_mlast));
-    if (h->chain.status || h->xchg_used) {
+    if (h->chain.status || h->tail.status || h->xchg_used) {
         BM_HIP(hipStreamSynchronize(h->stream));
         const int rc = check_device_status(h);
         if (rc) { h->mring_n = 0; *out_n = 0; return rc; }
@@ -1322,6 +1359,12 @@
     return 0;
 }
 
+int bm_rbm_tail_stats(bm_rbm *h, int64_t *out3) {
+    BM_CHECK(h && out3, "null argument");
+    out3[0] = (int64_t)h->tail.launches; out3[1] = (int64_t)h->tail.items_expected; out3[2] = (int64_t)tail_mode(h->tail);
+    return 0;
+}
+
 int bm_rbm_timer_start(bm_rbm *h) { BM_HIP(hipEventRecord(h->ev0, h->stream)); return 0; }
 int bm_rbm_timer_mark(bm_rbm *h) { BM_HIP(hipEventRecord(h->ev1, h->stream)); return 0; }
 int bm_rbm_timer_elapsed(bm_rbm *h, float *out_ms) {
diff --git a/boltzmann_machines_amd/csrc/bm_tail.h b/boltzmann_machines_amd/csrc/bm_tail.h
--- /dev/null
+++ b/boltzmann_machines_amd/csrc/bm_tail.h
@@ -0,0 +1,250 @@
+#pragma once
+#include "bm_chain.h"
+
+namespace bm {
+
+using GeoTailUp = GeoAct8;
+using GeoTailGrad = GeoGrad8;
+static_assert(GeoTailUp::NT == GeoTailGrad::NT && GeoTailUp::SMEM_FLOATS <= GeoTailGrad::SMEM_FLOATS, "one workgroup shape, one ring");
+static_assert(GeoTailGrad::SMEM_FLOATS >= CS_SMEM_FLOATS && GeoTailGrad::NT >= NT, "the bias blocks reuse the ring");
+
+struct TailArgs {
+    ActArgs up;
+    GradArgs g;
+    int up_tiles_j, grad_tiles_j;
+    unsigned n_up, n_grad, n_bias;
+    unsigned gen;
+    unsigned *flags;
+    unsigned *claim;
+    unsigned *claim_zero;
+    int *status;
+    long long *stamps;
+};
+static_assert(sizeof(TailArgs) <= 4096, "kernel arguments");
+
+__device__ __forceinline__ void tail_wait(const unsigned *flags, int n, unsigned gen, int *status) {
+    if ((threadIdx.x >> 6) == 0) {
+        const int lane = threadIdx.x & 63;
+        unsigned spins = 0;
+        for (;;) {
+            bool ok = true;
+            for (int f = lane; f < n; f += 64)
+                ok = ok && (__hip_atomic_load(flags + f, __ATOMIC_RELAXED, __HIP_MEMORY_SCOPE_AGENT) == gen);
+            if (__all(ok)) break;
+            __builtin_amdgcn_s_sleep(1);
+            if ((++spins & 1023u) == 0) {
+                const int st = __hip_atomic_load(status, __ATOMIC_RELAXED, __HIP_MEMORY_SCOPE_AGENT);
+                if (st || spins > (1u << 21)) {
+                    if (lane == 0 && !st) atomicExch(status, CHAIN_ERR_TIMEOUT);
+                    break;
+                }
+            }
+        }
+    }
+    wg_barrier();
+}
+
+struct TailUpSide : ActSide<GeoTailUp::E, typename PhiloxFor<GeoTailUp::MI>::type> {
+    static constexpr bool kWtNeg = true;
+};
+
+struct TailGradSide : GradSide<GeoTailGrad::NJ> {
+    static constexpr bool kWaitSeg2 = true, kCohP2 = true;
+    const unsigned *flags; int nflags; unsigned gen; int *status;
+    long long *stamp;
+    __device__ __forceinline__ void wait_inputs() {
+        if (stamp && threadIdx.x == 0) stamp[0] = wall_clock64();
+        tail_wait(flags, nflags, gen, status);
+        if (stamp && threadIdx.x == 0) stamp[1] = wall_clock64();
+    }
+};
+
+__device__ __forceinline__ void tail_slab(int n, int nb, int tiles_j, int &ti, int &tj) {
+    const int q = nb >> 3, r = nb & 7, x = n & 7;
+    const int t = (x < r ? x * (q + 1) : r * (q + 1) + (x - r) * q) + (n >> 3);
+    ti = small_div(t, tiles_j); tj = t - ti * tiles_j;
+}
+
+template <int PL>
+__device__ __forceinline__ void tail_up_tile(const ActArgs &a, int i0, int j0, float *smem, unsigned *claim, unsigned &nxt, long long *stp) {
+    using G = GeoTailUp;
+    constexpr int E = G::E;
+    const int tid = threadIdx.x, lane = tid & 63, w = tid >> 6;
+    const int wi = w % G::WI, wj = w / G::WI;
+    const int g = lane >> 4, l15 = lane & 15;
+    const int ib0 = i0 + wi * (16 * G::MI) + g * E;
+    const int j = j0 + wj * 16 + l15;
+    KRange kr;
+    kr.P1 = a.P1; kr.Q1 = a.Q1; kr.K1 = a.K1;
+    kr.P2 = a.P2; kr.Q2 = a.Q2; kr.K2 = 0;
+    TailUpSide side;
+    side.bias = a.bias; side.sigma = a.sigma; side.ib0 = ib0; side.I = a.I; side.with_rng = a.sample;
+    side.prev_row = nullptr;
+    const PhiloxKey key = a.key;
+    side.rng.init(key, ((unsigned long long)(a.row0 + j) * (unsigned long long)a.I + ib0) >> 2);
+    f32x4 acc[G::MI][1];
+#pragma unroll
+    for (int t = 0; t < G::MI; ++t) acc[t][0] = (f32x4){0.f, 0.f, 0.f, 0.f};
+    mainloop<XM, G, true, false, 0, PL, STG_DMA>(acc, kr, i0, j0, smem, side);
+    if (tid == 0) nxt = __hip_atomic_fetch_add(claim, 1u, __ATOMIC_RELAXED, __HIP_MEMORY_SCOPE_AGENT);
+    if (stp && tid == 0) stp[3] = wall_clock64();
+    (void)act_epilogue<G, 0>(a, key, acc, side, i0, j0);
+}
+
+__global__ __launch_bounds__(GeoTailGrad::NT, 1) void tail_kernel(TailArgs c) {
+    __shared__ __attribute__((aligned(16))) float smem[GeoTailGrad::SMEM_FLOATS];
+    __shared__ unsigned s_claim;
+    const int tid = threadIdx.x;
+    if (blockIdx.x == 0 && tid == 0) *c.claim_zero = 0u;
+    if (tid == 0) s_claim = __hip_atomic_fetch_add(c.claim, 1u, __ATOMIC_RELAXED, __HIP_MEMORY_SCOPE_AGENT);
+    __syncthreads();
+    unsigned n = s_claim;
+    const unsigned total = c.n_up + c.n_grad + c.n_bias;
+    int nitems = 0;
+    while (n < total) {
+        long long *stp = (c.stamps && blockIdx.x < 256) ? c.stamps + ((size_t)blockIdx.x * 8 + (nitems < 7 ? nitems : 7)) * 8 : nullptr;
+        if (stp && tid == 0) { stp[0] = wall_clock64(); stp[6] = (long long)n; }
+        unsigned nxt = 0;
+        if (n < c.n_up) {
+            int ti, tj;
+            tail_slab((int)n, (int)c.n_up, c.up_tiles_j, ti, tj);
+            if (c.up.p_xm) tail_up_tile<XM>(c.up, ti * GeoTailUp::TI, tj * GeoTailUp::TJ, smem, c.claim, nxt, stp);
+            else           tail_up_tile<KM>(c.up, ti * GeoTailUp::TI, tj * GeoTailUp::TJ, smem, c.claim, nxt, stp);
+            asm volatile("s_waitcnt vmcnt(0)" ::: "memory");
+            if (tid == 0) s_claim = nxt;
+            wg_barrier();
+            if (tid == 0) __hip_atomic_store(c.flags + n, c.gen, __ATOMIC_RELAXED, __HIP_MEMORY_SCOPE_AGENT);
+        } else {
+            if (tid == 0) nxt = __hip_atomic_fetch_add(c.claim, 1u, __ATOMIC_RELAXED, __HIP_MEMORY_SCOPE_AGENT);
+            if (n < c.n_up + c.n_grad) {
+                int ti, tj;
+                tail_slab((int)(n - c.n_up), (int)c.n_grad, c.grad_tiles_j, ti, tj);
+                TailGradSide side;
+                side.flags = c.flags; side.nflags = (int)c.n_up; side.gen = c.gen; side.status = c.status;
+                side.stamp = stp ? stp + 1 : nullptr;
+                grad_tile<GeoTailGrad, true, 0, STG_DMA>(c.g, ti, tj, smem, side);
+            } else {
+                if (tid >= NT) return;
+                const int wv = (int)(n - c.n_up - c.n_grad);
+                if (wv >= (c.g.bias.u.V + 63) / 64) tail_wait(c.flags, (int)c.n_up, c.gen, c.status);
+                rbm_bias_fused_block<true>(c.g.bias, wv, smem);
+            }
+            if (tid == 0) s_claim = nxt;
+            wg_barrier();
+        }
+        if (stp && tid == 0) stp[4] = wall_clock64();
+        n = s_claim;
+        ++nitems;
+    }
+    if (tid == 0 && nitems) atomicAdd(c.status + 1, nitems);
+}
+
+struct TailState {
+    unsigned *flags = nullptr, *claim = nullptr;
+    int *status = nullptr;
+    unsigned flags_cap = 0;
+    unsigned gen = 0;
+    unsigned launches = 0;
+    long long items_expected = 0;
+    int mode = -1;
+    long long *stamps = nullptr;
+    static constexpr int CLAIM_SLOTS = 16;
+    static constexpr size_t STAMP_WORDS = 256 * 8 * 8;
+    static constexpr unsigned MAX_UP = 1u << 14;
+    TailState() = default;
+    TailState(const TailState &) = delete;
+    TailState &operator=(const TailState &) = delete;
+    ~TailState() { release(); }
+    void release() {
+        if (stamps) {
+            const char *f = bm::dbg("tail_stamps");
+            std::vector<long long> hst(STAMP_WORDS);
+            if (f && hipMemcpy(hst.data(), stamps, STAMP_WORDS * 8, hipMemcpyDeviceToHost) == hipSuccess) {
+                FILE *fp = fopen(f, "wb");
+                if (fp) { fwrite(hst.data(), 8, STAMP_WORDS, fp); fclose(fp); }
+            }
+            (void)hipFree(stamps); stamps = nullptr;
+        }
+        if (flags) (void)hipFree(flags);
+        if (claim) (void)hipFree(claim);
+        if (status) (void)hipFree(status);
+        flags = claim = nullptr; status = nullptr;
+    }
+};
+
+static inline int tail_mode(TailState &ts) {
+    if (ts.mode < 0) {
+        const char *e = bm::dbg("tail");
+        ts.mode = e ? atoi(e) : 1;
+        hipDeviceProp_t pr; int d = 0; (void)hipGetDevice(&d);
+        if (!(hipGetDeviceProperties(&pr, d) == hipSuccess && strncmp(pr.gcnArchName, "gfx950", 6) == 0)) ts.mode = 0;
+    }
+    return ts.mode;
+}
+
+static inline bool tail_wanted(TailState &ts, int H, int V, int B) {
+    if (tail_mode(ts) <= 0) return false;
+    const int n_up = tile_grid<GeoTailUp>(H, B), n_grad = tile_grid<GeoTailGrad>(H, V);
+    if ((unsigned)n_up > TailState::MAX_UP) return false;
+    return ts.mode >= 2 || tail_rule(n_up, n_grad, device_cu_count());
+}
+
+static inline bool tail_legal(const ActArgs &a, const GradArgs &g) {
+    if (a.K2 > 0 || a.b3.K1 > 0 || a.prev || a.maxdiff || a.maxdiff_blk || a.rowacc || a.rowdot_out || a.acc_init ||
+        a.skip || a.chk_ctl || a.states16 || a.dot_mat || a.fe_flip || a.clamp_mask || a.row_mult || a.lit) return false;
+    if (a.kind != 0 || a.sample || a.means || a.states || !a.negmeans) return false;
+    if (!(operand_fast(a.P1, a.p_xm ? XM : KM, a.K1) && operand_fast(a.Q1, XM, a.K1))) return false;
+    if (g.form != 0 || !g.fused || g.pen || g.nbias <= 0 || g.bias.raw_only) return false;
+    if (!(operand_fast(g.Ppos, KM, g.Kpos) && operand_fast(g.Qpos, KM, g.Kpos) &&
+          operand_fast(g.Pneg, KM, g.Kneg) && operand_fast(g.Qneg, KM, g.Kneg))) return false;
+    if (g.Pneg.ptr != a.negmeans || !g.bias.hm_negated || g.bias.hm != a.negmeans) return false;
+    return (unsigned)tile_grid<GeoTailUp>(a.I, a.J) <= TailState::MAX_UP;
+}
+
+static inline int tail_launch(TailState &ts, const ActArgs &up, const GradArgs &g_in, hipStream_t st) {
+    if (tail_mode(ts) <= 0 || !tail_legal(up, g_in)) return 1;
+    const int ncu = device_cu_count();
+    TailArgs c;
+    memset(&c, 0, sizeof(c));
+    c.up = up; c.g = g_in;
+    c.g.fetch_at_fill = std::max(0, dbg_int("grad_fetch"));
+    c.up_tiles_j = (up.J + GeoTailUp::TJ - 1) / GeoTailUp::TJ;
+    c.grad_tiles_j = (g_in.J + GeoTailGrad::TJ - 1) / GeoTailGrad::TJ;
+    c.n_up = (unsigned)tile_grid<GeoTailUp>(up.I, up.J);
+    c.n_grad = (unsigned)tile_grid<GeoTailGrad>(g_in.I, g_in.J);
+    c.n_bias = (unsigned)g_in.nbias;
+    if (!ts.flags || c.n_up > ts.flags_cap) {
+        if (ts.flags) { if (hipStreamSynchronize(st) != hipSuccess) return -1; (void)hipFree(ts.flags); ts.flags = nullptr; }
+        const unsigned cap = std::max(c.n_up, 1024u);
+        if (hipMalloc((void **)&ts.flags, (size_t)cap * 4) != hipSuccess) return -1;
+        if (hipMemsetAsync(ts.flags, 0, (size_t)cap * 4, st) != hipSuccess) return -1;
+        ts.flags_cap = cap;
+        ts.gen = 0;
+        if (!ts.claim) {
+            if (hipMalloc((void **)&ts.claim, (size_t)TailState::CLAIM_SLOTS * 32 * 4) != hipSuccess) return -1;
+            if (hipMemsetAsync(ts.claim, 0, (size_t)TailState::CLAIM_SLOTS * 32 * 4, st) != hipSuccess) return -1;
+            if (hipMalloc((void **)&ts.status, 2 * sizeof(int)) != hipSuccess) return -1;
+            if (hipMemsetAsync(ts.status, 0, 2 * sizeof(int), st) != hipSuccess) return -1;
+        }
+    }
+    if (++ts.gen == 0) {
+        if (hipMemsetAsync(ts.flags, 0, (size_t)ts.flags_cap * 4, st) != hipSuccess) return -1;
+        ts.gen = 1;
+    }
+    c.gen = ts.gen;
+    c.flags = ts.flags;
+    c.claim = ts.claim + (size_t)(ts.launches % TailState::CLAIM_SLOTS) * 32;
+    c.claim_zero = ts.claim + (size_t)((ts.launches + TailState::CLAIM_SLOTS / 2) % TailState::CLAIM_SLOTS) * 32;
+    ++ts.launches;
+    c.status = ts.status;
+    const unsigned total = c.n_up + c.n_grad + c.n_bias;
+    ts.items_expected += (long long)total;
+    if (bm::dbg("tail_stamps") && !ts.stamps && hipMalloc((void **)&ts.stamps, TailState::STAMP_WORDS * 8) != hipSuccess) ts.stamps = nullptr;
+    if (ts.stamps) (void)hipMemsetAsync(ts.stamps, 0, TailState::STAMP_WORDS * 8, st);
+    c.stamps = ts.stamps;
+    const int grid = (int)std::min<unsigned>((unsigned)ncu, total);
+    hipLaunchKernelGGL(tail_kernel, dim3(grid), dim3(GeoTailGrad::NT), 0, st, c);
+    return 0;
+}
+
+}
diff --git a/boltzmann_machines_amd/engine.py b/boltzmann_machines_amd/engine.py
--- a/boltzmann_machines_amd/engine.py
+++ b/boltzmann_machines_amd/engine.py
@@ -196,6 +196,11 @@
     def chain_stats(self):
         out = (C.c_int64 * 3)()
         check(self.lib.bm_rbm_chain_stats(self._h, out))
+        return int(out[0]), int(out[1]), int(out[2])
+
+    def tail_stats(self):
+        out = (C.c_int64 * 3)()
+        check(self.lib.bm_rbm_tail_stats(self._h, out))
         return int(out[0]), int(out[1]), int(out[2])
 
     def profile(self, enable):
diff --git a/include/bm355.h b/include/bm355.h
--- a/include/bm355.h
+++ b/include/bm355.h
@@ -102,6 +102,8 @@
 int bm_rbm_kernel_times(bm_rbm *h, float *ms6, int32_t *n6);
 
 int bm_rbm_chain_stats(bm_rbm *h, int64_t *out3);
+
+int bm_rbm_tail_stats(bm_rbm *h, int64_t *out3);
 
 int bm_rbm_timer_start(bm_rbm *h);
 int bm_rbm_timer_stop(bm_rbm *h, float *out_ms);
```

After: 15800. No clear change (-0.4%).
